# rezashkv/diffusion_pruning

Measured on AMD Instinct MI355X. Metric: denoise-steps/s (SD-2.1 U-Net forward, 512x512, bs=4 per GPU, 50% channel mask), higher is better.
Workload: dtype bf16; 1 GPU; BASELINE configs[1]: SD-2.1 UNet2DConditionModelGated.forward, 64x64 latents (512x512), bs=4/GPU, fixed 50% mask (gated semantics), seeded random-init weights, HIP graph replay; global_batch=4, parallelism=replicas x1 (no data-path collective)

## Files before the change

diffusion_pruning_amd/csrc/conv_gemm.hip:

```cpp
#include "conv_gemm_core.h"

using namespace aptp_cg;

namespace {

template <typename T> struct Elem;
template <> struct Elem<__bf16> { static constexpr int EPC = 8, KS = 64; };
template <> struct Elem<float> { static constexpr int EPC = 4, KS = 32; };

template <int BM, int BN, int WM, int WN, typename T = __bf16>
__global__ __launch_bounds__(256) void conv_gemm_kernel(const KParams p) {
  static_assert(WM * WN == 4, "4 waves per workgroup");
  constexpr int EPC = Elem<T>::EPC, KS = Elem<T>::KS, ES = (int)sizeof(T);
  constexpr bool F32 = sizeof(T) == 4;
  constexpr int WTM = BM / WM, WTN = BN / WN;
  constexpr int MF = WTM / 16, NF = WTN / 16;
  constexpr int A_PASS = BM / 32, B_PASS = BN / 32;
  static_assert(BM % 32 == 0 && BN % 32 == 0 && WTM % 16 == 0 && WTN % 16 == 0, "tile shape");

  __shared__ __attribute__((aligned(16))) T smem[2 * (BM + BN) * KS];
  T* As = smem;
  T* Bs = smem + 2 * BM * KS;

  const int tid = threadIdx.x, lane = tid & 63, wave = tid >> 6;
  const int wm = wave / WN, wn = wave % WN;
  const int tiles_n = (p.N + BN - 1) / BN;
  const int tiles_m = (p.M + BM - 1) / BM;
  int tm, tn, kz;
  decode_block(p, tiles_m, tiles_n, tm, tn, kz);
  const int m0 = tm * BM, n0 = tn * BN;
  const int kt_begin = p.fd_sk.div(p.nK * kz);
  const int kt_end = p.fd_sk.div(p.nK * (kz + 1));
  LnRaw<MF> ln_raw;
  ln_rows_issue<MF, WTM>(p, m0, wm, lane, ln_raw);

  const __amdgpu_buffer_rsrc_t xsrc = __builtin_amdgcn_make_buffer_rsrc(const_cast<__bf16*>(p.x), 0, p.x_bytes, 0x00020000);
  const __amdgpu_buffer_rsrc_t wsrc = __builtin_amdgcn_make_buffer_rsrc(const_cast<__bf16*>(p.w), 0, p.w_bytes, 0x00020000);
  const __amdgpu_buffer_rsrc_t x2src = __builtin_amdgcn_make_buffer_rsrc(const_cast<__bf16*>(p.x2 ? p.x2 : p.x), 0, p.x2 ? p.x2_bytes : 0, 0x00020000);
  constexpr unsigned OOB = 0x80000000u;
  const int chunk = tid & 7, rowbase = tid >> 3;
  int a_iy0[A_PASS], a_ix0[A_PASS], a_pix0[A_PASS], a_m[A_PASS];
#pragma unroll
  for (int i = 0; i < A_PASS; ++i) {
    const int m = m0 + rowbase + 32 * i;
    if (m < p.M) {
      const int b = p.fd_hw.div(m), rem = m - b * p.HW;
      const int oy = p.fd_wout.div(rem), ox = rem - oy * p.Wout;
      a_iy0[i] = oy * p.stride - p.pad;
      a_ix0[i] = ox * p.stride - p.pad;
      a_pix0[i] = b * p.Hin * p.Win;
      a_m[i] = m;
    } else {
      a_iy0[i] = -100000; a_ix0[i] = -100000; a_pix0[i] = 0; a_m[i] = -1;
    }
  }
  unsigned b_off[B_PASS];
#pragma unroll
  for (int i = 0; i < B_PASS; ++i) {
    const int n = n0 + rowbase + 32 * i;
    b_off[i] = n < p.N ? (unsigned)(((int64_t)n * p.Ktot + chunk * EPC) * ES) : OOB;
  }

  const int nk_taps = p.KH * p.KW * p.ncc;
  int l_kt = kt_begin;
  int l_tap = 0, l_cc = 0, l_ky = 0, l_kx = 0;
  if (kt_begin != 0) {
    l_tap = kt_begin / p.ncc;
    l_cc = kt_begin - l_tap * p.ncc;
    l_ky = l_tap / p.KW;
    l_kx = l_tap - l_ky * p.KW;
  }
  if (kt_begin >= nk_taps) { l_ky = p.KH; l_kx = 0; l_cc = kt_begin - nk_taps; }

  u32x4 ra[A_PASS], rb[B_PASS];

  auto load_tile = [&](bool pred) {
    const int c = l_cc * KS + chunk * EPC;
    if (l_ky >= p.KH) {
      const bool c_ok = pred && c < p.Cin2;
#pragma unroll
      for (int i = 0; i < A_PASS; ++i) {
        const unsigned off = ((unsigned)a_m[i] * (unsigned)p.ldx2 + (unsigned)c) * (unsigned)ES;
        ra[i] = __builtin_amdgcn_raw_buffer_load_b128(x2src, (c_ok && a_m[i] >= 0) ? off : OOB, 0, 0);
      }
    } else {
      const bool c_ok = pred && c < p.Cin;
#pragma unroll
      for (int i = 0; i < A_PASS; ++i) {
        int iy = a_iy0[i] + l_ky, ix = a_ix0[i] + l_kx;
        const bool ok = c_ok && (unsigned)iy < (unsigned)p.HinE && (unsigned)ix < (unsigned)p.WinE && !(p.zins & (iy | ix));
        iy >>= p.ups; ix >>= p.ups;
        const unsigned off = ((unsigned)(a_pix0[i] + iy * p.Win + ix) * (unsigned)p.ldx + (unsigned)c) * (unsigned)ES;
        ra[i] = __builtin_amdgcn_raw_buffer_load_b128(xsrc, ok ? off : OOB, 0, 0);
      }
    }
    const unsigned koff = (unsigned)l_kt * (KS * ES);
#pragma unroll
    for (int i = 0; i < B_PASS; ++i) {
      rb[i] = __builtin_amdgcn_raw_buffer_load_b128(wsrc, (b_off[i] == OOB || !pred) ? OOB : b_off[i] + koff, 0, 0);
    }
    ++l_kt;
    if (++l_cc == (l_ky >= p.KH ? p.ncc2 : p.ncc)) {
      l_cc = 0;
      if (++l_kx == p.KW || l_ky >= p.KH) { l_kx = 0; ++l_ky; }
    }
  };

  auto store_tile = [&](int buf) {
#pragma unroll
    for (int i = 0; i < A_PASS; ++i) {
      const int r = rowbase + 32 * i;
      const int sw = chunk ^ ((r >> 1) & 7);
      *reinterpret_cast<u32x4*>(As + (buf * BM + r) * KS + sw * EPC) = ra[i];
    }
#pragma unroll
    for (int i = 0; i < B_PASS; ++i) {
      const int r = rowbase + 32 * i;
      const int sw = chunk ^ ((r >> 1) & 7);
      *reinterpret_cast<u32x4*>(Bs + (buf * BN + r) * KS + sw * EPC) = rb[i];
    }
  };

  f32x4 acc[MF][NF];
#pragma unroll
  for (int i = 0; i < MF; ++i)
#pragma unroll
    for (int j = 0; j < NF; ++j) acc[i][j] = (f32x4){0.f, 0.f, 0.f, 0.f};

  const int frow = lane & 15, fq = lane >> 4;
  auto compute = [&](int buf) {
    if constexpr (F32) {
#pragma unroll
// ... 3 lines not shown
        for (int i = 0; i < MF; ++i) {
          const int r = wm * WTM + i * 16 + frow;
          const int sw = (fq * 2 + h) ^ ((r >> 1) & 7);
          af[i] = *reinterpret_cast<const f32x4*>(As + (buf * BM + r) * KS + sw * EPC);
        }
#pragma unroll
        for (int j = 0; j < NF; ++j) {
          const int r = wn * WTN + j * 16 + frow;
          const int sw = (fq * 2 + h) ^ ((r >> 1) & 7);
          wf[j] = *reinterpret_cast<const f32x4*>(Bs + (buf * BN + r) * KS + sw * EPC);
        }
#pragma unroll
        for (int e = 0; e < 4; ++e)
#pragma unroll
          for (int i = 0; i < MF; ++i)
#pragma unroll
            for (int j = 0; j < NF; ++j)
              acc[i][j] = __builtin_amdgcn_mfma_f32_16x16x4f32(wf[j][e], af[i][e], acc[i][j], 0, 0, 0);
      }
    } else {
#pragma unroll
      for (int s = 0; s < 2; ++s) {
        bf16x8 af[MF], wf[NF];
#pragma unroll
        for (int i = 0; i < MF; ++i) {
          const int r = wm * WTM + i * 16 + frow;
          const int sw = (s * 4 + fq) ^ ((r >> 1) & 7);
          af[i] = *reinterpret_cast<const bf16x8*>(As + (buf * BM + r) * KS + sw * EPC);
        }
#pragma unroll
        for (int j = 0; j < NF; ++j) {
          const int r = wn * WTN + j * 16 + frow;
          const int sw = (s * 4 + fq) ^ ((r >> 1) & 7);
          wf[j] = *reinterpret_cast<const bf16x8*>(Bs + (buf * BN + r) * KS + sw * EPC);
        }
#pragma unroll
        for (int i = 0; i < MF; ++i)
#pragma unroll
          for (int j = 0; j < NF; ++j)
            acc[i][j] = __builtin_amdgcn_mfma_f32_16x16x32_bf16(wf[j], af[i], acc[i][j], 0, 0, 0);
      }
    }
  };

  float ln_mean[MF], ln_rstd[MF];
#pragma unroll
  for (int i = 0; i < MF; ++i) { ln_mean[i] = 0.f; ln_rstd[i] = 1.f; }
  {
    load_tile(kt_begin < kt_end);
    ln_rows_finish<MF>(p, lane, ln_raw, ln_mean, ln_rstd);
    store_tile(0);
    __syncthreads();
    int buf = 0;
    for (int kt = kt_begin; kt < kt_end; ++kt) {
      load_tile((kt + 1) < kt_end);
      compute(buf);
      store_tile(buf ^ 1);
      __syncthreads();
      buf ^= 1;
    }
  }

  if (p.split_k > 1 && p.counters) {
    if (!splitk_combine<256, MF, NF>(p, acc, tm * tiles_n + tn, kz, tid, reinterpret_cast<int*>(smem))) return;
    ln_rows_issue<MF, WTM>(p, m0, wm, lane, ln_raw, true);
    ln_rows_finish<MF>(p, lane, ln_raw, ln_mean, ln_rstd, true);
  } else
  if (p.split_k > 1) {
    float* ws = p.ws + (int64_t)kz * p.M * p.ws_ld;
#pragma unroll
    for (int i = 0; i < MF; ++i) {
      const int m = m0 + wm * WTM + i * 16 + frow;
      if (m >= p.M) continue;
#pragma unroll
      for (int j = 0; j < NF; ++j) {
        const int n = n0 + wn * WTN + j * 16 + fq * 4;
        if (n >= p.N) continue;
        float4 o; o.x = acc[i][j][0]; o.y = acc[i][j][1]; o.z = acc[i][j][2]; o.w = acc[i][j][3];
        *reinterpret_cast<float4*>(ws + (int64_t)m * p.ws_ld + n) = o;
      }
    }
    return;
  }
  run_epilogue<4, MF, NF, WTM, WTN, WN>(p, acc, m0, n0, tn, wm, wn, lane, wave, ln_mean, ln_rstd, reinterpret_cast<__bf16*>(smem));
}

__device__ uint4 g_zero_page[512];

template <int BM, int BN, int WM, int WN, int STAGES, bool PP = false, int KU = 1, int KS = 1>
__global__ __launch_bounds__(WM * WN * KS * 64) void conv_gemm_dma_kernel(const KParams p) {
  constexpr int NW = WM * WN;
  constexpr int NWA = NW * KS;
  constexpr int NT = NWA * 64;
  constexpr int RPP = NT / 8;
  static_assert(NWA == 4 || NWA == 8, "4 or 8 waves per workgroup");
  static_assert(KS == 1 || (KS == 2 && !PP), "intra-workgroup K split: two copies, ring schedules only");
  constexpr int WTM = BM / WM, WTN = BN / WN;
  constexpr int MF = WTM / 16, NF = WTN / 16;
  constexpr int A_PASS = (BM + RPP - 1) / RPP, B_PASS = (BN + RPP - 1) / RPP;
  static_assert(WTM % 16 == 0 && WTN % 16 == 0 && BM % 8 == 0 && BN % 8 == 0, "tile shape");

  __shared__ __attribute__((aligned(16))) __bf16 smem[STAGES * (BM + BN) * BK];
  __bf16* As = smem;
  __bf16* Bs = smem + STAGES * BM * BK;

  const int tid = threadIdx.x, lane = tid & 63;
  const int wave = __builtin_amdgcn_readfirstlane(tid >> 6);
  const int ks = KS == 2 ? wave / NW : 0, cw = KS == 2 ? wave % NW : wave;
  const int wm = cw / WN, wn = cw % WN;
  const int tiles_n = (p.N + BN - 1) / BN;
  const int tiles_m = (p.M + BM - 1) / BM;
  int tm, tn, kz;
  decode_block(p, tiles_m, tiles_n, tm, tn, kz);
  const int m0 = tm * BM, n0 = tn * BN;
  const int kt_begin = p.fd_sk.div(p.nK * kz);
  const int kt_end = p.fd_sk.div(p.nK * (kz + 1));
  __shared__ unsigned pf_scratch[64];
  prefetch_next(p, tid, NT, pf_scratch);
  LnRaw<MF> ln_raw;
  ln_rows_issue<MF, WTM>(p, m0, wm, lane, ln_raw);

  const int rowbase = tid >> 3;
  const int schunk = (tid & 7) ^ ((rowbase >> 1) & 7);
  const char* zpage = reinterpret_cast<const char*>(g_zero_page) + schunk * 16;
  const char* xbase = reinterpret_cast<const char*>(p.x) + schunk * 16;
  const bool tail_bad = ((p.ncc - 1) * BK + schunk * 8) >= p.Cin;
  const bool tail_bad2 = ((p.ncc2 - 1) * BK + schunk * 8) >= p.Cin2;
  const char* x2base = reinterpret_cast<const char*>(p.x2) + schunk * 16;
  int a_iy0[A_PASS], a_ix0[A_PASS], a_pix0[A_PASS], a_m[A_PASS];
#pragma unroll
  for (int i = 0; i < A_PASS; ++i) {
    const int m = m0 + rowbase + RPP * i;
    if (m < p.M && rowbase + RPP * i < BM) {
      const int b = p.fd_hw.div(m), rem = m - b * p.HW;
      const int oy = p.fd_wout.div(rem), ox = rem - oy * p.Wout;
      a_iy0[i] = oy * p.stride - p.pad;
      a_ix0[i] = ox * p.stride - p.pad;
      a_pix0[i] = b * p.Hin * p.Win;
      a_m[i] = m;
    } else {
      a_iy0[i] = -100000; a_ix0[i] = -100000; a_pix0[i] = 0; a_m[i] = -1;
    }
  }

  const int nk_taps = p.KH * p.KW * p.ncc;
  int l_tap = 0, l_cc = 0, l_ky = 0, l_kx = 0;
  if (kt_begin != 0) {
    l_tap = kt_begin / p.ncc;
    l_cc = kt_begin - l_tap * p.ncc;
    l_ky = l_tap / p.KW;
    l_kx = l_tap - l_ky * p.KW;
  }
  if (kt_begin >= nk_taps) { l_ky = p.KH; l_kx = 0; l_cc = kt_begin - nk_taps; }

  const char* a_ptr[A_PASS];
  auto set_tap = [&](int cc0) {
    if (l_ky >= p.KH) {
#pragma unroll
      for (int i = 0; i < A_PASS; ++i) {
        const uint64_t va = reinterpret_cast<uint64_t>(x2base) + ((unsigned)a_m[i] * (unsigned)p.ldx2) * 2u + (unsigned)cc0 * (BK * 2);
        const uint64_t vz = reinterpret_cast<uint64_t>(zpage) + (unsigned)cc0 * (BK * 2);
        a_ptr[i] = reinterpret_cast<const char*>((a_m[i] >= 0 && p.x2) ? va : vz);
      }
      return;
    }
#pragma unroll
    for (int i = 0; i < A_PASS; ++i) {
      int iy = a_iy0[i] + l_ky, ix = a_ix0[i] + l_kx;
      const bool ok = (unsigned)iy < (unsigned)p.HinE && (unsigned)ix < (unsigned)p.WinE && !(p.zins & (iy | ix));
      iy >>= p.ups; ix >>= p.ups;
      const unsigned off = ((unsigned)(a_pix0[i] + iy * p.Win + ix) * (unsigned)p.ldx) * 2u + (unsigned)cc0 * (BK * 2);
      const uint64_t va = reinterpret_cast<uint64_t>(xbase) + off;
      const uint64_t vz = reinterpret_cast<uint64_t>(zpage) + (unsigned)cc0 * (BK * 2);
      a_ptr[i] = reinterpret_cast<const char*>(ok ? va : vz);
    }
  };
  const char* b_ptr[B_PASS];
#pragma unroll
  for (int i = 0; i < B_PASS; ++i) {
    int n = n0 + rowbase + RPP * i;
    n = n < p.N ? n : p.N - 1;
    b_ptr[i] = reinterpret_cast<const char*>(p.w) + ((int64_t)n * p.Ktot + (int64_t)kt_begin * BK + schunk * 8) * 2;
  }
  set_tap(l_cc);

  auto issue_tile = [&](int buf) {
    const bool seg2 = l_ky >= p.KH;
    const bool last_cc = l_cc == (seg2 ? p.ncc2 : p.ncc) - 1;
    const bool tb = seg2 ? tail_bad2 : tail_bad;
#pragma unroll
    for (int i = 0; i < A_PASS; ++i) {
      if (wave * 8 + RPP * i < BM) {
        const char* src = (last_cc && tb) ? zpage : a_ptr[i];
        __bf16* dst = As + (buf * BM + wave * 8 + RPP * i) * BK;
        __builtin_amdgcn_global_load_lds((gbl_ptr)src, (lds_ptr)dst, 16, 0, 0);
      }
      a_ptr[i] += BK * 2;
    }
#pragma unroll
    for (int i = 0; i < B_PASS; ++i) {
      if (wave * 8 + RPP * i < BN) {
        __bf16* dst = Bs + (buf * BN + wave * 8 + RPP * i) * BK;
        __builtin_amdgcn_global_load_lds((gbl_ptr)b_ptr[i], (lds_ptr)dst, 16, 0, 0);
      }
      b_ptr[i] += BK * 2;
    }
    if (++l_cc == (seg2 ? p.ncc2 : p.ncc)) {
      l_cc = 0;
      if (++l_kx == p.KW || seg2) { l_kx = 0; ++l_ky; }
      set_tap(0);
    }
  };

  f32x4 acc[MF][NF];
  zero_acc(acc);

  const int frow = lane & 15, fq = lane >> 4;
  auto compute = [&](int buf) {
#pragma unroll
    for (int s0 = 0; s0 < 2 / KS; ++s0) {
      const int s = KS == 2 ? ks : s0;
      bf16x8 af[MF], wf[NF];
#pragma unroll
      for (int i = 0; i < MF; ++i) {
        const int r = wm * WTM + i * 16 + frow;
        const int sw = (s * 4 + fq) ^ ((r >> 1) & 7);
        af[i] = *reinterpret_cast<const bf16x8*>(As + (buf * BM + r) * BK + sw * 8);
      }
#pragma unroll
      for (int j = 0; j < NF; ++j) {
        const int r = wn * WTN + j * 16 + frow;
        const int sw = (s * 4 + fq) ^ ((r >> 1) & 7);
        wf[j] = *reinterpret_cast<const bf16x8*>(Bs + (buf * BN + r) * BK + sw * 8);
      }
#pragma unroll
      for (int i = 0; i < MF; ++i)
#pragma unroll
        for (int j = 0; j < NF; ++j) {
          acc[i][j] = __builtin_amdgcn_mfma_f32_16x16x32_bf16(wf[j], af[i], acc[i][j], 0, 0, 0);
        }
    }
  };

  float ln_mean[MF], ln_rstd[MF];
#pragma unroll
  for (int i = 0; i < MF; ++i) { ln_mean[i] = 0.f; ln_rstd[i] = 1.f; }
  if constexpr (STAGES == 2 && !PP && KU == 1) {
    if (kt_begin < kt_end) {
      issue_tile(0);
      ln_rows_finish<MF>(p, lane, ln_raw, ln_mean, ln_rstd);
      __syncthreads();
      int buf = 0;
      for (int kt = kt_begin; kt < kt_end; ++kt) {
        if (kt + 1 < kt_end) issue_tile(buf ^ 1);
        compute(buf);
        __syncthreads();
        buf ^= 1;
      }
    }
  } else {
    constexpr int D = (PP || KU == 2) ? STAGES - 2 : STAGES - 1;
    constexpr int DW = KU == 2 ? D - 2 : D - 1;
    constexpr int A_FULL = BM / RPP, B_FULL = BN / RPP;
    constexpr int NLD_LO = A_FULL + B_FULL, NLD_HI = A_PASS + B_PASS;
    static_assert(BM % RPP == 0, "ring: the activation tile must be whole row passes");
    static_assert(!PP || (NWA == 8 && KS == 1 && KU == 1), "ping-pong needs 8 waves");
    const bool hi = (NLD_HI != NLD_LO) && (wave * 8 + RPP * (B_PASS - 1) < BN);
    auto wait_ring = [&](bool full) { ring_wait<NLD_LO, NLD_HI, DW>(hi, full); };
    const int n = kt_end - kt_begin;
    if (n > 0) {
      const int pre = n < D ? n : D;
      for (int t = 0; t < pre; ++t) issue_tile(t);
      ln_rows_finish<MF>(p, lane, ln_raw, ln_mean, ln_rstd);
      wait_ring(pre == D);
      __builtin_amdgcn_s_barrier();
      asm volatile("" ::: "memory");
      if constexpr (PP) kloop_pp<STAGES, D>(n, wave >> 2, issue_tile, compute, wait_ring);
      else if constexpr (KU == 2) kloop_ku2<STAGES, D>(n, issue_tile, compute, wait_ring);
      else kloop_ring<STAGES, D>(n, issue_tile, compute, wait_ring);
    }
  }

  if constexpr (KS == 2) {
    f32x4* xch = reinterpret_cast<f32x4*>(smem) + cw * (MF * NF * 64) + lane;
    if (ks == 1) {
#pragma unroll
      for (int i = 0; i < MF; ++i)
#pragma unroll
        for (int j = 0; j < NF; ++j) xch[(i * NF + j) * 64] = acc[i][j];
    }
    __syncthreads();
    if (ks == 1) return;
#pragma unroll
    for (int i = 0; i < MF; ++i)
#pragma unroll
      for (int j = 0; j < NF; ++j) acc[i][j] += xch[(i * NF + j) * 64];
  }
  if (p.split_k > 1 && p.counters) {
    if (!splitk_combine<NW * 64, MF, NF>(p, acc, tm * tiles_n + tn, kz, tid, reinterpret_cast<int*>(smem))) return;
    ln_rows_issue<MF, WTM>(p, m0, wm, lane, ln_raw, true);
    ln_rows_finish<MF>(p, lane, ln_raw, ln_mean, ln_rstd, true);
  } else
  if (p.split_k > 1) {
    store_splitk_slab(p, acc, kz, m0 + wm * WTM, n0 + wn * WTN, frow, fq);
    return;
  }
  static_assert(NW * 16 * (WTN + 4) * 4 <= (int)sizeof(smem), "epilogue transpose buffer");
  static_assert(KS == 1 || NW * MF * NF * 64 * 16 <= (int)sizeof(smem), "accumulator hand-over buffer");
  run_epilogue<NW, MF, NF, WTM, WTN, WN>(p, acc, m0, n0, tn, wm, wn, lane, cw, ln_mean, ln_rstd, smem);
}

template <int BN, int STAGES>
__global__ __launch_bounds__(512) void conv3x3_halo_kernel(const KParams p) {
  constexpr int BM = 128, WM = 4, WN = 2, NW = 8, NT = 512, RPP = 64;
  constexpr int WTM = BM / WM, WTN = BN / WN, MF = WTM / 16, NF = WTN / 16;
  constexpr int PROWS = 264;
  constexpr int P_PASS = (PROWS + RPP - 1) / RPP, B_PASS = (BN + RPP - 1) / RPP;
  constexpr int D = STAGES - 1;
  static_assert(WTN % 16 == 0 && STAGES >= 3, "tile shape");

  __shared__ __attribute__((aligned(16))) __bf16 smem[2 * PROWS * BK + STAGES * BN * BK];
  __bf16* Ps = smem;
  __bf16* Bs = smem + 2 * PROWS * BK;

  const int tid = threadIdx.x, lane = tid & 63;
  const int wave = __builtin_amdgcn_readfirstlane(tid >> 6);
  const int wm = wave / WN, wn = wave % WN;
  const int tiles_n = (p.N + BN - 1) / BN;
  const int tiles_m = (p.M + BM - 1) / BM;
  int tm, tn, kz;
  decode_block(p, tiles_m, tiles_n, tm, tn, kz);
  const int m0 = tm * BM, n0 = tn * BN;
  const int kt_begin = p.fd_sk.div(p.nK * kz);
  const int kt_end = p.fd_sk.div(p.nK * (kz + 1));
  LnRaw<MF> ln_raw;
  ln_rows_issue<MF, WTM>(p, m0, wm, lane, ln_raw);

  const int W = p.Wout, PW = W + 2, R = BM / W;
  const int prows = (R + 2) * PW;
  const int b_img = p.fd_hw.div(m0), oy0 = (m0 - b_img * p.HW) / W;

  const int rowbase = tid >> 3;
  const int schunk = (tid & 7) ^ ((rowbase >> 1) & 7);
  const char* zpage = reinterpret_cast<const char*>(g_zero_page) + schunk * 16;
  const bool tail_bad = ((p.ncc - 1) * BK + schunk * 8) >= p.Cin;
  const char* p_ptr[P_PASS];
#pragma unroll
  for (int i = 0; i < P_PASS; ++i) {
    const int pr_ = rowbase + RPP * i;
    const int pr = pr_ / PW, pc = pr_ - pr * PW;
    const int iy = oy0 - 1 + pr, ix = pc - 1;
    const bool ok = pr_ < prows && (unsigned)iy < (unsigned)p.Hin && (unsigned)ix < (unsigned)p.Win;
    const unsigned off = ((unsigned)((b_img * p.Hin + iy) * p.Win + ix) * (unsigned)p.ldx) * 2u;
    p_ptr[i] = ok ? reinterpret_cast<const char*>(p.x) + off + schunk * 16 : nullptr;
  }
  auto issue_patch = [&](int cc, int pbuf) {
    const bool bad = tail_bad && cc == p.ncc - 1;
#pragma unroll
    for (int i = 0; i < P_PASS; ++i) {
      if (wave * 8 + RPP * i < prows) {
        const char* src = (p_ptr[i] && !bad) ? p_ptr[i] + cc * (BK * 2) : zpage;
        __bf16* dst = Ps + (pbuf * PROWS + wave * 8 + RPP * i) * BK;
        __builtin_amdgcn_global_load_lds((gbl_ptr)src, (lds_ptr)dst, 16, 0, 0);
      }
    }
  };
  const char* b_row[B_PASS];
#pragma unroll
  for (int i = 0; i < B_PASS; ++i) {
    int n = n0 + rowbase + RPP * i;
    n = n < p.N ? n : p.N - 1;
    b_row[i] = reinterpret_cast<const char*>(p.w) + ((int64_t)n * p.Ktot + schunk * 8) * 2;
  }
  const int cin_pad = p.ncc * BK;
  auto issue_w = [&](int kt, int stage) {
    const int cc = kt / 9, tap = kt - cc * 9;
    const int koff = (tap * cin_pad + cc * BK) * 2;
#pragma unroll
    for (int i = 0; i < B_PASS; ++i) {
      if (wave * 8 + RPP * i < BN) {
        __bf16* dst = Bs + (stage * BN + wave * 8 + RPP * i) * BK;
        __builtin_amdgcn_global_load_lds((gbl_ptr)(b_row[i] + koff), (lds_ptr)dst, 16, 0, 0);
      }
    }
  };

  f32x4 acc[MF][NF];
  zero_acc(acc);

  const int frow = lane & 15, fq = lane >> 4;
  int prow0[MF];
#pragma unroll
// ... 15 lines not shown
        af[i] = *reinterpret_cast<const bf16x8*>(Ps + (pbuf * PROWS + pr_) * BK + sw * 8);
      }
#pragma unroll
      for (int j = 0; j < NF; ++j) {
        const int r = wn * WTN + j * 16 + frow;
        const int sw = (s2 * 4 + fq) ^ ((r >> 1) & 7);
        wf[j] = *reinterpret_cast<const bf16x8*>(Bs + (stage * BN + r) * BK + sw * 8);
      }
#pragma unroll
      for (int i = 0; i < MF; ++i)
#pragma unroll
        for (int j = 0; j < NF; ++j)
          acc[i][j] = __builtin_amdgcn_mfma_f32_16x16x32_bf16(wf[j], af[i], acc[i][j], 0, 0, 0);
    }
  };

  float ln_mean[MF], ln_rstd[MF];
#pragma unroll
  for (int i = 0; i < MF; ++i) { ln_mean[i] = 0.f; ln_rstd[i] = 1.f; }

  constexpr int B_FULL = BN / RPP;
  constexpr int NLD_LO = B_FULL, NLD_HI = B_PASS;
  const bool hi = (NLD_HI != NLD_LO) && (wave * 8 + RPP * (B_PASS - 1) < BN);
  const int nld = hi ? NLD_HI : NLD_LO;
  int pw_cnt = 0;
#pragma unroll
  for (int i = 0; i < P_PASS; ++i) pw_cnt += (wave * 8 + RPP * i < prows) ? 1 : 0;
  auto wait_vm = [&](int allowed) {
    switch (allowed) {
      case 4: asm volatile("s_waitcnt vmcnt(4)" ::: "memory"); break;
      case 6: asm volatile("s_waitcnt vmcnt(6)" ::: "memory"); break;
      case 7: asm volatile("s_waitcnt vmcnt(7)" ::: "memory"); break;
      case 8: asm volatile("s_waitcnt vmcnt(8)" ::: "memory"); break;
      case 9: asm volatile("s_waitcnt vmcnt(9)" ::: "memory"); break;
      case 10: asm volatile("s_waitcnt vmcnt(10)" ::: "memory"); break;
      case 11: asm volatile("s_waitcnt vmcnt(11)" ::: "memory"); break;
      default: asm volatile("s_waitcnt vmcnt(0)" ::: "memory"); break;
    }
  };
  const int n = kt_end - kt_begin;
  if (n > 0) {
    const int cc_first = kt_begin / 9;
    issue_patch(cc_first, cc_first & 1);
    const int pre = n < D ? n : D;
    for (int t = 0; t < pre; ++t) issue_w(kt_begin + t, t);
    ln_rows_finish<MF>(p, lane, ln_raw, ln_mean, ln_rstd);
    ring_wait<NLD_LO, NLD_HI, D - 1>(hi, pre == D);
    __builtin_amdgcn_s_barrier();
    asm volatile("" ::: "memory");
    int cur = 0, nxt = D % STAGES;
    int cc = cc_first, tap = kt_begin - cc_first * 9;
    int since_patch = D;
    for (int kt = kt_begin; kt < kt_end; ++kt) {
      const bool issue = kt + D < kt_end;
      if (issue) issue_w(kt + D, nxt);
      if ((tap == 0 || kt == kt_begin) && (cc + 1) * 9 < kt_end) { issue_patch(cc + 1, (cc + 1) & 1); since_patch = 0; }
      compute(cc & 1, tap, cur);
      asm volatile("" ::: "memory");
      if (issue) wait_vm(nld * (D - 1) + (since_patch < D ? pw_cnt : 0));
      else asm volatile("s_waitcnt vmcnt(0)" ::: "memory");
      ++since_patch;
      asm volatile("s_waitcnt lgkmcnt(0)" ::: "memory");
      __builtin_amdgcn_s_barrier();
      asm volatile("" ::: "memory");
      cur = cur + 1 == STAGES ? 0 : cur + 1;
      nxt = nxt + 1 == STAGES ? 0 : nxt + 1;
      if (++tap == 9) { tap = 0; ++cc; }
    }
  }

  if (p.split_k > 1 && p.counters) {
    if (!splitk_combine<NT, MF, NF>(p, acc, tm * tiles_n + tn, kz, tid, reinterpret_cast<int*>(smem))) return;
    ln_rows_issue<MF, WTM>(p, m0, wm, lane, ln_raw, true);
    ln_rows_finish<MF>(p, lane, ln_raw, ln_mean, ln_rstd, true);
  } else
  if (p.split_k > 1) {
    store_splitk_slab(p, acc, kz, m0 + wm * WTM, n0 + wn * WTN, frow, fq);
    return;
  }
  static_assert(NW * 16 * (WTN + 4) * 4 <= (int)sizeof(smem), "epilogue transpose buffer");
  run_epilogue<NW, MF, NF, WTM, WTN, WN>(p, acc, m0, n0, tn, wm, wn, lane, wave, ln_mean, ln_rstd, smem);
}

__global__ __launch_bounds__(256) void splitk_reduce_kernel(const KParams p) {
  const int quads = (p.act == APTP_ACT_GEGLU) ? p.N / 8 : p.N / 4;
  const int64_t idx = (int64_t)blockIdx.x * blockDim.x + threadIdx.x;
  if (idx >= (int64_t)p.M * quads) return;
  const int m = (int)(idx / quads);
  const int q = (int)(idx - (int64_t)m * quads);
  int n;
  if (p.act == APTP_ACT_GEGLU) n = (q >> 2) * 32 + (q & 3) * 4;
  else n = q * 4;
  float h[4] = {0.f, 0.f, 0.f, 0.f}, g[4] = {0.f, 0.f, 0.f, 0.f};
  for (int z0 = 0; z0 < p.split_k; z0 += 4) {
    float4 a[4], c[4];
#pragma unroll
    for (int u = 0; u < 4; ++u) {
      const int z = z0 + u < p.split_k ? z0 + u : z0;
      const float* row = p.ws + ((int64_t)z * p.M + m) * p.ws_ld;
      a[u] = *reinterpret_cast<const float4*>(row + n);
      if (p.act == APTP_ACT_GEGLU) c[u] = *reinterpret_cast<const float4*>(row + n + 16);
    }
#pragma unroll
    for (int u = 0; u < 4; ++u) {
      if (z0 + u < p.split_k) {
        h[0] += a[u].x; h[1] += a[u].y; h[2] += a[u].z; h[3] += a[u].w;
        if (p.act == APTP_ACT_GEGLU) { g[0] += c[u].x; g[1] += c[u].y; g[2] += c[u].z; g[3] += c[u].w; }
      }
    }
  }
  RowCtx rc;
  row_info(p, m, rc);
  if (p.ln_stats) {
    const float4* sp = reinterpret_cast<const float4*>(p.ln_stats);
    float a = 0.f, a2 = 0.f;
    for (int pr = 0; pr < (p.ln_slots >> 1); ++pr) { const float4 t = sp[(int64_t)pr * p.M + m]; a += t.x + t.z; a2 += t.y + t.w; }
    ln_finish(p, a, a2, rc);
  }
  float st[2] = {0.f, 0.f};
  if (p.act == APTP_ACT_GEGLU) epilogue_quad<true>(p, m, rc, n, h, g, st);
  else epilogue_quad<false>(p, m, rc, n, h, h, st);
}

constexpr int GN_RED_NT = 1024;
constexpr int GN_RED_QPT = 6;
__global__ __launch_bounds__(GN_RED_NT) void splitk_reduce_gn_kernel(const KParams p) {
  __shared__ float red[2][GN_RED_NT];
  __shared__ float stat[2];
  const int g = blockIdx.x, b = blockIdx.y, tid = threadIdx.x;
  const int cg = p.gn_C / p.gn_groups, qpr = cg >> 2;
  const int nquads = p.HW * qpr;
  float v[GN_RED_QPT][4];
  float s1 = 0.f, s2 = 0.f;
#pragma unroll
  for (int i = 0; i < GN_RED_QPT; ++i) {
    const int q = tid + GN_RED_NT * i;
    if (q < nquads) {
      const int r = q / qpr, n = g * cg + (q - r * qpr) * 4;
      const int m = b * p.HW + r;
      float a[4] = {0.f, 0.f, 0.f, 0.f};
      for (int z0 = 0; z0 < p.split_k; z0 += 4) {
        float4 t[4];
#pragma unroll
        for (int u = 0; u < 4; ++u) {
          const int z = z0 + u < p.split_k ? z0 + u : z0;
          t[u] = *reinterpret_cast<const float4*>(p.ws + ((int64_t)z * p.M + m) * p.ws_ld + n);
        }
#pragma unroll
        for (int u = 0; u < 4; ++u)
          if (z0 + u < p.split_k) { a[0] += t[u].x; a[1] += t[u].y; a[2] += t[u].z; a[3] += t[u].w; }
      }
#pragma unroll
      for (int e = 0; e < 4; ++e) {
        float x = a[e];
        if (p.bias) x += p.bias[n + e];
        if (p.rowbias) x += p.rowbias[(int64_t)b * p.ld_rowbias + n + e];
        x = (float)(__bf16)x;
        v[i][e] = x;
        s1 += x; s2 += x * x;
      }
    }
  }
  red[0][tid] = s1; red[1][tid] = s2;
  __syncthreads();
  if (tid < 64) {
    float a = 0.f, c = 0.f;
#pragma unroll
    for (int w = 0; w < GN_RED_NT / 64; ++w) { a += red[0][tid + 64 * w]; c += red[1][tid + 64 * w]; }
#pragma unroll
    for (int off = 32; off >= 1; off >>= 1) { a += __shfl_xor(a, off); c += __shfl_xor(c, off); }
    if (tid == 0) {
      const float inv = 1.0f / ((float)cg * (float)p.HW);
      const float mean = a * inv;
      float var = c * inv - mean * mean;
      var = var < 0.f ? 0.f : var;
      stat[0] = mean; stat[1] = rsqrtf(var + p.gn_eps);
    }
  }
  __syncthreads();
  const float mean = stat[0], rstd = stat[1];
  __bf16* y = reinterpret_cast<__bf16*>(p.y);
#pragma unroll
  for (int i = 0; i < GN_RED_QPT; ++i) {
    const int q = tid + GN_RED_NT * i;
    if (q < nquads) {
      const int r = q / qpr, n = g * cg + (q - r * qpr) * 4;
      const int m = b * p.HW + r;
      float o[4];
#pragma unroll
      for (int e = 0; e < 4; ++e) {
        const float z = (v[i][e] - mean) * rstd * p.gn_gamma[n + e] + p.gn_beta[n + e];
        o[e] = p.gn_silu ? silu_f(z) : z;
      }
      uint2 pk; pk.x = pack_bf16x2(o[0], o[1]); pk.y = pack_bf16x2(o[2], o[3]);
      *reinterpret_cast<uint2*>(y + (int64_t)m * p.ldy + n) = pk;
    }
  }
  if (g == p.gn_groups - 1 && p.N > p.gn_C) {
    const int padw = p.N - p.gn_C;
    for (int e = tid; e < p.HW * padw; e += GN_RED_NT) {
      const int r = e / padw, n = p.gn_C + (e - r * padw);
      y[(int64_t)(b * p.HW + r) * p.ldy + n] = (__bf16)0.0f;
    }
  }
}

int pick_tile(const AptpConvGemmParams* p, int M) {
  if (p->tile != APTP_TILE_AUTO) return p->tile;
  const bool geglu = p->act == APTP_ACT_GEGLU;
  auto waste = [&](int bn) { return ((p->N + bn - 1) / bn) * bn - p->N; };
  int bn = 128;
  if (!geglu && waste(160) < waste(128)) bn = 160;
  if (p->N <= 64 || (waste(64) < waste(bn) && p->N < 128)) bn = 64;
  auto blocks = [&](int bm, int bn_) { return (int64_t)((M + bm - 1) / bm) * ((p->N + bn_ - 1) / bn_); };
  int bm = blocks(128, bn) >= 512 ? 128 : 64;
  if (bn == 160) return bm == 128 ? APTP_TILE_128x160 : APTP_TILE_64x160;
  if (bn == 128) return bm == 128 ? APTP_TILE_128x128 : APTP_TILE_64x128;
  return bm == 128 ? APTP_TILE_128x64 : APTP_TILE_64x64;
}

int fill_kparams(const AptpConvGemmParams* p, KParams& k) {
  APTP_CHECK(p && p->x && p->w && p->y, "conv_gemm: null pointer");
  APTP_CHECK(p->B > 0 && p->Hin > 0 && p->Win > 0 && p->Hout > 0 && p->Wout > 0, "conv_gemm: bad extent");
  APTP_CHECK(p->Cin > 0 && p->Cin % 8 == 0, "conv_gemm: Cin (%d) must be a positive multiple of 8", p->Cin);
  APTP_CHECK(p->ldx % 8 == 0 && p->ldx >= p->Cin, "conv_gemm: ldx (%lld) must be a multiple of 8 and >= Cin", (long long)p->ldx);
  APTP_CHECK(p->N > 0 && p->N % 8 == 0, "conv_gemm: N (%d) must be a positive multiple of 8", p->N);
  APTP_CHECK(p->cin_pad % BK == 0 && p->cin_pad >= p->Cin && p->cin_pad < p->Cin + BK, "conv_gemm: cin_pad (%d) != ceil(Cin/64)*64", p->cin_pad);
  APTP_CHECK(p->KH >= 1 && p->KW >= 1 && p->stride >= 1 && p->pad >= 0 && p->ups >= 0 && p->ups <= 2, "conv_gemm: bad filter geometry");
  APTP_CHECK(((uintptr_t)p->x % 16) == 0 && ((uintptr_t)p->w % 16) == 0 && ((uintptr_t)p->y % 8) == 0, "conv_gemm: pointer alignment");
  APTP_CHECK((p->act >= APTP_ACT_NONE && p->act <= APTP_ACT_GELU) || p->act == APTP_ACT_QUICK_GELU, "conv_gemm: unknown act %d", p->act);
  const int geglu = p->act == APTP_ACT_GEGLU;
  APTP_CHECK(!geglu || p->N % 32 == 0, "conv_gemm: GEGLU needs N %% 32 == 0");
  const int nout = geglu ? p->N / 2 : p->N;
  APTP_CHECK(p->ldy >= nout && p->ldy % 4 == 0, "conv_gemm: ldy (%lld) must be >= %d and a multiple of 4", (long long)p->ldy, nout);
  APTP_CHECK(!p->colgate || (p->gate_group > 0 && p->gate_B > 0 && nout % p->gate_group == 0), "conv_gemm: bad gate geometry");
  APTP_CHECK(!p->corr || (p->corr_B > 0 && p->Hout >= 2 && p->Wout >= 2), "conv_gemm: corr needs Hout,Wout >= 2");
  APTP_CHECK(!p->residual || (p->ldres % 4 == 0 && ((uintptr_t)p->residual % 8) == 0), "conv_gemm: residual alignment");
  APTP_CHECK(!p->depth || (p->depth_in && p->depth_B > 0 && p->lddin % 4 == 0), "conv_gemm: depth gate needs depth_in");
  APTP_CHECK(!p->rowbias || p->ld_rowbias % 4 == 0, "conv_gemm: ld_rowbias must be a multiple of 4");
  APTP_CHECK(p->split_k >= 1, "conv_gemm: split_k >= 1");
  const int64_t M64 = (int64_t)p->B * p->Hout * p->Wout;
  APTP_CHECK(M64 < (1ll << 31), "conv_gemm: M too large");
  const int sh = p->ups ? 1 : 0;
  const int HinE = p->Hin << sh, WinE = p->Win << sh;
  APTP_CHECK(p->pad_end >= 0, "conv_gemm: pad_end (%d) must be >= 0", p->pad_end);
  APTP_CHECK(p->pad_end == 0 || (!p->corr && !p->x2 && p->ups == 0), "conv_gemm: pad_end > 0 does not go with corr, x2 or ups");
  APTP_CHECK(p->Hout == (HinE + 2 * p->pad + p->pad_end - p->KH) / p->stride + 1 &&
             p->Wout == (WinE + 2 * p->pad + p->pad_end - p->KW) / p->stride + 1,
             "conv_gemm: Hout/Wout inconsistent with input extent, filter, stride and padding");
  k.x = (const __bf16*)p->x; k.ldx = p->ldx;
  k.B = p->B; k.Hin = p->Hin; k.Win = p->Win; k.Cin = p->Cin; k.Hout = p->Hout; k.Wout = p->Wout;
  k.KH = p->KH; k.KW = p->KW; k.stride = p->stride; k.pad = p->pad; k.ups = sh; k.zins = p->ups == 2 ? 1 : 0;
  k.HinE = HinE; k.WinE = WinE;
  const int f32 = p->io_f32 ? 1 : 0, es = f32 ? 4 : 2, ks = f32 ? 32 : BK;
  APTP_CHECK(!f32 || (p->out_f32 && !p->colstat_out && !p->gn_gamma && !p->prefetch),
             "conv_gemm: io_f32 (fp32 parity path) writes fp32 and has no column statistics / fused GroupNorm / prefetch");
  k.io_f32 = f32;
  k.x2 = (const __bf16*)p->x2; k.ldx2 = p->ldx2; k.Cin2 = p->x2 ? p->Cin2 : 0; k.ncc2 = p->x2 ? p->cin2_pad / ks : 0; k.x2_bytes = 0;
  if (p->x2) {
    APTP_CHECK(p->Cin2 > 0 && p->Cin2 % 8 == 0 && p->cin2_pad % BK == 0 && p->cin2_pad >= p->Cin2 && p->cin2_pad < p->Cin2 + BK,
               "conv_gemm: x2 needs Cin2 (%d) a positive multiple of 8 and cin2_pad (%d) == ceil(Cin2/64)*64", p->Cin2, p->cin2_pad);
    APTP_CHECK(p->ldx2 % 8 == 0 && p->ldx2 >= p->Cin2 && ((uintptr_t)p->x2 % 16) == 0, "conv_gemm: x2 row stride / alignment");
    APTP_CHECK(p->stride == 1 && p->ups == 0 && p->Hout == p->Hin && p->Wout == p->Win,
               "conv_gemm: x2 (second operand read at the output pixel) needs a stride-1, same-size convolution");
    const int64_t x2b = (((int64_t)p->B * p->Hout * p->Wout - 1) * p->ldx2 + p->Cin2) * es;
    APTP_CHECK(x2b < (1ll << 31), "conv_gemm: x2 larger than 2 GiB");
    k.x2_bytes = (int)x2b;
  }
  k.w = (const __bf16*)p->w; k.N = p->N; k.ncc = p->cin_pad / ks; k.nK = p->KH * p->KW * k.ncc + k.ncc2;
  k.Ktot = (int64_t)k.nK * ks;
  k.bias = p->bias; k.rowbias = p->rowbias; k.ld_rowbias = p->ld_rowbias;
  k.colgate = p->colgate; k.gate_group = p->gate_group; k.gate_B = p->gate_B;
  k.act = p->act; k.corr = p->corr; k.corr_B = p->corr_B;
  k.residual = (const __bf16*)p->residual; k.ldres = p->ldres;
  k.depth = p->depth; k.depth_B = p->depth_B; k.depth_in = (const __bf16*)p->depth_in; k.lddin = p->lddin;
  k.y = p->y; k.ldy = p->ldy; k.out_f32 = p->out_f32;
  k.split_k = p->split_k < k.nK ? p->split_k : k.nK;
  k.ws = (float*)p->workspace;
  k.M = (int)M64; k.HW = p->Hout * p->Wout; k.Nout = nout;
  k.ws_ld = p->N;
  APTP_CHECK(p->order >= 0 && p->order <= 3, "conv_gemm: order %d", p->order);
  if (p->order == 0) {
    const int64_t w_bytes = (int64_t)p->N * k.Ktot * 2;
    const int64_t a_bytes = (int64_t)p->B * p->Hin * p->Win * p->Cin * 2;
    k.order = w_bytes > a_bytes ? 1 : 2;
  } else {
    k.order = p->order - 1;
  }
  k.rstat_out = p->rowstat_out; k.rstat_slots = p->rowstat_slots;
  k.ln_stats = p->ln_stats; k.ln_slots = p->ln_slots; k.ln_colsum = p->ln_colsum; k.ln_eps = p->ln_eps;
  k.ln_invC = p->ln_C > 0 ? 1.0f / (float)p->ln_C : 0.f;
  APTP_CHECK(!p->rowstat_out || (!geglu && (!p->out_f32 || f32) && ((uintptr_t)p->rowstat_out % 16) == 0),
             "conv_gemm: rowstat_out needs a bf16, non-GEGLU output and an 8-byte aligned buffer");
  APTP_CHECK(!p->ln_stats || (p->ln_colsum && p->ln_slots > 0 && p->ln_C > 0 && p->KH == 1 && p->KW == 1 &&
                              p->ln_slots % 2 == 0 && ((uintptr_t)p->ln_stats % 16) == 0 && ((uintptr_t)p->ln_colsum % 16) == 0),
             "conv_gemm: folded LayerNorm needs ln_colsum [N], ln_slots > 0, ln_C > 0 and a 1x1 filter");
  k.counters = p->tile_counters;
  k.pf_ptr = ((uintptr_t)p->prefetch & 3) ? nullptr : (const char*)p->prefetch;
  k.pf_bytes = k.pf_ptr ? (p->prefetch_bytes < (1ll << 36) ? p->prefetch_bytes : (1ll << 36)) : 0;
  k.cstat_out = p->colstat_out; k.cstat_ld = p->colstat_ld;
  k.ustat_out = (long long*)p->ustat_out; k.ustat_unit = p->ustat_unit; k.ustat_units = p->ustat_units; k.ustat_nrep = p->ustat_nrep;
  APTP_CHECK(!p->ustat_out || (p->colstat_out && p->ustat_unit > 0 && p->ustat_units * p->ustat_unit >= nout && p->ustat_nrep >= 1 &&
                               (p->ustat_nrep & (p->ustat_nrep - 1)) == 0 && ((uintptr_t)p->ustat_out % 8) == 0),
             "conv_gemm: ustat_out goes with colstat_out; ustat_unit > 0, ustat_units >= ceil(N_out / unit), ustat_nrep a power of two");
  k.epi16 = !p->out_f32 && p->ldy % 8 == 0 && ((uintptr_t)p->y % 16) == 0 && nout % 8 == 0 &&
            (!p->residual || (p->ldres % 8 == 0 && ((uintptr_t)p->residual % 16) == 0)) &&
            (!p->depth || (p->lddin % 8 == 0 && ((uintptr_t)p->depth_in % 16) == 0));
  if (p->epilogue == 1) k.epi16 = 0;
  const int64_t xb = (((int64_t)p->B * p->Hin * p->Win - 1) * p->ldx + p->Cin) * es;
  const int64_t wb = (int64_t)p->N * k.Ktot * es;
  APTP_CHECK(xb < (1ll << 31) && wb < (1ll << 31), "conv_gemm: operand larger than 2 GiB");
  k.x_bytes = (int)xb; k.w_bytes = (int)wb;
  return APTP_OK;
}

template <int BM, int BN>
dim3 tile_grid(const KParams& k) { return dim3(((k.M + BM - 1) / BM) * ((k.N + BN - 1) / BN) * k.split_k, 1, 1); }
template <int BM, int BN, int WM, int WN>
void launch_tile(const KParams& k, hipStream_t s) {
  if (k.io_f32) hipLaunchKernelGGL((conv_gemm_kernel<BM, BN, WM, WN, float>), (tile_grid<BM, BN>(k)), dim3(256), 0, s, k);
  else hipLaunchKernelGGL((conv_gemm_kernel<BM, BN, WM, WN>), (tile_grid<BM, BN>(k)), dim3(256), 0, s, k);
}

template <int BM, int BN, int WM, int WN, int STAGES, bool PP, int KU, int KS>
void launch_dma(const KParams& k, hipStream_t s) {
  hipLaunchKernelGGL((conv_gemm_dma_kernel<BM, BN, WM, WN, STAGES, PP, KU, KS>), (tile_grid<BM, BN>(k)), dim3(WM * WN * KS * 64), 0, s, k);
}

template <int BM, int BN, int STAGES>
int launch_halo(const AptpConvGemmParams* p, const KParams& k, hipStream_t s) {
  static_assert(BM == 128, "conv3x3_halo_kernel: 128 output pixels per tile");
  const int W = p->Wout;
  if (!(p->KH == 3 && p->KW == 3 && p->stride == 1 && p->pad == 1 && p->pad_end == 0 && p->ups == 0 && !p->x2 && W > 0 && 128 % W == 0 &&
        (p->Hout * W) % 128 == 0 && (128 / W + 2) * (W + 2) <= 264)) {
    aptp_set_error("conv_gemm: the halo tiles need a 3x3 / stride-1 / pad-1 convolution without x2 whose width divides 128 (16, 32 or 64)");
    return APTP_EINVAL;
  }
  hipLaunchKernelGGL((conv3x3_halo_kernel<BN, STAGES>), (tile_grid<BM, BN>(k)), dim3(512), 0, s, k);
  return APTP_OK;
}

template <TileFamily F, int BM, int BN, int WM, int WN, int STAGES, int KU, int KS>
int launch_row(const AptpConvGemmParams* p, const KParams& k, int t, hipStream_t s) {
  if constexpr (F == TileFamily::REG) launch_tile<BM, BN, WM, WN>(k, s);
  else if constexpr (F == TileFamily::DMA || F == TileFamily::PP) launch_dma<BM, BN, WM, WN, STAGES, F == TileFamily::PP, KU, KS>(k, s);
  else if constexpr (F == TileFamily::HALO) return launch_halo<BM, BN, STAGES>(p, k, s);
  else if (k.split_k > 1 && !k.counters) { aptp_set_error("conv_gemm: the stream-K tiles combine in-kernel: split_k > 1 needs tile_counters"); return APTP_EINVAL; }
  else return aptp_launch_sk(k, t, s);
  return APTP_OK;
}

}

extern "C" int64_t aptp_conv_gemm_workspace_bytes(const AptpConvGemmParams* p) {
  if (!p || p->split_k <= 1) return 0;
  const int64_t M = (int64_t)p->B * p->Hout * p->Wout;
  const int t = pick_tile(p, (int)M);
  if (is_sk_tile(t))
    return (int64_t)aptp_sk_cus() * 2 * kTiles[t].bm * kTiles[t].bn * (int64_t)sizeof(float);
  int64_t mp = M, np = p->N;
  if (t > 0 && t < kNumTiles) {
    mp = (M + kTiles[t].bm - 1) / kTiles[t].bm * kTiles[t].bm;
    np = ((int64_t)p->N + kTiles[t].bn - 1) / kTiles[t].bn * kTiles[t].bn;
  }
  return (int64_t)p->split_k * mp * np * (int64_t)sizeof(float);
}

extern "C" int aptp_conv_gemm_tiles(const AptpConvGemmParams* p) {
  if (!p) return 0;
  const int64_t M = (int64_t)p->B * p->Hout * p->Wout;
  const int t = pick_tile(p, (int)M);
  if (t <= 0 || t >= kNumTiles) return 0;
  return (int)(((M + kTiles[t].bm - 1) / kTiles[t].bm) * ((p->N + kTiles[t].bn - 1) / kTiles[t].bn));
}

extern "C" int aptp_conv_gemm_colstat_rows(const AptpConvGemmParams* p) {
  if (!p) return 0;
  const int t = pick_tile(p, p->B * p->Hout * p->Wout);
  if (t <= 0 || t >= kNumTiles) return 0;
  return kTiles[t].bm / (kTiles[t].nw / kTiles[t].wn);
}

extern "C" int aptp_conv_gemm_rowstat_slots(const AptpConvGemmParams* p) {
  if (!p) return 0;
  const int t = pick_tile(p, p->B * p->Hout * p->Wout);
  if (t <= 0 || t >= kNumTiles) return 0;
  return ((p->N + kTiles[t].bn - 1) / kTiles[t].bn) * kTiles[t].wn;
}

extern "C" int aptp_conv_gemm_suggest_split_k(const AptpConvGemmParams* p) {
  if (!p) return 1;
  const int M = p->B * p->Hout * p->Wout;
  const int t = pick_tile(p, M);
  const int64_t blocks = (int64_t)((M + kTiles[t].bm - 1) / kTiles[t].bm) * ((p->N + kTiles[t].bn - 1) / kTiles[t].bn);
  const int nK = p->KH * p->KW * (p->cin_pad / BK);
  if (blocks >= 256) return 1;
  int s = (int)((512 + blocks - 1) / blocks);
  const int max_s = nK / 8 > 0 ? nK / 8 : 1;
  if (s > max_s) s = max_s;
  if (s > 32) s = 32;
  return s < 1 ? 1 : s;
}

extern "C" int aptp_conv_gemm(const AptpConvGemmParams* p, aptp_stream_t stream) {
  KParams k;
  const int rc = fill_kparams(p, k);
  if (rc != APTP_OK) return rc;
  if (k.split_k > 1) APTP_CHECK(k.ws != nullptr && ((uintptr_t)k.ws % 16) == 0, "conv_gemm: split_k > 1 needs a 16B-aligned workspace");
  if (k.split_k == 1) k.counters = nullptr;
  k.gn_gamma = p->gn_gamma; k.gn_beta = p->gn_beta; k.gn_groups = p->gn_groups; k.gn_C = p->gn_C; k.gn_silu = p->gn_silu; k.gn_eps = p->gn_eps;
  if (k.gn_gamma) {
    APTP_CHECK(k.gn_beta && k.split_k > 1 && !k.counters && !k.out_f32 && k.act == APTP_ACT_NONE && !k.colgate && !k.corr && !k.residual && !k.depth
               && !k.rstat_out && !k.cstat_out && !k.ln_stats, "conv_gemm: gn_gamma needs a plain bf16 convolution split along K with a reduce launch");
    APTP_CHECK(k.gn_groups > 0 && k.gn_C > 0 && k.gn_C <= k.N && k.gn_C % k.gn_groups == 0 && k.gn_C % 8 == 0 && (k.gn_C / k.gn_groups) % 4 == 0
               && (int64_t)k.HW * (k.gn_C / k.gn_groups) <= 4LL * GN_RED_QPT * GN_RED_NT && k.ldy % 4 == 0,
               "conv_gemm: gn_gamma geometry (C=%d groups=%d HW=%d)", k.gn_C, k.gn_groups, k.HW);
  }
  hipStream_t s = (hipStream_t)stream;
  int t = pick_tile(p, k.M);
  if (t < 0 || t >= kNumTiles) { aptp_set_error("conv_gemm: unknown tile %d", t); return APTP_EINVAL; }
  if (k.io_f32 && !is_reg_tile(t)) {
    aptp_set_error("conv_gemm: io_f32 (fp32 parity path) runs on the register-staged tiles 1..6 only (got tile %d)", t);
    return APTP_EINVAL;
  }
  if (is_dma_tile(t) && (p->cin_pad * 2 > 8064 || (p->x2 && p->cin2_pad * 2 > 8064))) {
    aptp_set_error("conv_gemm: LDS-DMA tiles need Cin <= 4032 (got cin_pad %d)", p->cin_pad);
    return APTP_EINVAL;
  }
  if (k.rstat_out) {
    const int slots = ((k.N + kTiles[t].bn - 1) / kTiles[t].bn) * kTiles[t].wn;
    if ((k.split_k != 1 && !k.counters) || k.rstat_slots != slots) {
      aptp_set_error("conv_gemm: rowstat_out needs split_k == 1 (or the in-kernel reduction) and rowstat_slots == aptp_conv_gemm_rowstat_slots() (%d), got split_k %d, slots %d",
                     slots, k.split_k, k.rstat_slots);
      return APTP_EINVAL;
    }
  }
  if (k.cstat_out) {
    const int wtm = kTiles[t].bm / (kTiles[t].nw / kTiles[t].wn), wtn = kTiles[t].bn / kTiles[t].wn;
    if (!k.epi16 || k.act == APTP_ACT_GEGLU || (k.split_k != 1 && !k.counters) || k.HW % wtm != 0 || wtn < 32 ||
        k.cstat_ld < k.Nout || ((uintptr_t)k.cstat_out % 8) != 0) {
      aptp_set_error("conv_gemm: colstat_out needs the coalesced bf16 epilogue, no GEGLU, split_k == 1 (or the in-kernel reduction), "
                     "Hout*Wout %% %d == 0 (aptp_conv_gemm_colstat_rows) and colstat_ld >= N", wtm);
      return APTP_EINVAL;
    }
    const int wl = k.act == APTP_ACT_GEGLU ? wtn / 2 : wtn;
    if (k.ustat_out && (wl % k.ustat_unit == 0 ? wl / k.ustat_unit : (wl - 1) / k.ustat_unit + 2) > 64) {
      aptp_set_error("conv_gemm: ustat_unit %d too small for the %d columns of a wave of tile %d (at most 64 units per wave)", k.ustat_unit, wl, t);
      return APTP_EINVAL;
    }
  }
  if (k.act == APTP_ACT_GEGLU && (kTiles[t].bn == 160)) {
    aptp_set_error("conv_gemm: GEGLU cannot use a 160-wide tile");
    return APTP_EINVAL;
  }
  {
    const int tiles_m = (k.M + kTiles[t].bm - 1) / kTiles[t].bm, tiles_n = (k.N + kTiles[t].bn - 1) / kTiles[t].bn;
    APTP_CHECK((int64_t)tiles_m * tiles_n * k.split_k < (1ll << 31) && (int64_t)k.nK * (k.split_k + 1) < (1ll << 31), "conv_gemm: grid too large");
    k.fd_hw = make_fastdiv(k.HW); k.fd_wout = make_fastdiv(k.Wout);
    k.fd_tm = make_fastdiv(tiles_m); k.fd_tn = make_fastdiv(tiles_n); k.fd_sk = make_fastdiv(k.split_k);
    k.fd_perm = make_fastdiv(tiles_n * k.split_k); k.fd_tmn = make_fastdiv(tiles_m * tiles_n);
  }
  static const bool lin_on = !(getenv("APTP_LIN") && getenv("APTP_LIN")[0] == '0');
  if (lin_on && p->epilogue != 2 && p->pad_end == 0 && aptp_lin_eligible(k, t)) {
    const int rc2 = aptp_launch_lin(k, t, s);
    if (rc2 != APTP_OK) return rc2;
    APTP_LAUNCH_CHECK();
    return APTP_OK;
  }
  static const bool lean_on = !(getenv("APTP_CONV_LEAN") && getenv("APTP_CONV_LEAN")[0] == '0');
  int rc2 = APTP_OK;
  if (lean_on && p->epilogue == 0 && p->pad_end == 0 && aptp_conv_lean_eligible(k, t)) rc2 = aptp_launch_conv_lean(k, t, s);
  else switch (t) {
#define X(NAME, FAMILY, BM, BN, WM, WN, STAGES, KU, KS, LIN, C3) \
    case APTP_TILE_##NAME: rc2 = launch_row<TileFamily::FAMILY, BM, BN, WM, WN, STAGES, KU, KS>(p, k, t, s); break;
    APTP_CONV_GEMM_TILES(X)
#undef X
    default: aptp_set_error("conv_gemm: unknown tile %d", t); return APTP_EINVAL;
  }
  if (rc2 != APTP_OK) return rc2;
  APTP_LAUNCH_CHECK();
  if (k.split_k > 1 && !k.counters) {
    if (k.gn_gamma) {
      hipLaunchKernelGGL(splitk_reduce_gn_kernel, dim3(k.gn_groups, k.B), dim3(GN_RED_NT), 0, s, k);
    } else {
      const int quads = (k.act == APTP_ACT_GEGLU) ? k.N / 8 : k.N / 4;
      const int64_t total = (int64_t)k.M * quads;
      hipLaunchKernelGGL(splitk_reduce_kernel, dim3((unsigned)((total + 255) / 256)), dim3(256), 0, s, k);
    }
    APTP_LAUNCH_CHECK();
  }
  return APTP_OK;
}
```

diffusion_pruning_amd/csrc/conv_gemm_core.h:

```cpp
#pragma once
#include "aptp_common.h"

namespace aptp_cg {


constexpr int BK = 64;
typedef __attribute__((ext_vector_type(4))) unsigned int u32x4;

struct FastDiv {
  unsigned mul, shr, one;
  __device__ __forceinline__ int div(int n) const { return (int)((__umulhi((unsigned)n, mul) + ((unsigned)n & one)) >> shr); }
};

struct KParams {
  const __bf16* x; int64_t ldx;
  int B, Hin, Win, Cin, Hout, Wout, KH, KW, stride, pad, ups;
  int zins;
  int HinE, WinE;
  const __bf16* w; int N; int ncc; int nK; int64_t Ktot;
  const __bf16* x2; int64_t ldx2; int Cin2; int ncc2; int x2_bytes;
  const float* bias; const float* rowbias; int ld_rowbias;
  const float* colgate; int gate_group, gate_B;
  int act;
  const float* corr; int corr_B;
  const __bf16* residual; int64_t ldres;
  const float* depth; int depth_B; const __bf16* depth_in; int64_t lddin;
  void* y; int64_t ldy; int out_f32;
  int split_k; float* ws;
  int x_bytes, w_bytes;
  int M, HW, Nout;
  int64_t ws_ld;
  int order;
  const char* pf_ptr; int64_t pf_bytes;
  int pf_lines, pf_per;
  int* counters;
  float* cstat_out; int cstat_ld;
  int epi16;
  int io_f32;
  float* rstat_out; int rstat_slots;
  const float* ln_stats; int ln_slots; const float* ln_colsum; float ln_eps; float ln_invC;
  const float* gn_gamma; const float* gn_beta; int gn_groups, gn_C, gn_silu; float gn_eps;
  long long* ustat_out; int ustat_unit, ustat_units, ustat_nrep;
  FastDiv fd_hw, fd_wout;
  FastDiv fd_tm, fd_tn, fd_sk, fd_perm, fd_tmn;
};

__device__ __forceinline__ void decode_block(const KParams& p, int tiles_m, int tiles_n, int& tm, int& tn, int& kz) {
  const int L = blockIdx.x;
  if (p.order == 0) {
    kz = p.fd_tmn.div(L);
    const int t = L - kz * (tiles_m * tiles_n);
    tm = p.fd_tn.div(t);
    tn = t - tm * tiles_n;
    return;
  }
  const int T = gridDim.x;
  const int xcd = L & 7, j = L >> 3;
  const int qq = T >> 3, r = T & 7;
  const int q = (xcd < r ? xcd * (qq + 1) : r * (qq + 1) + (xcd - r) * qq) + j;
  if (p.order == 1) {
    const int w = p.fd_tm.div(q);
    tm = q - w * tiles_m;
    tn = p.fd_sk.div(w);
    kz = w - tn * p.split_k;
  } else {
    const int per_m = tiles_n * p.split_k;
    tm = p.fd_perm.div(q);
    const int rest = q - tm * per_m;
    kz = p.fd_tn.div(rest);
    tn = rest - kz * tiles_n;
  }
}

struct RowCtx { int b, cls; float mean, rstd; };

struct ColVecs { float4 cs, cg, bb, bg; };

template <bool GEGLU>
__device__ __forceinline__ void load_colvecs(const KParams& p, int n, ColVecs& c) {
  c.cs = c.cg = c.bb = c.bg = make_float4(0.f, 0.f, 0.f, 0.f);
  if (p.ln_stats) {
    c.cs = *reinterpret_cast<const float4*>(p.ln_colsum + n);
    if (GEGLU) c.cg = *reinterpret_cast<const float4*>(p.ln_colsum + n + 16);
  }
  if (p.bias) {
    c.bb = *reinterpret_cast<const float4*>(p.bias + n);
    if (GEGLU) c.bg = *reinterpret_cast<const float4*>(p.bias + n + 16);
  }
}

template <bool GEGLU>
__device__ __forceinline__ void epilogue_pre(const KParams& p, const RowCtx& rc, int n, const ColVecs& cv, float h[4], float g[4], float v[4]) {
  const int b = rc.b, cls = rc.cls;
  if (p.ln_stats) {
    h[0] = rc.rstd * (h[0] - rc.mean * cv.cs.x); h[1] = rc.rstd * (h[1] - rc.mean * cv.cs.y);
    h[2] = rc.rstd * (h[2] - rc.mean * cv.cs.z); h[3] = rc.rstd * (h[3] - rc.mean * cv.cs.w);
    if (GEGLU) {
      g[0] = rc.rstd * (g[0] - rc.mean * cv.cg.x); g[1] = rc.rstd * (g[1] - rc.mean * cv.cg.y);
      g[2] = rc.rstd * (g[2] - rc.mean * cv.cg.z); g[3] = rc.rstd * (g[3] - rc.mean * cv.cg.w);
    }
  }
  if (p.bias) {
    h[0] += cv.bb.x; h[1] += cv.bb.y; h[2] += cv.bb.z; h[3] += cv.bb.w;
    if (GEGLU) { g[0] += cv.bg.x; g[1] += cv.bg.y; g[2] += cv.bg.z; g[3] += cv.bg.w; }
  }
  if (p.rowbias) {
    const float4 rb = *reinterpret_cast<const float4*>(p.rowbias + (int64_t)b * p.ld_rowbias + n);
    h[0] += rb.x; h[1] += rb.y; h[2] += rb.z; h[3] += rb.w;
  }
  const int c = GEGLU ? ((n >> 5) * 16 + (n & 15)) : n;
  if (p.colgate) {
    const float* gr = p.colgate + (int64_t)(b % p.gate_B) * ((GEGLU ? p.Nout : p.N) / p.gate_group);
#pragma unroll
    for (int r = 0; r < 4; ++r) {
      const float gm = gr[(c + r) / p.gate_group];
      h[r] *= gm;
      if (GEGLU) g[r] *= gm;
    }
  }
  if (GEGLU) {
#pragma unroll
    for (int r = 0; r < 4; ++r) v[r] = h[r] * gelu_erf_f(g[r]);
  } else if (p.act == APTP_ACT_SILU) {
#pragma unroll
    for (int r = 0; r < 4; ++r) v[r] = silu_f(h[r]);
  } else if (p.act == APTP_ACT_GELU) {
#pragma unroll
    for (int r = 0; r < 4; ++r) v[r] = gelu_erf_f(h[r]);
  } else if (p.act == APTP_ACT_QUICK_GELU) {
#pragma unroll
    for (int r = 0; r < 4; ++r) v[r] = quick_gelu_f(h[r]);
  } else {
#pragma unroll
    for (int r = 0; r < 4; ++r) v[r] = h[r];
  }
  if (p.corr) {
    const float4 cc = *reinterpret_cast<const float4*>(p.corr + ((int64_t)(b % p.corr_B) * 9 + cls) * p.Nout + c);
    v[0] += cc.x; v[1] += cc.y; v[2] += cc.z; v[3] += cc.w;
  }
}

template <bool GEGLU>
__device__ __forceinline__ void epilogue_quad(const KParams& p, int m, const RowCtx& rc, int n, float h[4], float g[4], float st[2]) {
  const int b = rc.b;
  float v[4];
  ColVecs cv;
  load_colvecs<GEGLU>(p, n, cv);
  epilogue_pre<GEGLU>(p, rc, n, cv, h, g, v);
  const int c = GEGLU ? ((n >> 5) * 16 + (n & 15)) : n;
  if (p.residual) {
    if (p.io_f32) {
      const float4 rr = *reinterpret_cast<const float4*>(reinterpret_cast<const float*>(p.residual) + (int64_t)m * p.ldres + c);
      v[0] += rr.x; v[1] += rr.y; v[2] += rr.z; v[3] += rr.w;
    } else {
      const uint2 rr = *reinterpret_cast<const uint2*>(p.residual + (int64_t)m * p.ldres + c);
      union { uint2 u; __bf16 e[4]; } ru; ru.u = rr;
#pragma unroll
      for (int r = 0; r < 4; ++r) v[r] += (float)ru.e[r];
    }
  }
  if (p.depth) {
    const float d = p.depth[b % p.depth_B];
    float din[4];
    if (p.io_f32) {
      const float4 rr = *reinterpret_cast<const float4*>(reinterpret_cast<const float*>(p.depth_in) + (int64_t)m * p.lddin + c);
      din[0] = rr.x; din[1] = rr.y; din[2] = rr.z; din[3] = rr.w;
    } else {
      const uint2 rr = *reinterpret_cast<const uint2*>(p.depth_in + (int64_t)m * p.lddin + c);
      union { uint2 u; __bf16 e[4]; } ru; ru.u = rr;
#pragma unroll
      for (int r = 0; r < 4; ++r) din[r] = (float)ru.e[r];
    }
#pragma unroll
    for (int r = 0; r < 4; ++r) v[r] = (1.0f - d) * din[r] + d * v[r];
  }
  if (p.out_f32) {
    float4 o; o.x = v[0]; o.y = v[1]; o.z = v[2]; o.w = v[3];
    *reinterpret_cast<float4*>(reinterpret_cast<float*>(p.y) + (int64_t)m * p.ldy + c) = o;
    if (p.io_f32 && p.rstat_out) {
#pragma unroll
      for (int r = 0; r < 4; ++r) { st[0] += v[r]; st[1] += v[r] * v[r]; }
    }
  } else {
    union { uint2 u; __bf16 e[4]; } o;
    o.u.x = pack_bf16x2(v[0], v[1]); o.u.y = pack_bf16x2(v[2], v[3]);
    *reinterpret_cast<uint2*>(reinterpret_cast<__bf16*>(p.y) + (int64_t)m * p.ldy + c) = o.u;
    if (p.rstat_out) {
#pragma unroll
      for (int r = 0; r < 4; ++r) { const float f = (float)o.e[r]; st[0] += f; st[1] += f * f; }
    }
  }
}

__device__ __forceinline__ void row_info(const KParams& p, int m, RowCtx& rc) {
  rc.b = p.fd_hw.div(m);
  rc.cls = 4;
  rc.mean = 0.f; rc.rstd = 1.f;
  if (p.corr) {
    const int rem = m - rc.b * p.HW;
    const int oy = p.fd_wout.div(rem), ox = rem - oy * p.Wout;
    const int rr = oy == 0 ? 0 : (oy == p.Hout - 1 ? 2 : 1);
    const int cc = ox == 0 ? 0 : (ox == p.Wout - 1 ? 2 : 1);
    rc.cls = rr * 3 + cc;
  }
}

__device__ __forceinline__ void ln_finish(const KParams& p, float a, float a2, RowCtx& rc) {
  const float mean = a * p.ln_invC;
  float var = a2 * p.ln_invC - mean * mean;
  var = var < 0.f ? 0.f : var;
  rc.mean = mean;
  rc.rstd = rsqrtf(var + p.ln_eps);
}

template <int MF>
struct LnRaw { float4 v[4][MF]; int mr[MF]; };

template <int MF, int WTM>
__device__ __forceinline__ void ln_rows_issue(const KParams& p, int m0, int wm, int lane, LnRaw<MF>& raw, bool split_ok = false) {
  if (!p.ln_stats || (p.split_k > 1 && !split_ok)) return;
  const int frow = lane & 15, fq = lane >> 4;
  const float4* sp = reinterpret_cast<const float4*>(p.ln_stats);
  const int npair = p.ln_slots >> 1;
#pragma unroll
  for (int i = 0; i < MF; ++i) {
    const int m = m0 + wm * WTM + i * 16 + frow;
    raw.mr[i] = m < p.M ? m : p.M - 1;
  }
#pragma unroll
  for (int u = 0; u < 4; ++u) {
    if (u * 4 < npair) {
      const int pr = u * 4 + fq;
      const int64_t row0 = (int64_t)(pr < npair ? pr : 0) * p.M;
#pragma unroll
      for (int i = 0; i < MF; ++i) raw.v[u][i] = sp[row0 + raw.mr[i]];
    } else {
#pragma unroll
      for (int i = 0; i < MF; ++i) raw.v[u][i] = make_float4(0.f, 0.f, 0.f, 0.f);
    }
  }
  asm volatile("" ::: "memory");
}

template <int MF>
__device__ __forceinline__ void ln_rows_finish(const KParams& p, int lane, const LnRaw<MF>& raw, float (&ln_mean)[MF], float (&ln_rstd)[MF],
                                               bool split_ok = false) {
  if (!p.ln_stats || (p.split_k > 1 && !split_ok)) return;
  const int fq = lane >> 4;
  const float4* sp = reinterpret_cast<const float4*>(p.ln_stats);
  const int npair = p.ln_slots >> 1;
  float lna[MF], lna2[MF];
#pragma unroll
  for (int i = 0; i < MF; ++i) { lna[i] = 0.f; lna2[i] = 0.f; }
#pragma unroll
  for (int u = 0; u < 4; ++u) {
    const bool ok = u * 4 + fq < npair;
#pragma unroll
    for (int i = 0; i < MF; ++i) {
      lna[i] += ok ? raw.v[u][i].x + raw.v[u][i].z : 0.f;
      lna2[i] += ok ? raw.v[u][i].y + raw.v[u][i].w : 0.f;
    }
  }
  for (int base = 16; base < npair; base += 16) {
#pragma unroll
    for (int u = 0; u < 4; ++u) {
      if (base + u * 4 < npair) {
        const int pr = base + u * 4 + fq;
        const bool ok = pr < npair;
        const int64_t row0 = (int64_t)(ok ? pr : 0) * p.M;
#pragma unroll
        for (int i = 0; i < MF; ++i) {
          const float4 t = sp[row0 + raw.mr[i]];
          lna[i] += ok ? t.x + t.z : 0.f; lna2[i] += ok ? t.y + t.w : 0.f;
        }
      }
    }
  }
#pragma unroll
  for (int i = 0; i < MF; ++i) {
    lna[i] += __shfl_xor(lna[i], 16); lna2[i] += __shfl_xor(lna2[i], 16);
    lna[i] += __shfl_xor(lna[i], 32); lna2[i] += __shfl_xor(lna2[i], 32);
    RowCtx rc;
    ln_finish(p, lna[i], lna2[i], rc);
    ln_mean[i] = rc.mean; ln_rstd[i] = rc.rstd;
  }
}

template <int MF, int NF, int WTM, int WTN, int WN>
__device__ __forceinline__ void tile_epilogue(const KParams& p, f32x4 (&acc)[MF][NF], int m0, int n0, int tn, int wm, int wn, int lane,
                                              const float (&ln_mean)[MF], const float (&ln_rstd)[MF]) {
  const int frow = lane & 15, fq = lane >> 4;
#pragma unroll
  for (int i = 0; i < MF; ++i) {
    const int m = m0 + wm * WTM + i * 16 + frow;
    if (m >= p.M) continue;
    RowCtx rc;
    row_info(p, m, rc);
    rc.mean = ln_mean[i]; rc.rstd = ln_rstd[i];
    float st[2] = {0.f, 0.f};
    if (p.act == APTP_ACT_GEGLU) {
      if constexpr (NF % 2 == 0) {
#pragma unroll
        for (int j = 0; j < NF; j += 2) {
          const int n = n0 + wn * WTN + j * 16 + fq * 4;
          if (n >= p.N) continue;
          float h[4] = {acc[i][j][0], acc[i][j][1], acc[i][j][2], acc[i][j][3]};
          float g[4] = {acc[i][j + 1][0], acc[i][j + 1][1], acc[i][j + 1][2], acc[i][j + 1][3]};
          epilogue_quad<true>(p, m, rc, n, h, g, st);
        }
      }
    } else {
#pragma unroll
      for (int j = 0; j < NF; ++j) {
        const int n = n0 + wn * WTN + j * 16 + fq * 4;
        if (n >= p.N) continue;
        float h[4] = {acc[i][j][0], acc[i][j][1], acc[i][j][2], acc[i][j][3]};
        epilogue_quad<false>(p, m, rc, n, h, h, st);
      }
    }
    if (p.rstat_out) {
      st[0] += __shfl_xor(st[0], 16); st[1] += __shfl_xor(st[1], 16);
      st[0] += __shfl_xor(st[0], 32); st[1] += __shfl_xor(st[1], 32);
      if (fq == 0) {
        float2 o; o.x = st[0]; o.y = st[1];
        const int slot = tn * WN + wn;
        reinterpret_cast<float2*>(p.rstat_out)[((int64_t)(slot >> 1) * p.M + m) * 2 + (slot & 1)] = o;
      }
    }
  }
}

constexpr float USTAT_SUM_SCALE = 1048576.0f;
constexpr float USTAT_SQ_SCALE = 4096.0f;
template <int WL>
__device__ __forceinline__ void emit_unit_stats(const KParams& p, const float (&tot)[2][(WL + 63) / 64], float* buf, int lane, int cw0,
                                                int row0) {
  __builtin_amdgcn_fence(__ATOMIC_ACQ_REL, "wavefront");
  __builtin_amdgcn_wave_barrier();
#pragma unroll
  for (int q = 0; q < (WL + 63) / 64; ++q) {
    const int t = lane + 64 * q;
    if (t < WL) { buf[t] = tot[0][q]; buf[WL + t] = tot[1][q]; }
  }
  __builtin_amdgcn_fence(__ATOMIC_ACQ_REL, "wavefront");
  __builtin_amdgcn_wave_barrier();
  const int cend = cw0 + WL < p.Nout ? cw0 + WL : p.Nout;
  if (cw0 >= cend || row0 >= p.M) return;
  const int unit = p.ustat_unit;
  const int u0 = cw0 / unit, u1 = (cend - 1) / unit;
  const int u = u0 + lane;
  if (u > u1) return;
  const int lo = (u * unit > cw0 ? u * unit : cw0) - cw0;
  const int hi = ((u + 1) * unit < cend ? (u + 1) * unit : cend) - cw0;
  float s = 0.f, s2 = 0.f;
  for (int c = lo; c < hi; ++c) { s += buf[c]; s2 += buf[WL + c]; }
  const int b = p.fd_hw.div(row0);
  const int rep = (int)blockIdx.x & (p.ustat_nrep - 1);
  unsigned long long* dst = reinterpret_cast<unsigned long long*>(p.ustat_out) + (((int64_t)rep * p.B + b) * p.ustat_units + u) * 2;
  __hip_atomic_fetch_add(dst, (unsigned long long)__float2ll_rn(s * USTAT_SUM_SCALE), __ATOMIC_RELAXED, __HIP_MEMORY_SCOPE_AGENT);
  __hip_atomic_fetch_add(dst + 1, (unsigned long long)__float2ll_rn(s2 * USTAT_SQ_SCALE), __ATOMIC_RELAXED, __HIP_MEMORY_SCOPE_AGENT);
}

template <int WL, int RPP>
__device__ __forceinline__ void emit_col_stats(const KParams& p, const float (&cs)[8], const float (&cs2)[8], float* buf, int lane, int lrow,
                                               int lc8, int cw0, int rblk, int row0) {
  float tot[2][(WL + 63) / 64];
#pragma unroll
  for (int ph = 0; ph < 2; ++ph) {
    if (lrow < RPP) {
      float* dst = buf + lrow * WL + lc8 * 8;
      if (ph == 0) {
        *reinterpret_cast<float4*>(dst) = make_float4(cs[0], cs[1], cs[2], cs[3]);
        *reinterpret_cast<float4*>(dst + 4) = make_float4(cs[4], cs[5], cs[6], cs[7]);
      } else {
        *reinterpret_cast<float4*>(dst) = make_float4(cs2[0], cs2[1], cs2[2], cs2[3]);
        *reinterpret_cast<float4*>(dst + 4) = make_float4(cs2[4], cs2[5], cs2[6], cs2[7]);
      }
    }
    __builtin_amdgcn_fence(__ATOMIC_ACQ_REL, "wavefront");
    __builtin_amdgcn_wave_barrier();
#pragma unroll
    for (int q = 0; q < (WL + 63) / 64; ++q) {
      const int t = lane + 64 * q;
      float a = 0.f;
      if (t < WL) {
#pragma unroll
        for (int r = 0; r < RPP; ++r) a += buf[r * WL + t];
      }
      tot[ph][q] = a;
    }
    __builtin_amdgcn_fence(__ATOMIC_ACQ_REL, "wavefront");
    __builtin_amdgcn_wave_barrier();
  }
  float2* dstg = reinterpret_cast<float2*>(p.cstat_out) + (int64_t)rblk * p.cstat_ld;
#pragma unroll
  for (int q = 0; q < (WL + 63) / 64; ++q) {
    const int t = lane + 64 * q;
    if (t < WL && cw0 + t < p.Nout) dstg[cw0 + t] = make_float2(tot[0][q], tot[1][q]);
  }
  if (p.ustat_out) emit_unit_stats<WL>(p, tot, buf, lane, cw0, row0);
}

template <bool GEGLU, int MF, int NF, int WTM, int WTN, int WN>
__device__ __forceinline__ void tile_epilogue_lds(const KParams& p, f32x4 (&acc)[MF][NF], int m0, int n0, int tn, int wm, int wn,
                                                  int lane, const float (&ln_mean)[MF], const float (&ln_rstd)[MF], float* buf) {
  constexpr int WL = GEGLU ? WTN / 2 : WTN;
  constexpr int PITCH = WL + 4;
  constexpr int LPR = WL / 8;
  constexpr int RPP = 64 / LPR;
  constexpr int NPASS = (16 + RPP - 1) / RPP;
  constexpr bool POW2 = (LPR & (LPR - 1)) == 0;
  const int frow = lane & 15, fq = lane >> 4;
  const int lrow = lane / LPR, lc8 = lane - lrow * LPR;
  const int c0 = (GEGLU ? ((n0 + wn * WTN) >> 1) : (n0 + wn * WTN)) + lc8 * 8;
  const bool lane_on = lrow < RPP && c0 < p.Nout;
  __bf16* const yb = reinterpret_cast<__bf16*>(p.y);
  float cs[8], cs2[8];
#pragma unroll
  for (int e = 0; e < 8; ++e) { cs[e] = 0.f; cs2[e] = 0.f; }
#pragma unroll
  for (int i = 0; i < MF; ++i) {
    const int mbase = m0 + wm * WTM + i * 16;
    u32x4 rres[NPASS], rdin[NPASS];
#pragma unroll
    for (int ps = 0; ps < NPASS; ++ps) {
      const int r = ps * RPP + lrow, m2 = mbase + r;
      const bool on = lane_on && r < 16 && m2 < p.M;
      rres[ps] = (u32x4){0u, 0u, 0u, 0u}; rdin[ps] = (u32x4){0u, 0u, 0u, 0u};
      if (on && p.residual) rres[ps] = *reinterpret_cast<const u32x4*>(p.residual + (int64_t)m2 * p.ldres + c0);
      if (on && p.depth) rdin[ps] = *reinterpret_cast<const u32x4*>(p.depth_in + (int64_t)m2 * p.lddin + c0);
    }
    {
      const int m = mbase + frow;
      RowCtx rc;
      row_info(p, m < p.M ? m : p.M - 1, rc);
      rc.mean = ln_mean[i]; rc.rstd = ln_rstd[i];
      if constexpr (GEGLU) {
        if constexpr (NF % 2 == 0) {
#pragma unroll
          for (int j = 0; j < NF; j += 2) {
            const int n = n0 + wn * WTN + j * 16 + fq * 4;
            float h[4] = {acc[i][j][0], acc[i][j][1], acc[i][j][2], acc[i][j][3]};
            float g[4] = {acc[i][j + 1][0], acc[i][j + 1][1], acc[i][j + 1][2], acc[i][j + 1][3]};
            float v[4] = {0.f, 0.f, 0.f, 0.f};
            if (n < p.N) {
              ColVecs cv;
              load_colvecs<true>(p, n, cv);
              epilogue_pre<true>(p, rc, n, cv, h, g, v);
            }
            *reinterpret_cast<float4*>(buf + frow * PITCH + (j / 2) * 16 + fq * 4) = make_float4(v[0], v[1], v[2], v[3]);
          }
        }
      } else {
#pragma unroll
        for (int j = 0; j < NF; ++j) {
          const int n = n0 + wn * WTN + j * 16 + fq * 4;
          float h[4] = {acc[i][j][0], acc[i][j][1], acc[i][j][2], acc[i][j][3]};
          float v[4] = {0.f, 0.f, 0.f, 0.f};
          if (n < p.N) {
            ColVecs cv;
            load_colvecs<false>(p, n, cv);
            epilogue_pre<false>(p, rc, n, cv, h, h, v);
          }
          *reinterpret_cast<float4*>(buf + frow * PITCH + j * 16 + fq * 4) = make_float4(v[0], v[1], v[2], v[3]);
        }
      }
    }
    __builtin_amdgcn_fence(__ATOMIC_ACQ_REL, "wavefront");
    __builtin_amdgcn_wave_barrier();
#pragma unroll
    for (int ps = 0; ps < NPASS; ++ps) {
      const int r = ps * RPP + lrow, m2 = mbase + r;
      const bool on = lane_on && r < 16 && m2 < p.M;
      float v[8];
      {
        const int rr = r < 16 ? r : 15;
        const float4 a = *reinterpret_cast<const float4*>(buf + rr * PITCH + lc8 * 8);
        const float4 b4 = *reinterpret_cast<const float4*>(buf + rr * PITCH + lc8 * 8 + 4);
        v[0] = a.x; v[1] = a.y; v[2] = a.z; v[3] = a.w; v[4] = b4.x; v[5] = b4.y; v[6] = b4.z; v[7] = b4.w;
      }
      if (p.residual) {
        float f[8];
        union { u32x4 v; uint4 s; } cv; cv.v = rres[ps];
        unpack_bf16x8(cv.s, f);
#pragma unroll
        for (int e = 0; e < 8; ++e) v[e] += f[e];
      }
      if (p.depth) {
        const float d = p.depth[p.fd_hw.div(m2 < p.M ? m2 : p.M - 1) % p.depth_B];
        float f[8];
        union { u32x4 v; uint4 s; } cv; cv.v = rdin[ps];
        unpack_bf16x8(cv.s, f);
#pragma unroll
        for (int e = 0; e < 8; ++e) v[e] = (1.0f - d) * f[e] + d * v[e];
      }
      const uint4 o = pack_bf16x8(v);
      if (on) *reinterpret_cast<uint4*>(yb + (int64_t)m2 * p.ldy + c0) = o;
      if constexpr (!GEGLU) {
        if (p.cstat_out && on) {
          float f[8];
          unpack_bf16x8(o, f);
#pragma unroll
          for (int e = 0; e < 8; ++e) { cs[e] += f[e]; cs2[e] += f[e] * f[e]; }
        }
      }
      if constexpr (POW2) {
        if (p.rstat_out) {
          float f[8], s0 = 0.f, s1 = 0.f;
          unpack_bf16x8(o, f);
          if (c0 < p.Nout) {
#pragma unroll
            for (int e = 0; e < 8; ++e) { s0 += f[e]; s1 += f[e] * f[e]; }
          }
#pragma unroll
          for (int off = 1; off < LPR; off <<= 1) { s0 += __shfl_xor(s0, off); s1 += __shfl_xor(s1, off); }
          if (lrow < RPP && r < 16 && m2 < p.M && lc8 == 0) {
            float2 q; q.x = s0; q.y = s1;
            const int slot = tn * WN + wn;
            reinterpret_cast<float2*>(p.rstat_out)[((int64_t)(slot >> 1) * p.M + m2) * 2 + (slot & 1)] = q;
          }
        }
      }
    }
  }
  if constexpr (!GEGLU && WL >= 32) {
    static_assert(RPP * WL <= 16 * PITCH, "column-statistics staging");
    if (p.cstat_out) emit_col_stats<WL, RPP>(p, cs, cs2, buf, lane, lrow, lc8, n0 + wn * WTN, m0 / WTM + wm, m0 + wm * WTM);
  }
}

template <int WTM, int WTN>
struct LeanEpiIn {
  static constexpr int LPR = WTN / 8, RPF = 64 / LPR, NPF = (16 + RPF - 1) / RPF, NP = (WTM / 16) * NPF;
  float cb[8], rb[8], gm[8];
  float cr[NP][8];
  u32x4 res[NP];
  bool one_b;
};

template <int WTM, int WTN>
__device__ __forceinline__ void lean_epi_sample(const KParams& p, int b, int cc, float (&rb)[8], float (&gm)[8]) {
  if (p.rowbias) {
    const float4 a = *reinterpret_cast<const float4*>(p.rowbias + (int64_t)b * p.ld_rowbias + cc);
    const float4 c = *reinterpret_cast<const float4*>(p.rowbias + (int64_t)b * p.ld_rowbias + cc + 4);
    rb[0] = a.x; rb[1] = a.y; rb[2] = a.z; rb[3] = a.w; rb[4] = c.x; rb[5] = c.y; rb[6] = c.z; rb[7] = c.w;
  }
  if (p.colgate) {
    const float* gr = p.colgate + (int64_t)(b % p.gate_B) * (p.N / p.gate_group);
#pragma unroll
    for (int e = 0; e < 8; ++e) gm[e] = gr[(cc + e) / p.gate_group];
  }
}

template <int WTM, int WTN>
__device__ __forceinline__ void lean_epi_load(const KParams& p, int m0, int n0, int wm, int wn, int lane, LeanEpiIn<WTM, WTN>& in) {
  using E = LeanEpiIn<WTM, WTN>;
  const int lrow = lane / E::LPR, lc8 = lane - lrow * E::LPR;
  const int c0 = n0 + wn * WTN + lc8 * 8;
  const int cc = c0 < p.Nout ? c0 : p.Nout - 8;
  const int mw0 = m0 + wm * WTM;
  const int mf = mw0 < p.M ? mw0 : p.M - 1, ml = mw0 + WTM - 1 < p.M ? mw0 + WTM - 1 : p.M - 1;
  const int b0 = p.fd_hw.div(mf);
  in.one_b = p.fd_hw.div(ml) == b0;
#pragma unroll
  for (int e = 0; e < 8; ++e) { in.cb[e] = 0.f; in.rb[e] = 0.f; in.gm[e] = 1.f; }
  if (p.bias) {
    const float4 a = *reinterpret_cast<const float4*>(p.bias + cc), c = *reinterpret_cast<const float4*>(p.bias + cc + 4);
    in.cb[0] = a.x; in.cb[1] = a.y; in.cb[2] = a.z; in.cb[3] = a.w; in.cb[4] = c.x; in.cb[5] = c.y; in.cb[6] = c.z; in.cb[7] = c.w;
  }
  lean_epi_sample<WTM, WTN>(p, b0, cc, in.rb, in.gm);
#pragma unroll
  for (int q = 0; q < E::NP; ++q) {
    const int i = q / E::NPF, ps = q - i * E::NPF;
    const int r = ps * E::RPF + lrow, m2 = mw0 + i * 16 + (r < 16 ? r : 15);
    const int mc = m2 < p.M ? m2 : p.M - 1;
    in.res[q] = (u32x4){0u, 0u, 0u, 0u};
    if (p.residual) in.res[q] = *reinterpret_cast<const u32x4*>(p.residual + (int64_t)mc * p.ldres + cc);
#pragma unroll
    for (int e = 0; e < 8; ++e) in.cr[q][e] = 0.f;
    if (p.corr) {
      RowCtx rc;
      row_info(p, mc, rc);
      const float* cp = p.corr + ((int64_t)(rc.b % p.corr_B) * 9 + rc.cls) * p.Nout + cc;
      const float4 a = *reinterpret_cast<const float4*>(cp), c = *reinterpret_cast<const float4*>(cp + 4);
      in.cr[q][0] = a.x; in.cr[q][1] = a.y; in.cr[q][2] = a.z; in.cr[q][3] = a.w;
      in.cr[q][4] = c.x; in.cr[q][5] = c.y; in.cr[q][6] = c.z; in.cr[q][7] = c.w;
    }
  }
}

template <int MF, int NF, int WTM, int WTN>
__device__ __forceinline__ void lean_epilogue(const KParams& p, f32x4 (&acc)[MF][NF], int m0, int n0, int wm, int wn, int lane,
                                              const LeanEpiIn<WTM, WTN>& in, float* buf) {
  using E = LeanEpiIn<WTM, WTN>;
  constexpr int WL = WTN, PITCH = WL + 4, LPR = E::LPR, RPF = E::RPF, NPF = E::NPF;
  static_assert(WL % 8 == 0 && WL >= 32 && RPF * WL <= 16 * PITCH, "transposed layout / column-statistics staging");
  const int frow = lane & 15, fq = lane >> 4;
  const int lrow = lane / LPR, lc8 = lane - lrow * LPR;
  const int c0 = n0 + wn * WTN + lc8 * 8;
  const int cc = c0 < p.Nout ? c0 : p.Nout - 8;
  const bool lane_on = lrow < RPF && c0 < p.Nout;
  const int mw0 = m0 + wm * WTM;
  __bf16* const yb = reinterpret_cast<__bf16*>(p.y);
  float cs[8], cs2[8];
#pragma unroll
  for (int e = 0; e < 8; ++e) { cs[e] = 0.f; cs2[e] = 0.f; }
#pragma unroll
  for (int i = 0; i < MF; ++i) {
    if (i > 0) {
      __builtin_amdgcn_fence(__ATOMIC_ACQ_REL, "wavefront");
      __builtin_amdgcn_wave_barrier();
    }
#pragma unroll
    for (int j = 0; j < NF; ++j) *reinterpret_cast<f32x4*>(buf + frow * PITCH + j * 16 + fq * 4) = acc[i][j];
    __builtin_amdgcn_fence(__ATOMIC_ACQ_REL, "wavefront");
    __builtin_amdgcn_wave_barrier();
#pragma unroll
    for (int ps = 0; ps < NPF; ++ps) {
      const int q = i * NPF + ps;
      const int r = ps * RPF + lrow, m2 = mw0 + i * 16 + r;
      const bool on = lane_on && r < 16 && m2 < p.M;
      float v[8];
      {
        const int rr = r < 16 ? r : 15;
        const float4 a = *reinterpret_cast<const float4*>(buf + rr * PITCH + lc8 * 8);
        const float4 b4 = *reinterpret_cast<const float4*>(buf + rr * PITCH + lc8 * 8 + 4);
        v[0] = a.x; v[1] = a.y; v[2] = a.z; v[3] = a.w; v[4] = b4.x; v[5] = b4.y; v[6] = b4.z; v[7] = b4.w;
      }
      float rb[8], gm[8];
#pragma unroll
      for (int e = 0; e < 8; ++e) { rb[e] = in.rb[e]; gm[e] = in.gm[e]; }
      if (!in.one_b && (p.rowbias || p.colgate)) {
        const int mr = mw0 + i * 16 + (r < 16 ? r : 15), mc = mr < p.M ? mr : p.M - 1;
        lean_epi_sample<WTM, WTN>(p, p.fd_hw.div(mc), cc, rb, gm);
      }
      if (p.bias) {
#pragma unroll
        for (int e = 0; e < 8; ++e) v[e] += in.cb[e];
      }
      if (p.rowbias) {
#pragma unroll
        for (int e = 0; e < 8; ++e) v[e] += rb[e];
      }
      if (p.colgate) {
#pragma unroll
        for (int e = 0; e < 8; ++e) v[e] *= gm[e];
      }
      if (p.act == APTP_ACT_SILU) {
#pragma unroll
        for (int e = 0; e < 8; ++e) v[e] = silu_f(v[e]);
      }
      if (p.corr) {
#pragma unroll
        for (int e = 0; e < 8; ++e) v[e] += in.cr[q][e];
      }
#if defined(__HIP_DEVICE_COMPILE__)
#pragma unroll
      for (int e = 0; e < 8; ++e) asm volatile("" : "+v"(v[e]));
#endif
      if (p.residual) {
        float f[8];
        union { u32x4 v; uint4 s; } cv; cv.v = in.res[q];
        unpack_bf16x8(cv.s, f);
#pragma unroll
        for (int e = 0; e < 8; ++e) v[e] += f[e];
      }
      const uint4 o = pack_bf16x8(v);
      if (on) *reinterpret_cast<uint4*>(yb + (int64_t)m2 * p.ldy + c0) = o;
      if (p.cstat_out && on) {
        float f[8];
        unpack_bf16x8(o, f);
#pragma unroll
        for (int e = 0; e < 8; ++e) { cs[e] += f[e]; cs2[e] += f[e] * f[e]; }
      }
    }
  }
  if (p.cstat_out) {
    __builtin_amdgcn_fence(__ATOMIC_ACQ_REL, "wavefront");
    __builtin_amdgcn_wave_barrier();
    emit_col_stats<WL, RPF>(p, cs, cs2, buf, lane, lrow, lc8, n0 + wn * WTN, m0 / WTM + wm, mw0);
  }
}

template <int NT, int MF, int NF>
__device__ __forceinline__ bool splitk_combine(const KParams& p, f32x4 (&acc)[MF][NF], int tile, int kz, int tid, int* lds_word) {
  constexpr int PER = MF * NF;
  float4* const slab = reinterpret_cast<float4*>(p.ws) + (int64_t)tile * p.split_k * (PER * NT);
  float4* const mine = slab + (int64_t)kz * (PER * NT);
  {
    const __amdgpu_buffer_rsrc_t srsrc = __builtin_amdgcn_make_buffer_rsrc(mine, 0, PER * NT * 16, 0x00020000);
#pragma unroll
    for (int i = 0; i < MF; ++i)
#pragma unroll
      for (int j = 0; j < NF; ++j) {
        __builtin_amdgcn_raw_buffer_store_b128(__builtin_bit_cast(u32x4, acc[i][j]), srsrc, ((i * NF + j) * NT + tid) * 16, 0, 16);
      }
  }
  asm volatile("s_waitcnt vmcnt(0)" ::: "memory");
  __syncthreads();
  if (tid == 0) *lds_word = __hip_atomic_fetch_add(p.counters + tile, 1, __ATOMIC_RELAXED, __HIP_MEMORY_SCOPE_AGENT);
  __syncthreads();
  const int ticket = *reinterpret_cast<volatile int*>(lds_word);
  if (ticket != p.split_k - 1) return false;
  if (tid == 0) {
    __hip_atomic_store(p.counters + tile, 0, __ATOMIC_RELAXED, __HIP_MEMORY_SCOPE_AGENT);
    __builtin_amdgcn_fence(__ATOMIC_ACQUIRE, "agent");
    asm volatile("s_waitcnt vmcnt(0)" ::: "memory");
  }
  __syncthreads();
#pragma unroll
  for (int i = 0; i < MF; ++i)
#pragma unroll
    for (int j = 0; j < NF; ++j) acc[i][j] = (f32x4){0.f, 0.f, 0.f, 0.f};
  for (int z = 0; z < p.split_k; ++z) {
    const float4* src = slab + (int64_t)z * (PER * NT);
    float4 t[MF][NF];
#pragma unroll
    for (int i = 0; i < MF; ++i)
#pragma unroll
      for (int j = 0; j < NF; ++j) t[i][j] = src[(i * NF + j) * NT + tid];
#pragma unroll
    for (int i = 0; i < MF; ++i)
#pragma unroll
      for (int j = 0; j < NF; ++j) {
        acc[i][j][0] += t[i][j].x; acc[i][j][1] += t[i][j].y; acc[i][j][2] += t[i][j].z; acc[i][j][3] += t[i][j].w;
      }
  }
  return true;
}

__device__ __forceinline__ void prefetch_next(const KParams& p, int tid, int nt, unsigned* scratch) {
  if (!p.pf_ptr) return;
  const int xcd = blockIdx.x & 7;
  aptp_prefetch_slice(p.pf_ptr, p.pf_bytes, xcd, blockIdx.x >> 3, ((int)gridDim.x + 7 - xcd) >> 3, tid, nt, scratch);
}

template <int NW, int MF, int NF, int WTM, int WTN, int WN>
__device__ __forceinline__ void run_epilogue(const KParams& p, f32x4 (&acc)[MF][NF], int m0, int n0, int tn, int wm, int wn, int lane,
                                             int wave, const float (&ln_mean)[MF], const float (&ln_rstd)[MF], __bf16* smem) {
  constexpr int PITCH_MAX = WTN + 4;
  constexpr bool POW2 = ((WTN / 8) & (WTN / 8 - 1)) == 0;
  if (p.epi16 && (POW2 || !p.rstat_out)) {
    __syncthreads();
    float* buf = reinterpret_cast<float*>(smem) + wave * 16 * PITCH_MAX;
    if (p.act == APTP_ACT_GEGLU) {
      if constexpr (NF % 2 == 0) tile_epilogue_lds<true, MF, NF, WTM, WTN, WN>(p, acc, m0, n0, tn, wm, wn, lane, ln_mean, ln_rstd, buf);
    } else {
      tile_epilogue_lds<false, MF, NF, WTM, WTN, WN>(p, acc, m0, n0, tn, wm, wn, lane, ln_mean, ln_rstd, buf);
    }
  } else {
    tile_epilogue<MF, NF, WTM, WTN, WN>(p, acc, m0, n0, tn, wm, wn, lane, ln_mean, ln_rstd);
  }
}

inline FastDiv make_fastdiv(int d) {
  FastDiv f;
  if (d <= 1) { f.mul = 0; f.shr = 0; f.one = ~0u; return f; }
  int l = 0;
  while ((1ll << l) < d) ++l;
  const int p = 31 + l;
  f.mul = (unsigned)(((1ull << p) + (unsigned)d - 1) / (unsigned)d);
  f.shr = (unsigned)(p - 32);
  f.one = 0;
  return f;
}

int aptp_sk_cus();
int aptp_launch_sk(const KParams& k, int tile, hipStream_t s);
bool aptp_lin_eligible(const KParams& k, int tile);
int aptp_launch_lin(const KParams& k, int tile, hipStream_t s);
bool aptp_conv_lean_eligible(const KParams& k, int tile);
int aptp_launch_conv_lean(const KParams& k, int tile, hipStream_t s);

}

#include "conv_gemm_tiles.h"
#include "conv_gemm_kloop.h"
```

diffusion_pruning_amd/csrc/conv_gemm_sk.hip:

```cpp
#include "conv_gemm_core.h"

using namespace aptp_cg;

namespace {


struct SkParams {
  int G, T, tiles_m, tiles_n, nK, U;
  int whole;
  FastDiv fd_nk, fd_G, fd_U, fd_tm, fd_tn;
};

__device__ __forceinline__ void wait_vm(int allowed) {
  if (allowed >= 7) asm volatile("s_waitcnt vmcnt(7)" ::: "memory");
  else if (allowed >= 6) asm volatile("s_waitcnt vmcnt(6)" ::: "memory");
  else if (allowed >= 3) asm volatile("s_waitcnt vmcnt(3)" ::: "memory");
  else asm volatile("s_waitcnt vmcnt(0)" ::: "memory");
}

__device__ __forceinline__ void wait_tile(int t, int hidx, int cnt_h0, int cnt_h1) {
  const int newer = hidx - (2 * t + 2);
  wait_vm(newer <= 0 ? 0 : ((newer + 1) >> 1) * cnt_h0 + (newer >> 1) * cnt_h1);
}

// ... 258 lines not shown
        slot_barrier();
        cur = nxt;
      }
    } else {
      for (int tt = 0; tt < n; ++tt) {
        read_frags(cur, 0, af0, wf0);
        issue_half();
        slot_barrier();
        __builtin_amdgcn_s_setprio(1);
        mfmas(af0, wf0);
        __builtin_amdgcn_s_setprio(0);
        slot_barrier();
        read_frags(cur, 1, af0, wf0);
        issue_half();
        if (grp == 1) wait_tile(tt + 1, hidx, cnt_h0, cnt_h1);
        slot_barrier();
        __builtin_amdgcn_s_setprio(1);
        mfmas(af0, wf0);
        __builtin_amdgcn_s_setprio(0);
        if (grp == 0) wait_tile(tt + 1, hidx, cnt_h0, cnt_h1);
        slot_barrier();
        cur = cur + 1 == S ? 0 : cur + 1;
      }
    }
    if (grp == 0) slot_barrier();

    bool emit = true;
    if (n != sk.nK) emit = sk_combine<NT, MF, NF>(p, sk, acc, tile, g, tid, reinterpret_cast<int*>(smem));
    if (emit) {
      float ln_mean[MF], ln_rstd[MF];
#pragma unroll
      for (int i = 0; i < MF; ++i) { ln_mean[i] = 0.f; ln_rstd[i] = 1.f; }
      LnRaw<MF> ln_raw;
      ln_rows_issue<MF, WTM>(p, m0, wm, lane, ln_raw, true);
      ln_rows_finish<MF>(p, lane, ln_raw, ln_mean, ln_rstd, true);
      run_epilogue<NW, MF, NF, WTM, WTN, WN>(p, acc, m0, n0, tn, wm, wn, lane, wave, ln_mean, ln_rstd, smem);
    }
    __syncthreads();
    u += n;
  }
}

int g_sk_cus = 0;

template <int BM, int BN, int WM, int WN, bool RDC>
int launch_sk(const KParams& k, hipStream_t s) {
  SkParams sk;
  sk.tiles_m = (k.M + BM - 1) / BM; sk.tiles_n = (k.N + BN - 1) / BN;
  sk.T = sk.tiles_m * sk.tiles_n; sk.nK = k.nK;
  const int64_t U = (int64_t)sk.T * sk.nK;
  const int cus = aptp_sk_cus();
  sk.whole = k.split_k > 1 ? 0 : 1;
  const int64_t units = sk.whole ? sk.T : U;
  sk.G = (int)(units < cus ? units : cus);
  APTP_CHECK(U * (sk.G + 1) < (1ll << 31) && sk.T <= 65536, "conv_gemm: stream-K work list too large (%d tiles x %d K-steps)", sk.T, sk.nK);
  sk.U = (int)U;
  APTP_CHECK(sk.whole || (k.ws && k.counters), "conv_gemm: the stream-K tiles with split_k > 1 need workspace and tile_counters");
  sk.fd_nk = make_fastdiv(sk.nK); sk.fd_G = make_fastdiv(sk.G); sk.fd_U = make_fastdiv(sk.U);
  sk.fd_tm = make_fastdiv(sk.tiles_m); sk.fd_tn = make_fastdiv(sk.tiles_n);
  hipLaunchKernelGGL((conv_gemm_sk_kernel<BM, BN, WM, WN, RDC>), dim3(sk.G), dim3(512), 0, s, k, sk);
  return APTP_OK;
}

}

namespace aptp_cg {

int aptp_sk_cus() {
  if (g_sk_cus == 0) {
    int dev = 0, n = 0;
    if (hipGetDevice(&dev) != hipSuccess || hipDeviceGetAttribute(&n, hipDeviceAttributeMultiprocessorCount, dev) != hipSuccess || n <= 0) n = 256;
    g_sk_cus = n;
  }
  return g_sk_cus;
}

template <TileFamily F, int BM, int BN, int WM, int WN>
static int launch_sk_row(const KParams& k, int tile, hipStream_t s) {
  if constexpr (F == TileFamily::SK || F == TileFamily::SKL) return launch_sk<BM, BN, WM, WN, F == TileFamily::SK>(k, s);
  aptp_set_error("conv_gemm: unknown stream-K tile %d", tile); return APTP_EINVAL;
}

int aptp_launch_sk(const KParams& k, int tile, hipStream_t s) {
  switch (tile) {
#define X(NAME, FAMILY, BM, BN, WM, WN, STAGES, KU, KS, LIN, C3) \
    case APTP_TILE_##NAME: return launch_sk_row<TileFamily::FAMILY, BM, BN, WM, WN>(k, tile, s);
    APTP_CONV_GEMM_TILES(X)
#undef X
  }
  return launch_sk_row<TileFamily::NONE, 0, 0, 0, 0>(k, tile, s);
}

}
```

diffusion_pruning_amd/csrc/conv_lean.hip:

```cpp
#include "conv_gemm_core.h"

namespace {
using namespace aptp_cg;

constexpr unsigned ZERO_OFF = 0x80000000u;
constexpr int NTAB = 10;

__device__ __forceinline__ void dma16(__amdgpu_buffer_rsrc_t r, __bf16* lds, unsigned voff, int soff) {
#if defined(__HIP_DEVICE_COMPILE__)
  __builtin_amdgcn_raw_ptr_buffer_load_lds(r, (lds_ptr)lds, 16, voff, soff, 0, 0);
#endif
}

template <int BM, int BN, int WM, int WN, int STAGES, bool PP, int KU>
__global__ __launch_bounds__(WM * WN * 64) void conv_lean_kernel(const KParams p) {
  constexpr int NW = WM * WN, NT = NW * 64, RPP = NT / 8;
  constexpr int WTM = BM / WM, WTN = BN / WN, MF = WTM / 16, NF = WTN / 16;
  constexpr int A_PASS = BM / RPP, B_PASS = (BN + RPP - 1) / RPP;
  constexpr int B_FULL = BN / RPP, NLD_LO = A_PASS + B_FULL, NLD_HI = A_PASS + B_PASS;
  static_assert(NW == 4 || NW == 8, "4 or 8 waves");
  static_assert(BM % RPP == 0 && WTM % 16 == 0 && WTN % 16 == 0 && BN % 8 == 0, "tile shape");
  static_assert(NW * 16 * (WTN + 4) * 4 <= STAGES * (BM + BN) * BK * 2, "epilogue transpose buffer");

  __shared__ __attribute__((aligned(16))) __bf16 smem[STAGES * (BM + BN) * BK];
  __shared__ unsigned pf_scratch[64];
  __bf16* As = smem;
  __bf16* Bs = smem + STAGES * BM * BK;

  const int tid = threadIdx.x, lane = tid & 63;
  const int wave = __builtin_amdgcn_readfirstlane(tid >> 6);
  const int wm = wave / WN, wn = wave % WN;
  const int tiles_n = (p.N + BN - 1) / BN, tiles_m = (p.M + BM - 1) / BM;
  int tm, tn, kz;
  decode_block(p, tiles_m, tiles_n, tm, tn, kz);
  const int m0 = tm * BM, n0 = tn * BN;
  const int kt_begin = p.fd_sk.div(p.nK * kz);
  const int kt_end = p.fd_sk.div(p.nK * (kz + 1));

  prefetch_hosted(p, tid, NT, pf_scratch);

  const int rowbase = tid >> 3;
  const unsigned schunk = (unsigned)((tid & 7) ^ ((rowbase >> 1) & 7));
  unsigned tab[A_PASS][NTAB];
#pragma unroll
  for (int i = 0; i < A_PASS; ++i) {
    const int m = m0 + rowbase + RPP * i;
    if (m < p.M) {
      const int b = p.fd_hw.div(m), rem = m - b * p.HW;
      const int oy = p.fd_wout.div(rem), ox = rem - oy * p.Wout;
      const int iy0 = oy * p.stride - 1, ix0 = ox * p.stride - 1, pix0 = b * p.Hin * p.Win;
#pragma unroll
      for (int t = 0; t < 9; ++t) {
        int iy = iy0 + t / 3, ix = ix0 + t % 3;
        const bool ok = (unsigned)iy < (unsigned)p.HinE && (unsigned)ix < (unsigned)p.WinE && !(p.zins & (iy | ix));
        iy >>= p.ups; ix >>= p.ups;
        tab[i][t] = ok ? ((unsigned)(pix0 + iy * p.Win + ix) * (unsigned)p.ldx) * 2u + schunk * 16u : ZERO_OFF;
      }
      tab[i][9] = p.x2 ? ((unsigned)m * (unsigned)p.ldx2) * 2u + schunk * 16u : ZERO_OFF;
    } else {
#pragma unroll
      for (int t = 0; t < NTAB; ++t) tab[i][t] = ZERO_OFF;
    }
  }
  unsigned boff[B_PASS];
#pragma unroll
  for (int i = 0; i < B_PASS; ++i) {
    int n = n0 + rowbase + RPP * i;
    n = n < p.N ? n : p.N - 1;
    boff[i] = (unsigned)(n * (unsigned)p.Ktot) * 2u + schunk * 16u;
  }
  const bool tail_bad = (int)((p.ncc - 1) * BK + schunk * 8) >= p.Cin;
  const bool tail_bad2 = (int)((p.ncc2 - 1) * BK + schunk * 8) >= p.Cin2;
  const __amdgpu_buffer_rsrc_t xr = __builtin_amdgcn_make_buffer_rsrc(const_cast<__bf16*>(p.x), 0, p.x_bytes, 0x00020000);
  const __amdgpu_buffer_rsrc_t x2r =
      __builtin_amdgcn_make_buffer_rsrc(const_cast<__bf16*>(p.x2 ? p.x2 : p.x), 0, p.x2 ? p.x2_bytes : 0, 0x00020000);
  const __amdgpu_buffer_rsrc_t wr = __builtin_amdgcn_make_buffer_rsrc(const_cast<__bf16*>(p.w), 0, p.w_bytes, 0x00020000);

  int l_kt = kt_begin, l_tap = 0, l_cc = kt_begin;
  if (kt_begin != 0) {
    l_tap = kt_begin / p.ncc;
    if (l_tap > 9) l_tap = 9;
    l_cc = kt_begin - l_tap * p.ncc;
  }
  auto next_tap = [&]() {
#pragma unroll
    for (int i = 0; i < A_PASS; ++i)
#pragma unroll
      for (int t = 0; t + 1 < NTAB; ++t) tab[i][t] = tab[i][t + 1];
  };
  for (int t = 0; t < l_tap; ++t) next_tap();

  auto issue_tile = [&](int stage) {
    const bool seg2 = l_tap == 9;
    const int ncur = seg2 ? p.ncc2 : p.ncc;
    const bool pad = l_cc == ncur - 1 && (seg2 ? tail_bad2 : tail_bad);
    const int sa = __builtin_amdgcn_readfirstlane(l_cc * (BK * 2));
    const int sb = __builtin_amdgcn_readfirstlane(l_kt * (BK * 2));
#pragma unroll
    for (int i = 0; i < A_PASS; ++i) {
      __bf16* dst = As + (stage * BM + wave * 8 + RPP * i) * BK;
      if (seg2) dma16(x2r, dst, pad ? ZERO_OFF : tab[i][0], sa);
      else dma16(xr, dst, pad ? ZERO_OFF : tab[i][0], sa);
    }
#pragma unroll
    for (int i = 0; i < B_PASS; ++i) {
      if (wave * 8 + RPP * i < BN) {
        __bf16* dst = Bs + (stage * BN + wave * 8 + RPP * i) * BK;
        dma16(wr, dst, boff[i], sb);
      }
    }
    ++l_kt;
    if (++l_cc == ncur) {
      l_cc = 0;
      if (l_tap < 9) {
        ++l_tap;
        next_tap();
      }
    }
  };

  f32x4 acc[MF][NF];
  zero_acc(acc);
  const int frow = lane & 15, fq = lane >> 4;
  auto compute = [&](int stage) {
#pragma unroll
    for (int s = 0; s < 2; ++s) {
      bf16x8 af[MF], wf[NF];
#pragma unroll
      for (int i = 0; i < MF; ++i) {
        const int r = wm * WTM + i * 16 + frow;
        af[i] = *reinterpret_cast<const bf16x8*>(As + (stage * BM + r) * BK + ((s * 4 + fq) ^ ((r >> 1) & 7)) * 8);
      }
#pragma unroll
      for (int j = 0; j < NF; ++j) {
        const int r = wn * WTN + j * 16 + frow;
        wf[j] = *reinterpret_cast<const bf16x8*>(Bs + (stage * BN + r) * BK + ((s * 4 + fq) ^ ((r >> 1) & 7)) * 8);
      }
#pragma unroll
      for (int i = 0; i < MF; ++i)
#pragma unroll
        for (int j = 0; j < NF; ++j) acc[i][j] = __builtin_amdgcn_mfma_f32_16x16x32_bf16(wf[j], af[i], acc[i][j], 0, 0, 0);
    }
  };

  constexpr int D = PP ? STAGES - 2 : (KU == 2 ? STAGES - 2 : STAGES - 1);
  constexpr int DW = KU == 2 ? D - 2 : D - 1;
  static_assert(STAGES >= 2 && D >= 1, "ring");
  static_assert(!PP || NW == 8, "ping-pong: 8 waves");
  static_assert(KU == 1 || !PP, "two K-tiles per barrier: ring schedule only");
  const bool hi = (NLD_HI != NLD_LO) && (wave * 8 + RPP * (B_PASS - 1) < BN);
  auto wait_ring = [&](bool full) { ring_wait<NLD_LO, NLD_HI, DW>(hi, full); };
  const int n = kt_end - kt_begin;
  const int pre = n < D ? n : D;
  for (int t = 0; t < pre; ++t) issue_tile(t);
  LeanEpiIn<WTM, WTN> ein;
  if (p.split_k == 1) lean_epi_load<WTM, WTN>(p, m0, n0, wm, wn, lane, ein);

  if (n > 0) {
    wait_ring(pre == D);
    __builtin_amdgcn_s_barrier();
    asm volatile("" ::: "memory");
    if constexpr (PP) kloop_pp<STAGES, D>(n, wave >> 2, issue_tile, compute, wait_ring);
    else if constexpr (KU == 2) kloop_ku2<STAGES, D>(n, issue_tile, compute, wait_ring);
    else kloop_ring<STAGES, D>(n, issue_tile, compute, wait_ring);
  }

  if (p.split_k > 1 && p.counters) {
    if (!splitk_combine<NT, MF, NF>(p, acc, tm * tiles_n + tn, kz, tid, reinterpret_cast<int*>(smem))) return;
    lean_epi_load<WTM, WTN>(p, m0, n0, wm, wn, lane, ein);
  } else if (p.split_k > 1) {
    store_splitk_slab(p, acc, kz, m0 + wm * WTM, n0 + wn * WTN, frow, fq);
    return;
  }
  __syncthreads();
  lean_epilogue<MF, NF, WTM, WTN>(p, acc, m0, n0, wm, wn, lane, ein, reinterpret_cast<float*>(smem) + wave * 16 * (WTN + 4));
}

template <int BM, int BN, int WM, int WN, int STAGES, bool PP, int KU>
void launch_lean(KParams k, hipStream_t s) {
  const int grid = ((k.M + BM - 1) / BM) * ((k.N + BN - 1) / BN) * k.split_k;
  set_prefetch_slices(k, grid);
  hipLaunchKernelGGL((conv_lean_kernel<BM, BN, WM, WN, STAGES, PP, KU>), dim3(grid), dim3(WM * WN * 64), 0, s, k);
}

}

namespace aptp_cg {

bool aptp_conv_lean_eligible(const KParams& k, int tile) {
  if (k.KH != 3 || k.KW != 3 || k.pad != 1 || (k.stride != 1 && k.stride != 2)) return false;
  if (k.io_f32 || k.out_f32 || !k.epi16 || k.ln_stats || k.rstat_out || k.depth) return false;
  if (k.act != APTP_ACT_NONE && k.act != APTP_ACT_SILU) return false;
  if (k.Nout < 8 || k.ncc < 1) return false;
  return tile_known(tile) && kTiles[tile].c3;
}

template <bool C3, int BM, int BN, int WM, int WN, int STAGES, bool PP, int KU>
static bool launch_lean_row(const KParams& k, hipStream_t s) {
  if constexpr (C3) launch_lean<BM, BN, WM, WN, STAGES, PP, KU>(k, s);
  return C3;
}

int aptp_launch_conv_lean(const KParams& k, int tile, hipStream_t s) {
  switch (tile) {
#define X(NAME, FAMILY, BM, BN, WM, WN, STAGES, KU, KS, LIN, C3) case APTP_TILE_##NAME: \
    if (launch_lean_row<C3 != 0, BM, BN, WM, WN, STAGES, TileFamily::FAMILY == TileFamily::PP, KU>(k, s)) return APTP_OK; break;
    APTP_CONV_GEMM_TILES(X)
#undef X
  }
  aptp_set_error("conv_lean: tile %d has no lean instantiation", tile); return APTP_EINVAL;
}

}
```

diffusion_pruning_amd/launch_policy.py:

```python
import json
import math
import os
import re

from . import _lib as L

BK = 64
DMA_TILE_FIRST = L.TILE_DMA_128x128
DMA_MAX_CHANNELS = 4032
SK_TILE_FIRST = L.TILE_SK_256x160
SK_MAX_CHANNELS = 32704
_HALO_TILES = (L.TILE_HALO_128x160, L.TILE_HALO_128x128)
_LEAN_TILES = frozenset(getattr(L, "TILE_" + t) for t in (
    "DMA_64x128 DMA_128x64 DMA_64x64 DMA3_64x128 DMA3_128x64 DMA3_64x64 DMA4_64x128 DMA4_64x64 DMA4_128x64 DMA6_64x64 DMA8S_64x64 "
    "DMA6_64x128 DMA6_128x64 KU2S4_64x64 KU2S6_64x64 KU2S4_64x128 KU2S6_64x128 KU2S4_128x64").split())

TUNING_NEAREST = os.environ.get("APTP_TUNING_NEAREST", "1") != "0"
TUNING_MAX_DIST = 2.0
LEAN_REMAP = os.environ.get("APTP_LEAN_REMAP", "1") != "0"
SK_AUTO = os.environ.get("APTP_SK_AUTO", "1") == "1"
SK_AUTO_MIN_OUTPUTS = 256 * 256 * 160
SK_AUTO_MIN_KSTEPS = 16
SPLITK_FORCE_IN_KERNEL = os.environ.get("APTP_SPLITK_FORCE_INKERNEL", "0") == "1"
COLS_SPLIT_MAX = int(os.environ.get("APTP_COLS_SPLIT_MAX", "2"))

_KEY = re.compile(r"M(\d+)_N(\d+)_C(\d+)_T(\d+)_s(\d+)u(\d+)g(\d+)(?:x(\d+))?$")


def tuning_key(M, N, Cin, taps, stride, ups, geglu, Cin2: int = 0) -> str:
    return f"M{M}_N{N}_C{Cin}_T{taps}_s{stride}u{ups}g{int(bool(geglu))}" + (f"x{Cin2}" if Cin2 else "")


def parse_key(key: str):
    m = _KEY.match(key)
    return m and tuple(int(t) if t else 0 for t in m.groups())


def key_of(p) -> str:
    return tuning_key(p.B * p.Hout * p.Wout, p.N, p.Cin, p.KH * p.KW, p.stride, p.ups, p.act == L.ACT_GEGLU, p.Cin2 if p.x2 else 0)


_path = os.environ.get("APTP_TUNING") or os.path.join(os.path.dirname(os.path.abspath(__file__)), "tuning_gfx950.json")
TUNING = {}
if os.path.exists(_path):
    with open(_path) as _f:
        TUNING.update(json.load(_f))
_classes = None
_near = {}


def invalidate():
    global _classes
    _classes = None
    _near.clear()


def set_tuning(table):
    table = dict(table)
    TUNING.clear()
    TUNING.update(table)
    invalidate()


def set_entry(key: str, entry):
    if entry is None:
        TUNING.pop(key, None)
    else:
        TUNING[key] = entry
    invalidate()


def _nearest(key, M, N, Cin, taps, stride, ups, geglu, Cin2):
    global _classes
    if key in _near:
        return _near[key]
    if _classes is None:
        _classes = {}
        for k, v in TUNING.items():
            s = parse_key(k)
            if s is not None:
                _classes.setdefault((s[3], s[4], s[5], s[6], s[7] > 0), []).append((s[0], s[1], s[3] * s[2] + s[7], v))
    K = taps * Cin + Cin2
    best, bd = None, TUNING_MAX_DIST
    for (M2, N2, K2, v) in _classes.get((taps, stride, ups, int(bool(geglu)), Cin2 > 0), ()):
        if v["tile"] in _HALO_TILES and M2 != M:
            continue
        if v["tile"] >= DMA_TILE_FIRST and max(Cin, Cin2) > DMA_MAX_CHANNELS:
            continue
        dm = math.log2(M / M2)
        d = (0.5 * dm if dm > 0 else -1.5 * dm) + abs(math.log2(N / N2)) + abs(math.log2(K / K2))
        if d < bd:
            best, bd = v, d
    if best is not None:
        nK = (K + BK - 1) // BK
        best = dict(best)
        best["split_k"] = max(1, min(int(best["split_k"]), nK // 4 if nK >= 8 else 1))
    _near[key] = best
    return best


def tuning_lookup(M, N, Cin, taps, stride, ups, geglu, Cin2: int = 0):
    key = tuning_key(M, N, Cin, taps, stride, ups, geglu, Cin2)
    hit = TUNING.get(key)
    if hit is None and TUNING_NEAREST:
        hit = _nearest(key, M, N, Cin, taps, stride, ups, geglu, Cin2)
    return hit


def _lean_tile(M):
    return L.TILE_DMA_128x64 if M >= 8192 else (L.TILE_DMA3_64x64 if M >= 2048 else L.TILE_KU2S4_64x64)


def choose_launch(M, N, Cin, cin_pad, KH, KW, stride, ups, act, Cin2, cin2_pad, *, plain_linear, f32, tile, split_k, order):
    if split_k is not None or tile != 0 or f32:
        return tile, split_k, None, order
    taps, geglu = KH * KW, act == L.ACT_GEGLU
    channels = max(cin_pad, cin2_pad)
    sk_sized = SK_AUTO and M * N >= SK_AUTO_MIN_OUTPUTS and taps * (cin_pad // BK) + cin2_pad // BK >= SK_AUTO_MIN_KSTEPS
    lean = LEAN_REMAP and plain_linear and cin_pad <= DMA_MAX_CHANNELS
    key = tuning_key(M, N, Cin, taps, stride, ups, geglu, Cin2)
    tuned = TUNING.get(key)
    if tuned is None and TUNING_NEAREST:
        tuned = _nearest(key, M, N, Cin, taps, stride, ups, geglu, Cin2)
        if tuned is not None and sk_sized:
            tuned = None
    if tuned is not None and tuned["tile"] >= DMA_TILE_FIRST \
            and channels > (SK_MAX_CHANNELS if tuned["tile"] >= SK_TILE_FIRST else DMA_MAX_CHANNELS):
        tuned = None
    if tuned is not None:
        tile = tuned["tile"]
        if lean and tile not in _LEAN_TILES and tuned["split_k"] == 1 and "insitu" not in tuned:
            tile = _lean_tile(M)
        return tile, tuned["split_k"], bool(tuned.get("in_kernel", 0)), order or tuned.get("order", 1)
    if lean and not (M <= 512 and cin_pad >= 1280):
        return _lean_tile(M), 1, None, order
    if sk_sized and channels <= SK_MAX_CHANNELS:
        return (L.TILE_SK_256x128 if geglu else L.TILE_SK_256x160), 2, True, order or 3
    return 0, None, None, order


def splitk_in_kernel(split_k, in_kernel, *, explicit, reduce_launch, rowstats, colstats) -> bool:
    if reduce_launch:
        return False
    if SPLITK_FORCE_IN_KERNEL:
        return True
    if in_kernel is None:
        in_kernel = split_k <= 4 or explicit
    return in_kernel or rowstats or (colstats and split_k <= COLS_SPLIT_MAX)
```

diffusion_pruning_amd/ops.py:

```python
from __future__ import annotations

import ctypes
import os
import threading
from dataclasses import dataclass
from typing import Optional

import torch

from . import _lib, scratch
from ._lib import ImageInParams, LatentDistParams, UnetEpilogueParams, UnetPrologueParams
from ._lib import ACT_GELU, AttentionCausalParams, TokenEmbedParams
from ._lib import AttentionBiasParams, EmbedLnParams, MaskedMeanParams
from ._lib import ACT_QUICK_GELU, ImagePatchesParams, L2NormalizeParams, MmdRbfParams, VitEmbedLnParams
from ._lib import EOS_ARGMAX, EOS_FIRST, EosPoolLnParams, ImagePatchesPilParams, PairedCosineParams
from ._lib import GuidedStepParams, LossStageParams, LossTermsParams, PhiloxNormalParams, TrainNoiseParams
from ._lib import (ACT_GEGLU, ACT_NONE, ACT_SILU, AttentionBwdParams, AttentionParams, ConvGemmParams, DepthLerpParams, GateBwdParams, WgradParams, FfTailParams, FoldRowsParams, PackDgradParams, MseParams,
                   GegluParams, GroupNormBwdParams, GroupNormParams, LayerNormBwdParams, LayerNormParams,
                   ColsumParams, LayerNormPgradParams, AttentionWideParams, ImageOutParams)
from .launch_policy import (BK, SK_AUTO, SK_TILE_FIRST, TUNING, _HALO_TILES, choose_launch, key_of, parse_key,
                            set_entry, set_tuning, splitk_in_kernel, tuning_key, tuning_lookup)

ACT_DTYPE = torch.bfloat16


def _stream() -> int:
    return torch.cuda.current_stream().cuda_stream


def _ptr(t: Optional[torch.Tensor]):
    return None if t is None else ctypes.c_void_p(t.data_ptr())


def _check_act(x: torch.Tensor, name: str):
    if x.dtype not in (torch.bfloat16, torch.float32) or x.dim() != 4 or x.stride(3) != 1 or not x.is_cuda:
        raise ValueError(f"{name}: expected a CUDA bf16 (or, parity path, fp32) [B,H,W,C] tensor with contiguous channels, got "
                         f"{x.dtype} {tuple(x.shape)} strides {x.stride()}")
    B, H, W, C = x.shape
    ld = _ld(x)
    if (W > 1 and x.stride(2) != ld) or (H > 1 and x.stride(1) != W * ld) or (B > 1 and x.stride(0) != H * W * ld):
        raise ValueError(f"{name}: rows must be uniformly strided (ld={ld}), got strides {x.stride()}")
    if ld % 8 != 0 or x.data_ptr() % 16 != 0:
        raise ValueError(f"{name}: pixel stride {ld} must be a multiple of 8 elements and the base 16-byte aligned")
    return ld


def _ld(x: torch.Tensor) -> int:
    B, H, W, C = x.shape
    if W > 1:
        return x.stride(2)
    if H > 1:
        return x.stride(1)
    if B > 1:
        return x.stride(0)
    return max(x.stride(2), C)


def _set_views(p, **views):
    for name, t in views.items():
        setattr(p, name, t.data_ptr())
        setattr(p, name + "_stride_b", t.stride(0))
        setattr(p, name + "_stride_l", t.stride(1))


@dataclass
class PackedWeight:
    w: torch.Tensor
    bias: Optional[torch.Tensor]
    N: int
    Cin: int
    KH: int
    KW: int
    geglu: bool = False
    ln_colsum: Optional[torch.Tensor] = None
    Cin2: int = 0
    cin2_pad: int = 0
    cin_pad_: int = 0

    @property
    def cin_pad(self) -> int:
        return self.cin_pad_ or self.w.shape[2]


def round_up(v: int, m: int) -> int:
    return (v + m - 1) // m * m


def pack_weight(w: torch.Tensor, bias: Optional[torch.Tensor] = None, *, out_idx: Optional[torch.Tensor] = None,
                in_idx: Optional[torch.Tensor] = None, n_pad_to: int = 8, cin_pad_to: int = 8,
                geglu: bool = False, device=None, ln_gamma: Optional[torch.Tensor] = None,
                ln_beta: Optional[torch.Tensor] = None) -> PackedWeight:
    if w.dim() == 2:
        w = w[:, :, None, None]
    device = device or w.device
    w = w.to(device=device, dtype=torch.float32)
    if bias is not None:
        bias = bias.to(device=device, dtype=torch.float32)
    if ln_gamma is not None:
        assert w.shape[2] == 1 and w.shape[3] == 1 and in_idx is None, "a LayerNorm folds into a linear layer over all its channels"
        ga = ln_gamma.to(device=device, dtype=torch.float32)
        be = ln_beta.to(device=device, dtype=torch.float32)
        shift = w[:, :, 0, 0] @ be
        bias = shift if bias is None else bias + shift
        w = w * ga[None, :, None, None]
    if geglu:
        inner = w.shape[0] // 2
        wh, wg = w[:inner], w[inner:]
        bh, bg = (bias[:inner], bias[inner:]) if bias is not None else (None, None)
        if out_idx is not None:
            out_idx = out_idx.to(device)
            wh, wg = wh[out_idx], wg[out_idx]
            if bias is not None:
                bh, bg = bh[out_idx], bg[out_idx]
        if in_idx is not None:
            in_idx = in_idx.to(device)
            wh, wg = wh[:, in_idx], wg[:, in_idx]
        n_live = wh.shape[0]
        n_p = round_up(n_live, 16)

        def padrows(t):
            if t.shape[0] == n_p:
                return t
            return torch.cat([t, t.new_zeros((n_p - t.shape[0],) + tuple(t.shape[1:]))], 0)
        wh, wg = padrows(wh), padrows(wg)
        w = torch.stack([wh.reshape(n_p // 16, 16, *wh.shape[1:]), wg.reshape(n_p // 16, 16, *wg.shape[1:])], 1)
        w = w.reshape(2 * n_p, *wh.shape[1:])
        if bias is not None:
            bh, bg = padrows(bh), padrows(bg)
            bias = torch.stack([bh.reshape(n_p // 16, 16), bg.reshape(n_p // 16, 16)], 1).reshape(2 * n_p)
    else:
        if out_idx is not None:
            out_idx = out_idx.to(device)
            w = w[out_idx]
            if bias is not None:
                bias = bias[out_idx]
        if in_idx is not None:
            w = w[:, in_idx.to(device)]
        n_live = w.shape[0]
        n_p = round_up(n_live, n_pad_to)
        if n_p != n_live:
            w = torch.cat([w, w.new_zeros((n_p - n_live,) + tuple(w.shape[1:]))], 0)
            if bias is not None:
                bias = torch.cat([bias, bias.new_zeros(n_p - n_live)], 0)
    N, Cin, KH, KW = w.shape
    cin_live = round_up(Cin, cin_pad_to)
    cin_pad = round_up(cin_live, BK)
    packed = torch.zeros(N, KH * KW, cin_pad, dtype=ACT_DTYPE, device=device)
    packed[:, :, :Cin] = w.permute(0, 2, 3, 1).reshape(N, KH * KW, Cin).to(ACT_DTYPE)
    colsum = packed.float().sum(dim=(1, 2)).contiguous() if ln_gamma is not None else None
    return PackedWeight(packed.contiguous(), None if bias is None else bias.contiguous(), N, cin_live, KH, KW, geglu, colsum)


def pack_weight_cat(pw: PackedWeight, w2: torch.Tensor, bias2: Optional[torch.Tensor] = None, *,
                    in_idx: Optional[torch.Tensor] = None) -> PackedWeight:
    assert not pw.geglu and pw.ln_colsum is None and pw.Cin2 == 0
    dev = pw.w.device
    w2 = w2.to(device=dev, dtype=torch.float32).reshape(w2.shape[0], -1)
    if in_idx is not None:
        w2 = w2[:, in_idx.to(dev)]
    n_live, c2 = w2.shape
    assert n_live <= pw.N
    c2_live = round_up(c2, 8)
    c2_pad = round_up(c2_live, BK)
    ext = torch.zeros(pw.N, c2_pad, dtype=ACT_DTYPE, device=dev)
    ext[:n_live, :c2] = w2.to(ACT_DTYPE)
    flat = torch.cat([pw.w.reshape(pw.N, -1), ext], 1).reshape(pw.N, 1, -1).contiguous()
    bias = pw.bias
    if bias2 is not None:
        b2 = torch.zeros(pw.N, dtype=torch.float32, device=dev)
        b2[:n_live] = bias2.to(device=dev, dtype=torch.float32)
        bias = b2 if bias is None else bias + b2
    return PackedWeight(flat, bias, pw.N, pw.Cin, pw.KH, pw.KW, False, None, c2_live, c2_pad, pw.cin_pad)


LAUNCH_LOG = None
GN_LAUNCH_LOG = None
ATTN_LAUNCH_LOG = None

SPLITK_IN_KERNEL = True

scratch_domain, _domain = scratch.scratch_domain, scratch.domain
_tile_counters, _N_COUNTERS = scratch.counters, scratch.N_COUNTERS
_workspace, _ws_capture_keep = scratch.workspace, scratch.capture_keep
ustat_begin, ustat_end, _ustat_alloc = scratch.ustat_begin, scratch.ustat_end, scratch.ustat_alloc
USTAT, USTAT_NREP = scratch.USTAT, scratch.USTAT_NREP

GN_DEFAULT_VARIANT = 0
GN_STATS_ONE_LAUNCH = True

ATTN_VARIANT = int(os.environ.get("APTP_ATTN_VARIANT", "0"))

GN_FUSED_FINALIZE = False

EPILOGUE = 0


COLSTATS = True
COLSTATS_MIN_HW = 1024


def _root(t: torch.Tensor) -> torch.Tensor:
    return t._base if t._base is not None else t


def _colstats_drop(out: torch.Tensor):
    d = getattr(_root(out), "_aptp_colstats", None)
    if d:
        d.pop(out.storage_offset(), None)


def _colstats_put(out: torch.Tensor, stats: torch.Tensor, rows_per_block: int, ustat=None):
    root = _root(out)
    d = getattr(root, "_aptp_colstats", None)
    if d is None:
        d = {}
        root._aptp_colstats = d
    d[out.storage_offset()] = (stats, rows_per_block, out.shape[3], (out.shape[0], out.shape[1] * out.shape[2]), _ld(out), ustat)


def _colstats_get(x: torch.Tensor, C: int):
    d = getattr(_root(x), "_aptp_colstats", None)
    if not d:
        return None
    segs, off, left, pad = [], x.storage_offset(), x.shape[3], x.shape[3] - C
    while left > 0 and len(segs) < 2:
        rec = d.get(off)
        if rec is None or rec[3] != (x.shape[0], x.shape[1] * x.shape[2]) or rec[4] != _ld(x) or rec[2] > left:
            return None
        segs.append([rec[0], rec[1], rec[2], rec[5] if len(rec) > 5 else None])
        off += rec[2]
        left -= rec[2]
    if left != 0 or segs[-1][2] <= pad:
        return None
# ... 4 lines not shown
class _PrefetchPlan:

    def __init__(self):
        self.seq = []
        self.i = 0

    def begin(self):
        self.i = 0

    def step(self, w):
        i, self.i = self.i, self.i + 1
        if i < len(self.seq) and self.seq[i] is w:
            nxt = self.seq[i + 1] if i + 1 < len(self.seq) else None
        else:
            del self.seq[i:]
            self.seq.append(w)
            nxt = None
        if nxt is not None and not (PREFETCH_MIN_BYTES <= nxt.numel() * nxt.element_size() <= PREFETCH_MAX_BYTES):
            return None
        return nxt


_tls = threading.local()


def set_prefetch_plan(plan: Optional[_PrefetchPlan]):
    _tls.prefetch_plan = plan
    if plan is not None:
        plan.begin()


def _current_prefetch_plan() -> Optional[_PrefetchPlan]:
    return getattr(_tls, "prefetch_plan", None)


PREFETCH_WEIGHTS = os.environ.get("APTP_PREFETCH", "1") == "1"
PREFETCH_MIN_BYTES = int(os.environ.get("APTP_PREFETCH_MIN", "0"))
PREFETCH_MAX_BYTES = int(os.environ.get("APTP_PREFETCH_MAX", str(12 << 20)))


def conv_gemm(x: torch.Tensor, pw: PackedWeight, *, stride: int = 1, pad: Optional[int] = None, ups: int = 0,
              out: Optional[torch.Tensor] = None, rowbias: Optional[torch.Tensor] = None,
              colgate: Optional[torch.Tensor] = None, gate_group: int = 0, act: int = ACT_NONE,
              corr: Optional[torch.Tensor] = None, residual: Optional[torch.Tensor] = None,
              depth: Optional[torch.Tensor] = None, depth_in: Optional[torch.Tensor] = None,
              out_f32: bool = False, split_k: Optional[int] = None, tile: int = 0, order: int = 0,
              rowstats: bool = False, ln=None, colstats: bool = False, x2: Optional[torch.Tensor] = None,
              prefetch=None, gn=None, pad_end: int = 0):
    if pad_end < 0 or (pad_end and (ups or corr is not None or x2 is not None)):
        raise ValueError("conv_gemm: pad_end must be >= 0 and does not go with ups, corr or x2")
    lib = _lib.load()
    if gn is not None and (colgate is not None or act != ACT_NONE or pw.geglu or corr is not None or residual is not None
                           or depth is not None or out_f32 or rowstats or ln is not None or out is not None):
        raise ValueError("conv_gemm: gn= goes with a plain bf16 convolution (bias / rowbias only)")
    _check_act(x, "conv_gemm x")
    B, Hin, Win, Cx = x.shape
    if Cx != pw.Cin:
        raise ValueError(f"conv_gemm: x has {Cx} channels, packed weight expects {pw.Cin}")
    if pad is None:
        pad = pw.KH // 2
    sh = 1 if ups else 0
    HinE, WinE = Hin << sh, Win << sh
    Hout = (HinE + 2 * pad + pad_end - pw.KH) // stride + 1
    Wout = (WinE + 2 * pad + pad_end - pw.KW) // stride + 1
    if pw.geglu:
        act = ACT_GEGLU
    nout = pw.N // 2 if act == ACT_GEGLU else pw.N
    f32 = x.dtype == torch.float32
    gn_f32 = None
    if f32:
        if pw.w.dtype != torch.float32:
            raise ValueError("conv_gemm: fp32 activations need weights packed under ops.ACT_DTYPE = torch.float32")
        out_f32, colstats, prefetch, gn_f32, gn = True, False, False, gn, None
        if tile not in (0, 1, 2, 3, 4, 5, 6):
            raise ValueError("conv_gemm: the fp32 parity path runs on the register-staged tiles 1..6")
    if out is None:
        out = torch.empty(B, Hout, Wout, nout, dtype=torch.float32 if out_f32 else torch.bfloat16, device=x.device)
    else:
        _colstats_drop(out)
        if tuple(out.shape) != (B, Hout, Wout, nout) or out.stride(3) != 1:
            raise ValueError(f"conv_gemm: out shape {tuple(out.shape)} != {(B, Hout, Wout, nout)}")
        if out.dtype != (torch.float32 if out_f32 else torch.bfloat16):
            raise ValueError("conv_gemm: out dtype mismatch")
    p = ConvGemmParams()
    p.x, p.ldx = x.data_ptr(), _ld(x)
    p.B, p.Hin, p.Win, p.Cin, p.Hout, p.Wout = B, Hin, Win, Cx, Hout, Wout
    p.KH, p.KW, p.stride, p.pad, p.ups = pw.KH, pw.KW, stride, pad, ups
    p.pad_end = pad_end
    p.w, p.N, p.cin_pad = pw.w.data_ptr(), pw.N, pw.cin_pad
    if (x2 is not None) != (pw.Cin2 > 0):
        raise ValueError("conv_gemm: x2 goes with weights packed by pack_weight_cat (and only with them)")
    if x2 is not None:
        _check_act(x2, "conv_gemm x2")
        if tuple(x2.shape) != (B, Hout, Wout, pw.Cin2):
            raise ValueError(f"conv_gemm: x2 shape {tuple(x2.shape)} != {(B, Hout, Wout, pw.Cin2)}")
        p.x2, p.ldx2, p.Cin2, p.cin2_pad = x2.data_ptr(), _ld(x2), pw.Cin2, pw.cin2_pad
    p.bias = None if pw.bias is None else pw.bias.data_ptr()
    if rowbias is not None:
        assert rowbias.dtype == torch.float32 and rowbias.dim() == 2 and rowbias.shape[0] == B and rowbias.stride(1) == 1
        assert rowbias.shape[1] >= pw.N
        p.rowbias, p.ld_rowbias = rowbias.data_ptr(), rowbias.stride(0)
    if colgate is not None:
        assert colgate.dtype == torch.float32 and colgate.dim() == 2 and colgate.is_contiguous()
        assert gate_group > 0 and colgate.shape[1] * gate_group == nout and B % colgate.shape[0] == 0
        p.colgate, p.gate_group, p.gate_B = colgate.data_ptr(), gate_group, colgate.shape[0]
    p.act = act
    if corr is not None:
        assert corr.dtype == torch.float32 and corr.is_contiguous() and corr.shape[1:] == (9, nout)
        assert B % corr.shape[0] == 0
        p.corr, p.corr_B = corr.data_ptr(), corr.shape[0]
    if residual is not None:
        _check_act(residual, "conv_gemm residual")
        assert tuple(residual.shape) == (B, Hout, Wout, nout)
        p.residual, p.ldres = residual.data_ptr(), _ld(residual)
    if depth is not None:
        assert depth.dtype == torch.float32 and depth.dim() == 1 and B % depth.shape[0] == 0 and depth_in is not None
        _check_act(depth_in, "conv_gemm depth_in")
        assert tuple(depth_in.shape) == (B, Hout, Wout, nout)
        p.depth, p.depth_B = depth.data_ptr(), depth.shape[0]
        p.depth_in, p.lddin = depth_in.data_ptr(), _ld(depth_in)
    p.y, p.ldy, p.out_f32 = out.data_ptr(), _ld(out), int(out_f32)
    p.epilogue = EPILOGUE
    p.io_f32 = int(f32)
    if f32:
        for t_, nm in ((x2, "x2"), (residual, "residual"), (depth_in, "depth_in")):
            if t_ is not None and t_.dtype != torch.float32:
                raise ValueError(f"conv_gemm: fp32 parity path: {nm} must be fp32 too")
    if prefetch is False:
        prefetch = None
    elif PREFETCH_WEIGHTS and prefetch is None:
        plan = _current_prefetch_plan()
        if plan is not None:
            prefetch = plan.step(pw.w)
    if prefetch is not None:
        p.prefetch, p.prefetch_bytes = prefetch.data_ptr(), prefetch.numel() * prefetch.element_size()
    plain_linear = pw.KH == 1 and pw.KW == 1 and stride == 1 and not ups and x2 is None and colgate is None and corr is None \
        and rowbias is None and depth is None and not out_f32 and gn is None and (act != ACT_GEGLU or (residual is None and not rowstats))
    p.split_k = 1
    p.tile, sk, in_kernel, p.order = choose_launch(B * Hout * Wout, pw.N, Cx, pw.cin_pad, pw.KH, pw.KW, stride, ups, act, pw.Cin2, pw.cin2_pad,
                                                   plain_linear=plain_linear, f32=f32, tile=tile, split_k=split_k, order=order)
    p.split_k = max(1, int(lib.aptp_conv_gemm_suggest_split_k(ctypes.byref(p)) if sk is None else sk))
    ws = cnt = None
    gn_fused = False
    if gn is not None and FUSE_GN_REDUCE and p.split_k > 1 and Hout * Wout <= GN_REDUCE_MAX_HW:
        gamma, beta, groups, eps_, silu_, Cn = gn
        cgn = Cn // groups
        gn_fused = Cn % 8 == 0 and Cn % groups == 0 and cgn % 4 == 0 and Hout * Wout * cgn <= 4 * 24 * 256 and Cn <= nout
    if gn_fused:
        colstats = False
        p.gn_gamma, p.gn_beta, p.gn_groups, p.gn_C, p.gn_silu, p.gn_eps = gamma.data_ptr(), beta.data_ptr(), groups, Cn, int(silu_), eps_
    want_cols = colstats and COLSTATS and Hout * Wout >= COLSTATS_MIN_HW and act != ACT_GEGLU and not out_f32
    if p.split_k > 1:
        in_kernel = splitk_in_kernel(p.split_k, in_kernel, explicit=split_k is not None, reduce_launch=gn_fused, rowstats=rowstats, colstats=want_cols)
        sk_tile = p.tile >= SK_TILE_FIRST
        if (SPLITK_IN_KERNEL or sk_tile) and (in_kernel or sk_tile) and lib.aptp_conv_gemm_tiles(ctypes.byref(p)) <= _N_COUNTERS:
            cnt = _tile_counters(x.device)
            if cnt is not None:
                p.tile_counters = cnt.data_ptr()
        if sk_tile and cnt is None:
            p.split_k = 1
        else:
            ws = _workspace(lib.aptp_conv_gemm_workspace_bytes(ctypes.byref(p)), x.device)
            p.workspace = ws.data_ptr()
    stats = None
    if rowstats and (p.split_k == 1 or cnt is not None):
        slots = lib.aptp_conv_gemm_rowstat_slots(ctypes.byref(p))
        assert slots % 2 == 0
        stats = torch.empty(slots // 2, B * Hout * Wout, 4, dtype=torch.float32, device=x.device)
        p.rowstat_out, p.rowstat_slots = stats.data_ptr(), slots
    cstats = ustat = None
    if want_cols and (p.split_k == 1 or cnt is not None) and _ld(out) % 8 == 0 and out.data_ptr() % 16 == 0 and nout % 8 == 0 \
            and (residual is None or (_ld(residual) % 8 == 0 and residual.data_ptr() % 16 == 0)) \
            and (depth_in is None or (_ld(depth_in) % 8 == 0 and depth_in.data_ptr() % 16 == 0)) and p.epilogue == 0:
        rpb = lib.aptp_conv_gemm_colstat_rows(ctypes.byref(p))
        if rpb > 0 and (Hout * Wout) % rpb == 0:
            M = B * Hout * Wout
            nblk = (M + rpb - 1) // rpb + 16
            cstats = torch.empty(nblk, nout, 2, dtype=torch.float32, device=x.device)
            p.colstat_out, p.colstat_ld = cstats.data_ptr(), nout
            ustat = _ustat_alloc(B, nout)
            if ustat is not None:
                p.ustat_out, p.ustat_unit, p.ustat_units, p.ustat_nrep = ustat[0].data_ptr(), ustat[1], ustat[2], ustat[3]
    if ln is not None:
        ln_stats, ln_eps = ln
        if pw.ln_colsum is None:
            raise ValueError("conv_gemm: ln= needs weights packed with ln_gamma / ln_beta")
        assert ln_stats.dtype == torch.float32 and ln_stats.is_contiguous() and ln_stats.shape[1] == B * Hout * Wout \
            and ln_stats.shape[2] == 4
        p.ln_stats, p.ln_slots, p.ln_colsum = ln_stats.data_ptr(), 2 * ln_stats.shape[0], pw.ln_colsum.data_ptr()
        p.ln_eps, p.ln_C = ln_eps, Cx
    elif pw.ln_colsum is not None:
        raise ValueError("conv_gemm: weights with a folded LayerNorm need ln=(stats, eps)")
    _lib.check(lib.aptp_conv_gemm(ctypes.byref(p), _stream()), "aptp_conv_gemm")
    if cstats is not None:
        _colstats_put(out, cstats, rpb, ustat)
    if LAUNCH_LOG is not None:
        LAUNCH_LOG.append({"params": p, "flops": 2.0 * B * Hout * Wout * pw.N * (pw.KH * pw.KW * pw.Cin + pw.Cin2),
                           "keep": (x, pw, out, rowbias, colgate, corr, residual, depth, depth_in, ws, stats, ln, cnt, cstats, x2, gn, ustat)})
    if f32 and gn_f32 is not None:
        gn = gn_f32
    if gn is not None and not gn_fused:
        gamma, beta, groups, eps_, silu_, Cn = gn
        return groupnorm(out, gamma, beta, groups, eps_, silu_, C=Cn)
    return (out, stats) if rowstats else out


def linear(x: torch.Tensor, pw: PackedWeight, **kw) -> torch.Tensor:
    B, L, C = x.shape
    out = kw.pop("out", None)
    for k in ("residual", "depth_in"):
        if kw.get(k) is not None:
            kw[k] = kw[k].unsqueeze(2)
    y = conv_gemm(x.unsqueeze(2), pw, pad=0, out=None if out is None else out.unsqueeze(2), **kw)
    if "rowstats" in kw:
        return (y[0].squeeze(2), y[1]) if kw["rowstats"] else (y.squeeze(2), None)
    return y.squeeze(2)


def groupnorm(x: torch.Tensor, gamma: torch.Tensor, beta: torch.Tensor, groups: int, eps: float, silu: bool,
              C: Optional[int] = None, out: Optional[torch.Tensor] = None, keep_stats: bool = False, variant: int = 0):
    lib = _lib.load()
    _check_act(x, "groupnorm x")
    B, H, W, Cp = x.shape
# ... 1908 lines not shown
```

diffusion_pruning_amd/unet.py:

```python
from __future__ import annotations

import os

import math
from dataclasses import dataclass, field
from typing import Any, Dict, List, Optional, Tuple, Union

import torch
import torch.nn as nn

from . import ops
from .gates import DepthGate, LinearWidthGate, WidthGate
from .modules import LinearP, PlannedModule, _capturing, _Params, _PlanCache, _versions
from .ops import PackedWeight



class Conv2dP(_Params):
    def __init__(self, cin, cout, k):
        super().__init__()
        self.in_channels, self.out_channels, self.kernel_size = cin, cout, (k, k)
        self.weight = nn.Parameter(torch.empty(cout, cin, k, k))
        self.bias = nn.Parameter(torch.empty(cout))


class NormP(_Params):
    def __init__(self, c, eps, groups=None):
        super().__init__()
        self.num_channels, self.eps, self.num_groups = c, eps, groups
        self.weight = nn.Parameter(torch.empty(c))
        self.bias = nn.Parameter(torch.empty(c))


def _nhwc(x: torch.Tensor) -> torch.Tensor:
    return x.permute(0, 2, 3, 1)


def _nchw(x: torch.Tensor) -> torch.Tensor:
    return x.permute(0, 3, 1, 2)


def _f32(t: torch.Tensor) -> torch.Tensor:
    return t.detach().float().contiguous()


@dataclass
class TembBundle:
    emb_silu: torch.Tensor
    proj: Dict[int, torch.Tensor] = field(default_factory=dict)


@dataclass
class CtxBundle:
    ehs: torch.Tensor
    kv: Dict[int, torch.Tensor] = field(default_factory=dict)
    key: Any = None


def _live_index(mask: torch.Tensor, group: int) -> torch.Tensor:
    g = torch.nonzero(mask > 0.5).flatten()
    return (g[:, None] * group + torch.arange(group)[None, :]).flatten()


class _CatSlot:

    def __init__(self, c_hidden: int, c_skip: int):
        self.ch, self.cs, self.buf = c_hidden, c_skip, None

    def view(self, which: int, B: int, H: int, W: int, C: int, device) -> Optional[torch.Tensor]:
        if C != (self.ch if which == 0 else self.cs):
            return None
        if self.buf is None:
            self.buf = torch.empty(B, H, W, self.ch + self.cs, dtype=ops.ACT_DTYPE, device=device)
        elif tuple(self.buf.shape[:3]) != (B, H, W) or self.buf.device != device:
            return None
        return self.buf[..., :self.ch] if which == 0 else self.buf[..., self.ch:]


def _ft_mode(mod) -> bool:
    return torch.is_grad_enabled() or mod.__dict__.get("_pk") is not None


def _take_dst(mod, B: int, H: int, W: int, C: int, device) -> Optional[torch.Tensor]:
    d = mod.__dict__.pop("_out_dst", None)
    if d is None or _ft_mode(mod):
        return None
    return d[0].view(d[1], B, H, W, C, device)
# ... 699 lines not shown
            pw = pl[name + "_ln"] = pl[name + "_ln_make"]()
        return ops.linear(h, pw, ln=(st, 1e-5), **kw)

    @staticmethod
    def _ret(t, return_dict):
        if not return_dict:
            return (t,)
        return Transformer2DModelOutput(sample=t)

    def _ctx_kv(self, ehs, pl, tb, dev):
        if isinstance(ehs, CtxBundle):
            kv = ehs.kv.get(id(tb.attn2))
            if kv is not None:
                return kv
            ehs_t = ehs.ehs
        else:
            ehs_t = ehs.to(device=dev, dtype=ops.ACT_DTYPE)
        pw = pl.get("a2_kv")
        if pw is None:
            pw = ops.pack_weight(pl["a2_kv_w"], None, device=dev)
            pl["a2_kv"] = pw
        gkw = {}
        if pl["a2_dense_gate"]:
            gkw = dict(colgate=self._gate(tb.attn2.gate, dev, 2), gate_group=64)
        return ops.linear(ehs_t, pw, **gkw)


class Transformer2DModelWidthDepthGated(Transformer2DModelWidthGated):
    depth_gated = True

    def __init__(self, *args, **kwargs):
        super().__init__(*args, **kwargs)
        self.depth_gate = DepthGate(1)

    def _depth_state(self):
        h = self.depth_gate.host_value().flatten()
        if bool(((h == 0) | (h == 1)).all()) and bool((h == h[0]).all()):
            return float(h[0]), None
        return None, self.depth_gate.gate_f.detach().flatten().to(dtype=torch.float32)


@dataclass
class Transformer2DModelOutput:
    sample: torch.Tensor


@dataclass
class UNet2DConditionOutput:
    sample: torch.Tensor


class _Resample2D(PlannedModule):
    conv_kw: dict = {}

    def __init__(self, channels: int):
        super().__init__()
        self.conv = Conv2dP(channels, channels, 3)
        self._plans = _PlanCache(cap=1)

    def plan(self, device) -> dict:
        return self._plans.lookup(str(device), _versions(self), lambda: {
            "pw": ops.pack_weight(self.conv.weight.detach(), self.conv.bias.detach(), device=device)})

    def _out_hw(self, H: int, W: int) -> Tuple[int, int]:
        raise NotImplementedError

    def _resample(self, hidden_states):
        x = _nhwc(hidden_states)
        if _ft_mode(self):
            self.__dict__.pop("_out_dst", None)
        pl = self.plan(x.device)
        pw = pl["pw"]

        def get_bwd():
            if "pwb" not in pl:
                pl["pwb"] = ops.pack_weight_dgrad(self.conv.weight.detach(), device=x.device)
            return pl["pwb"]
        if _ft_mode(self) and self.conv.weight.requires_grad:
            return _nchw(_cw(self, x, self.conv.weight, self.conv.bias, pw, get_bwd, **self.conv_kw))
        if torch.is_grad_enabled() and x.requires_grad:
            from . import autograd as AG
            return _nchw(AG.conv(x, pw, get_bwd, **self.conv_kw))
        dst = _take_dst(self, x.shape[0], *self._out_hw(x.shape[1], x.shape[2]), pw.N, x.device)
        return _nchw(ops.conv_gemm(x, pw, out=dst, colstats=True, **self.conv_kw))


class Downsample2D(_Resample2D):
    conv_kw = {"stride": 2, "pad": 1}

    def _out_hw(self, H, W):
        return (H - 1) // 2 + 1, (W - 1) // 2 + 1

    def forward(self, hidden_states, scale: float = 1.0):
        return self._resample(hidden_states)


class Upsample2D(_Resample2D):
    conv_kw = {"ups": 1}

    def _out_hw(self, H, W):
        return 2 * H, 2 * W

    def forward(self, hidden_states, output_size=None, scale: float = 1.0):
        return self._resample(hidden_states)


class _GatedContainer(nn.Module):
    has_cross_attention = True

    def _init_common(self):
        self.structure = {"width": [], "depth": []}
        self.total_macs, self.prunable_macs = 0.0, 0.0

    def get_gate_structure(self):
        if len(self.structure["width"]) == 0:
            structure = {"width": [], "depth": []}
            for b in list(self.resnets) + list(self.attentions):
                s = b.get_gate_structure()
                structure["width"].append(s["width"])
                structure["depth"].append(s["depth"])
            self.structure = structure
        return self.structure

    def set_gate_structure(self, arch_vectors):
        width_vectors, depth_vectors = arch_vectors["width"], arch_vectors["depth"]
        for b in list(self.resnets) + list(self.attentions):
            s = b.get_gate_structure()
            block_vectors = {"width": [], "depth": []}
            for i in range(len(s["width"])):
                assert s["width"][i] == width_vectors[0].shape[1]
                block_vectors["width"].append(width_vectors.pop(0))
            for i in range(len(s["depth"])):
                if s["depth"][i] == 1:
                    block_vectors["depth"].append(depth_vectors.pop(0))
            b.set_gate_structure(block_vectors)


def _make_resnet(cin, cout, temb, depth_gated, groups, eps, concat=False, skip_dim=None):
    cls = ResnetBlock2DWidthDepthGated if depth_gated else ResnetBlock2DWidthGated
    return cls(in_channels=cin, out_channels=cout, temb_channels=temb, groups=groups, eps=eps,
               is_input_concatenated=concat, skip_connection_dim=skip_dim)


def _make_attn(ch, heads, xdim, depth_gated, groups, gated_ff, ff_gate_width):
    cls = Transformer2DModelWidthDepthGated if depth_gated else Transformer2DModelWidthGated
    return cls(heads, ch // heads, in_channels=ch, cross_attention_dim=xdim, norm_num_groups=groups,
               gated_ff=gated_ff, ff_gate_width=ff_gate_width)


class CrossAttnDownBlock2DWidthHalfDepthGated(_GatedContainer):
    def __init__(self, in_channels, out_channels, temb_channels, num_layers, num_attention_heads, cross_attention_dim,
                 add_downsample, resnet_groups=32, resnet_eps=1e-5, gated_ff=True, ff_gate_width=32, with_attention=True):
        super().__init__()
        self.has_cross_attention = with_attention
        resnets, attentions = [], []
        for i in range(num_layers):
            last = i == num_layers - 1
            resnets.append(_make_resnet(in_channels if i == 0 else out_channels, out_channels, temb_channels, last,
                                        resnet_groups, resnet_eps))
            if with_attention:
                attentions.append(_make_attn(out_channels, num_attention_heads, cross_attention_dim, last,
                                             resnet_groups, gated_ff, ff_gate_width))
        self.attentions = nn.ModuleList(attentions)
        self.resnets = nn.ModuleList(resnets)
        self.downsamplers = nn.ModuleList([Downsample2D(out_channels)]) if add_downsample else None
        self._init_common()

    def forward(self, hidden_states, temb=None, encoder_hidden_states=None, attention_mask=None,
                cross_attention_kwargs=None, encoder_attention_mask=None, scale: float = 1.0):
        output_states = ()
        for i, resnet in enumerate(self.resnets):
            hidden_states = resnet(hidden_states, temb)
            if self.has_cross_attention:
                hidden_states = self.attentions[i](hidden_states, encoder_hidden_states=encoder_hidden_states,
                                                   return_dict=False)[0]
            output_states = output_states + (hidden_states,)
        if self.downsamplers is not None:
            for d in self.downsamplers:
                hidden_states = d(hidden_states)
            output_states = output_states + (hidden_states,)
        return hidden_states, output_states
# ... 614 lines not shown
```

Baseline: 206.6 steps/s.

## Lower nearest-upsample + 3x3 conv to four 2x2 phase convolutions

Adds a phase-decomposition path for Upsample2D: the 3x3 conv over a 2x nearest-upsampled input is rewritten as four 2x2 convolutions on the original-resolution input, using pre-folded weights per output phase. Kernels gain a PHASE template that maps GEMM rows to (batch, phase, y, x), selects the per-phase weight slab, and scatters outputs to interleaved positions. This cuts the MACs per upsampler conv from 9 taps to 4 and avoids reading the virtually upsampled input. In exchange it stores a four-phase weight pack and needs tiles whose rows divide Hin*Win, and the epilogue writes are strided.

```diff
diff --git a/diffusion_pruning_amd/csrc/conv_gemm.hip b/diffusion_pruning_amd/csrc/conv_gemm.hip
--- a/diffusion_pruning_amd/csrc/conv_gemm.hip
+++ b/diffusion_pruning_amd/csrc/conv_gemm.hip
@@ -8,7 +8,7 @@
 template <> struct Elem<__bf16> { static constexpr int EPC = 8, KS = 64; };
 template <> struct Elem<float> { static constexpr int EPC = 4, KS = 32; };
 
-template <int BM, int BN, int WM, int WN, typename T = __bf16>
+template <int BM, int BN, int WM, int WN, typename T = __bf16, bool PHASE = false>
 __global__ __launch_bounds__(256) void conv_gemm_kernel(const KParams p) {
   static_assert(WM * WN == 4, "4 waves per workgroup");
   constexpr int EPC = Elem<T>::EPC, KS = Elem<T>::KS, ES = (int)sizeof(T);
@@ -35,7 +35,8 @@
   ln_rows_issue<MF, WTM>(p, m0, wm, lane, ln_raw);
 
   const __amdgpu_buffer_rsrc_t xsrc = __builtin_amdgcn_make_buffer_rsrc(const_cast<__bf16*>(p.x), 0, p.x_bytes, 0x00020000);
-  const __amdgpu_buffer_rsrc_t wsrc = __builtin_amdgcn_make_buffer_rsrc(const_cast<__bf16*>(p.w), 0, p.w_bytes, 0x00020000);
+  const char* const wtile = reinterpret_cast<const char*>(p.w) + (PHASE ? phase_w_offset(p, m0) * ES : 0);
+  const __amdgpu_buffer_rsrc_t wsrc = __builtin_amdgcn_make_buffer_rsrc(const_cast<char*>(wtile), 0, p.w_bytes, 0x00020000);
   const __amdgpu_buffer_rsrc_t x2src = __builtin_amdgcn_make_buffer_rsrc(const_cast<__bf16*>(p.x2 ? p.x2 : p.x), 0, p.x2 ? p.x2_bytes : 0, 0x00020000);
   constexpr unsigned OOB = 0x80000000u;
   const int chunk = tid & 7, rowbase = tid >> 3;
@@ -44,10 +45,15 @@
   for (int i = 0; i < A_PASS; ++i) {
     const int m = m0 + rowbase + 32 * i;
     if (m < p.M) {
-      const int b = p.fd_hw.div(m), rem = m - b * p.HW;
-      const int oy = p.fd_wout.div(rem), ox = rem - oy * p.Wout;
-      a_iy0[i] = oy * p.stride - p.pad;
-      a_ix0[i] = ox * p.stride - p.pad;
+      int b;
+      if constexpr (PHASE) gather_origin(p, m, b, a_iy0[i], a_ix0[i]);
+      else {
+        b = p.fd_hw.div(m);
+        const int rem = m - b * p.HW;
+        const int oy = p.fd_wout.div(rem), ox = rem - oy * p.Wout;
+        a_iy0[i] = oy * p.stride - p.pad;
+        a_ix0[i] = ox * p.stride - p.pad;
+      }
       a_pix0[i] = b * p.Hin * p.Win;
       a_m[i] = m;
     } else {
@@ -217,12 +223,12 @@
     }
     return;
   }
-  run_epilogue<4, MF, NF, WTM, WTN, WN>(p, acc, m0, n0, tn, wm, wn, lane, wave, ln_mean, ln_rstd, reinterpret_cast<__bf16*>(smem));
+  run_epilogue<4, MF, NF, WTM, WTN, WN, PHASE>(p, acc, m0, n0, tn, wm, wn, lane, wave, ln_mean, ln_rstd, reinterpret_cast<__bf16*>(smem));
 }
 
 __device__ uint4 g_zero_page[512];
 
-template <int BM, int BN, int WM, int WN, int STAGES, bool PP = false, int KU = 1, int KS = 1>
+template <int BM, int BN, int WM, int WN, int STAGES, bool PP = false, int KU = 1, int KS = 1, bool PHASE = false>
 __global__ __launch_bounds__(WM * WN * KS * 64) void conv_gemm_dma_kernel(const KParams p) {
   constexpr int NW = WM * WN;
   constexpr int NWA = NW * KS;
@@ -267,10 +273,15 @@
   for (int i = 0; i < A_PASS; ++i) {
     const int m = m0 + rowbase + RPP * i;
     if (m < p.M && rowbase + RPP * i < BM) {
-      const int b = p.fd_hw.div(m), rem = m - b * p.HW;
-      const int oy = p.fd_wout.div(rem), ox = rem - oy * p.Wout;
-      a_iy0[i] = oy * p.stride - p.pad;
-      a_ix0[i] = ox * p.stride - p.pad;
+      int b;
+      if constexpr (PHASE) gather_origin(p, m, b, a_iy0[i], a_ix0[i]);
+      else {
+        b = p.fd_hw.div(m);
+        const int rem = m - b * p.HW;
+        const int oy = p.fd_wout.div(rem), ox = rem - oy * p.Wout;
+        a_iy0[i] = oy * p.stride - p.pad;
+        a_ix0[i] = ox * p.stride - p.pad;
+      }
       a_pix0[i] = b * p.Hin * p.Win;
       a_m[i] = m;
     } else {
@@ -315,7 +326,7 @@
   for (int i = 0; i < B_PASS; ++i) {
     int n = n0 + rowbase + RPP * i;
     n = n < p.N ? n : p.N - 1;
-    b_ptr[i] = reinterpret_cast<const char*>(p.w) + ((int64_t)n * p.Ktot + (int64_t)kt_begin * BK + schunk * 8) * 2;
+    b_ptr[i] = reinterpret_cast<const char*>(p.w) + ((PHASE ? phase_w_offset(p, m0) : 0) + (int64_t)n * p.Ktot + (int64_t)kt_begin * BK + schunk * 8) * 2;
   }
   set_tap(l_cc);
 
@@ -442,7 +453,7 @@
   }
   static_assert(NW * 16 * (WTN + 4) * 4 <= (int)sizeof(smem), "epilogue transpose buffer");
   static_assert(KS == 1 || NW * MF * NF * 64 * 16 <= (int)sizeof(smem), "accumulator hand-over buffer");
-  run_epilogue<NW, MF, NF, WTM, WTN, WN>(p, acc, m0, n0, tn, wm, wn, lane, cw, ln_mean, ln_rstd, smem);
+  run_epilogue<NW, MF, NF, WTM, WTN, WN, PHASE>(p, acc, m0, n0, tn, wm, wn, lane, cw, ln_mean, ln_rstd, smem);
 }
 
 template <int BN, int STAGES>
@@ -624,6 +635,7 @@
   run_epilogue<NW, MF, NF, WTM, WTN, WN>(p, acc, m0, n0, tn, wm, wn, lane, wave, ln_mean, ln_rstd, smem);
 }
 
+template <bool PHASE = false>
 __global__ __launch_bounds__(256) void splitk_reduce_kernel(const KParams p) {
   const int quads = (p.act == APTP_ACT_GEGLU) ? p.N / 8 : p.N / 4;
   const int64_t idx = (int64_t)blockIdx.x * blockDim.x + threadIdx.x;
@@ -660,8 +672,8 @@
     ln_finish(p, a, a2, rc);
   }
   float st[2] = {0.f, 0.f};
-  if (p.act == APTP_ACT_GEGLU) epilogue_quad<true>(p, m, rc, n, h, g, st);
-  else epilogue_quad<false>(p, m, rc, n, h, h, st);
+  if (p.act == APTP_ACT_GEGLU) epilogue_quad<true, PHASE>(p, m, rc, n, h, g, st);
+  else epilogue_quad<false, PHASE>(p, m, rc, n, h, h, st);
 }
 
 constexpr int GN_RED_NT = 1024;
@@ -768,7 +780,7 @@
   APTP_CHECK(p->ldx % 8 == 0 && p->ldx >= p->Cin, "conv_gemm: ldx (%lld) must be a multiple of 8 and >= Cin", (long long)p->ldx);
   APTP_CHECK(p->N > 0 && p->N % 8 == 0, "conv_gemm: N (%d) must be a positive multiple of 8", p->N);
   APTP_CHECK(p->cin_pad % BK == 0 && p->cin_pad >= p->Cin && p->cin_pad < p->Cin + BK, "conv_gemm: cin_pad (%d) != ceil(Cin/64)*64", p->cin_pad);
-  APTP_CHECK(p->KH >= 1 && p->KW >= 1 && p->stride >= 1 && p->pad >= 0 && p->ups >= 0 && p->ups <= 2, "conv_gemm: bad filter geometry");
+  APTP_CHECK(p->KH >= 1 && p->KW >= 1 && p->stride >= 1 && p->pad >= 0 && p->ups >= 0 && p->ups <= 3, "conv_gemm: bad filter geometry");
   APTP_CHECK(((uintptr_t)p->x % 16) == 0 && ((uintptr_t)p->w % 16) == 0 && ((uintptr_t)p->y % 8) == 0, "conv_gemm: pointer alignment");
   APTP_CHECK((p->act >= APTP_ACT_NONE && p->act <= APTP_ACT_GELU) || p->act == APTP_ACT_QUICK_GELU, "conv_gemm: unknown act %d", p->act);
   const int geglu = p->act == APTP_ACT_GEGLU;
@@ -783,10 +795,19 @@
   APTP_CHECK(p->split_k >= 1, "conv_gemm: split_k >= 1");
   const int64_t M64 = (int64_t)p->B * p->Hout * p->Wout;
   APTP_CHECK(M64 < (1ll << 31), "conv_gemm: M too large");
-  const int sh = p->ups ? 1 : 0;
+  const bool phase = p->ups == 3;
+  const int sh = (p->ups == 1 || p->ups == 2) ? 1 : 0;
   const int HinE = p->Hin << sh, WinE = p->Win << sh;
   APTP_CHECK(p->pad_end >= 0, "conv_gemm: pad_end (%d) must be >= 0", p->pad_end);
   APTP_CHECK(p->pad_end == 0 || (!p->corr && !p->x2 && p->ups == 0), "conv_gemm: pad_end > 0 does not go with corr, x2 or ups");
+  if (phase) {
+    APTP_CHECK(p->KH == 2 && p->KW == 2 && p->stride == 1 && p->pad == 1 && p->Hout == 2 * p->Hin && p->Wout == 2 * p->Win,
+               "conv_gemm: ups = 3 (phase convolutions) needs KH = KW = 2, stride 1, pad 1, Hout = 2 Hin and Wout = 2 Win");
+    APTP_CHECK(!p->x2 && !p->corr && !p->residual && !p->rowbias && !p->colgate && !p->depth && !geglu && !p->ln_stats &&
+               !p->rowstat_out && !p->gn_gamma && p->pad_end == 0,
+               "conv_gemm: ups = 3 goes with bias, activation and column statistics only (no x2, corr, residual, rowbias, colgate, "
+               "depth, GEGLU, ln, rowstats, gn or pad_end)");
+  } else
   APTP_CHECK(p->Hout == (HinE + 2 * p->pad + p->pad_end - p->KH) / p->stride + 1 &&
              p->Wout == (WinE + 2 * p->pad + p->pad_end - p->KW) / p->stride + 1,
              "conv_gemm: Hout/Wout inconsistent with input extent, filter, stride and padding");
@@ -794,6 +815,7 @@
   k.B = p->B; k.Hin = p->Hin; k.Win = p->Win; k.Cin = p->Cin; k.Hout = p->Hout; k.Wout = p->Wout;
   k.KH = p->KH; k.KW = p->KW; k.stride = p->stride; k.pad = p->pad; k.ups = sh; k.zins = p->ups == 2 ? 1 : 0;
   k.HinE = HinE; k.WinE = WinE;
+  k.phase = phase ? 1 : 0; k.HWin = p->Hin * p->Win;
   const int f32 = p->io_f32 ? 1 : 0, es = f32 ? 4 : 2, ks = f32 ? 32 : BK;
   APTP_CHECK(!f32 || (p->out_f32 && !p->colstat_out && !p->gn_gamma && !p->prefetch),
              "conv_gemm: io_f32 (fp32 parity path) writes fp32 and has no column statistics / fused GroupNorm / prefetch");
@@ -852,6 +874,7 @@
   const int64_t xb = (((int64_t)p->B * p->Hin * p->Win - 1) * p->ldx + p->Cin) * es;
   const int64_t wb = (int64_t)p->N * k.Ktot * es;
   APTP_CHECK(xb < (1ll << 31) && wb < (1ll << 31), "conv_gemm: operand larger than 2 GiB");
+  APTP_CHECK(!phase || 4 * wb < (1ll << 31), "conv_gemm: ups = 3: the four-phase weight pack is larger than 2 GiB");
   k.x_bytes = (int)xb; k.w_bytes = (int)wb;
   return APTP_OK;
 }
@@ -860,13 +883,16 @@
 dim3 tile_grid(const KParams& k) { return dim3(((k.M + BM - 1) / BM) * ((k.N + BN - 1) / BN) * k.split_k, 1, 1); }
 template <int BM, int BN, int WM, int WN>
 void launch_tile(const KParams& k, hipStream_t s) {
-  if (k.io_f32) hipLaunchKernelGGL((conv_gemm_kernel<BM, BN, WM, WN, float>), (tile_grid<BM, BN>(k)), dim3(256), 0, s, k);
+  if (k.phase && k.io_f32) hipLaunchKernelGGL((conv_gemm_kernel<BM, BN, WM, WN, float, true>), (tile_grid<BM, BN>(k)), dim3(256), 0, s, k);
+  else if (k.phase) hipLaunchKernelGGL((conv_gemm_kernel<BM, BN, WM, WN, __bf16, true>), (tile_grid<BM, BN>(k)), dim3(256), 0, s, k);
+  else if (k.io_f32) hipLaunchKernelGGL((conv_gemm_kernel<BM, BN, WM, WN, float>), (tile_grid<BM, BN>(k)), dim3(256), 0, s, k);
   else hipLaunchKernelGGL((conv_gemm_kernel<BM, BN, WM, WN>), (tile_grid<BM, BN>(k)), dim3(256), 0, s, k);
 }
 
 template <int BM, int BN, int WM, int WN, int STAGES, bool PP, int KU, int KS>
 void launch_dma(const KParams& k, hipStream_t s) {
-  hipLaunchKernelGGL((conv_gemm_dma_kernel<BM, BN, WM, WN, STAGES, PP, KU, KS>), (tile_grid<BM, BN>(k)), dim3(WM * WN * KS * 64), 0, s, k);
+  if (k.phase) hipLaunchKernelGGL((conv_gemm_dma_kernel<BM, BN, WM, WN, STAGES, PP, KU, KS, true>), (tile_grid<BM, BN>(k)), dim3(WM * WN * KS * 64), 0, s, k);
+  else hipLaunchKernelGGL((conv_gemm_dma_kernel<BM, BN, WM, WN, STAGES, PP, KU, KS>), (tile_grid<BM, BN>(k)), dim3(WM * WN * KS * 64), 0, s, k);
 }
 
 template <int BM, int BN, int STAGES>
@@ -969,6 +995,13 @@
     aptp_set_error("conv_gemm: LDS-DMA tiles need Cin <= 4032 (got cin_pad %d)", p->cin_pad);
     return APTP_EINVAL;
   }
+  if (k.phase) {
+    if (k.HWin % kTiles[t].bm != 0 || kTiles[t].family == TileFamily::HALO || is_sk_tile(t)) {
+      aptp_set_error("conv_gemm: ups = 3 needs a tile whose %d rows divide Hin*Win (%d), and no halo / stream-K tile (got tile %d)",
+                     kTiles[t].bm, k.HWin, t);
+      return APTP_EINVAL;
+    }
+  }
   if (k.rstat_out) {
     const int slots = ((k.N + kTiles[t].bn - 1) / kTiles[t].bn) * kTiles[t].wn;
     if ((k.split_k != 1 && !k.counters) || k.rstat_slots != slots) {
@@ -999,6 +1032,7 @@
     const int tiles_m = (k.M + kTiles[t].bm - 1) / kTiles[t].bm, tiles_n = (k.N + kTiles[t].bn - 1) / kTiles[t].bn;
     APTP_CHECK((int64_t)tiles_m * tiles_n * k.split_k < (1ll << 31) && (int64_t)k.nK * (k.split_k + 1) < (1ll << 31), "conv_gemm: grid too large");
     k.fd_hw = make_fastdiv(k.HW); k.fd_wout = make_fastdiv(k.Wout);
+    k.fd_hwin = make_fastdiv(k.HWin); k.fd_win = make_fastdiv(k.Win);
     k.fd_tm = make_fastdiv(tiles_m); k.fd_tn = make_fastdiv(tiles_n); k.fd_sk = make_fastdiv(k.split_k);
     k.fd_perm = make_fastdiv(tiles_n * k.split_k); k.fd_tmn = make_fastdiv(tiles_m * tiles_n);
   }
@@ -1027,7 +1061,8 @@
     } else {
       const int quads = (k.act == APTP_ACT_GEGLU) ? k.N / 8 : k.N / 4;
       const int64_t total = (int64_t)k.M * quads;
-      hipLaunchKernelGGL(splitk_reduce_kernel, dim3((unsigned)((total + 255) / 256)), dim3(256), 0, s, k);
+      if (k.phase) hipLaunchKernelGGL(splitk_reduce_kernel<true>, dim3((unsigned)((total + 255) / 256)), dim3(256), 0, s, k);
+      else hipLaunchKernelGGL(splitk_reduce_kernel<false>, dim3((unsigned)((total + 255) / 256)), dim3(256), 0, s, k);
     }
     APTP_LAUNCH_CHECK();
   }
diff --git a/diffusion_pruning_amd/csrc/conv_gemm_core.h b/diffusion_pruning_amd/csrc/conv_gemm_core.h
--- a/diffusion_pruning_amd/csrc/conv_gemm_core.h
+++ b/diffusion_pruning_amd/csrc/conv_gemm_core.h
@@ -43,6 +43,8 @@
   long long* ustat_out; int ustat_unit, ustat_units, ustat_nrep;
   FastDiv fd_hw, fd_wout;
   FastDiv fd_tm, fd_tn, fd_sk, fd_perm, fd_tmn;
+  int phase, HWin;
+  FastDiv fd_hwin, fd_win;
 };
 
 __device__ __forceinline__ void decode_block(const KParams& p, int tiles_m, int tiles_n, int& tm, int& tn, int& kz) {
@@ -72,6 +74,27 @@
   }
 }
 
+__device__ __forceinline__ void phase_row(const KParams& p, int m, int& b, int& y, int& x, int& py, int& px) {
+  const int q = p.fd_hwin.div(m), rem = m - q * p.HWin;
+  y = p.fd_win.div(rem); x = rem - y * p.Win;
+  b = q >> 2; py = (q >> 1) & 1; px = q & 1;
+}
+__device__ __forceinline__ void gather_origin(const KParams& p, int m, int& b, int& iy0, int& ix0) {
+  int y, x, py, px;
+  phase_row(p, m, b, y, x, py, px);
+  iy0 = y + py - 1; ix0 = x + px - 1;
+}
+__device__ __forceinline__ int64_t phase_w_offset(const KParams& p, int m0) {
+  return (int64_t)(p.fd_hwin.div(m0) & 3) * p.N * p.Ktot;
+}
+template <bool PHASE>
+__device__ __forceinline__ int64_t out_row(const KParams& p, int m) {
+  if constexpr (!PHASE) return m;
+  int b, y, x, py, px;
+  phase_row(p, m, b, y, x, py, px);
+  return (int64_t)b * p.HW + (2 * y + py) * p.Wout + 2 * x + px;
+}
+
 struct RowCtx { int b, cls; float mean, rstd; };
 
 struct ColVecs { float4 cs, cg, bb, bg; };
@@ -140,7 +163,7 @@
   }
 }
 
-template <bool GEGLU>
+template <bool GEGLU, bool PHASE = false>
 __device__ __forceinline__ void epilogue_quad(const KParams& p, int m, const RowCtx& rc, int n, float h[4], float g[4], float st[2]) {
   const int b = rc.b;
   float v[4];
@@ -176,7 +199,7 @@
   }
   if (p.out_f32) {
     float4 o; o.x = v[0]; o.y = v[1]; o.z = v[2]; o.w = v[3];
-    *reinterpret_cast<float4*>(reinterpret_cast<float*>(p.y) + (int64_t)m * p.ldy + c) = o;
+    *reinterpret_cast<float4*>(reinterpret_cast<float*>(p.y) + out_row<PHASE>(p, m) * p.ldy + c) = o;
     if (p.io_f32 && p.rstat_out) {
 #pragma unroll
       for (int r = 0; r < 4; ++r) { st[0] += v[r]; st[1] += v[r] * v[r]; }
@@ -184,7 +207,7 @@
   } else {
     union { uint2 u; __bf16 e[4]; } o;
     o.u.x = pack_bf16x2(v[0], v[1]); o.u.y = pack_bf16x2(v[2], v[3]);
-    *reinterpret_cast<uint2*>(reinterpret_cast<__bf16*>(p.y) + (int64_t)m * p.ldy + c) = o.u;
+    *reinterpret_cast<uint2*>(reinterpret_cast<__bf16*>(p.y) + out_row<PHASE>(p, m) * p.ldy + c) = o.u;
     if (p.rstat_out) {
 #pragma unroll
       for (int r = 0; r < 4; ++r) { const float f = (float)o.e[r]; st[0] += f; st[1] += f * f; }
@@ -286,7 +309,7 @@
   }
 }
 
-template <int MF, int NF, int WTM, int WTN, int WN>
+template <int MF, int NF, int WTM, int WTN, int WN, bool PHASE = false>
 __device__ __forceinline__ void tile_epilogue(const KParams& p, f32x4 (&acc)[MF][NF], int m0, int n0, int tn, int wm, int wn, int lane,
                                               const float (&ln_mean)[MF], const float (&ln_rstd)[MF]) {
   const int frow = lane & 15, fq = lane >> 4;
@@ -306,7 +329,7 @@
           if (n >= p.N) continue;
           float h[4] = {acc[i][j][0], acc[i][j][1], acc[i][j][2], acc[i][j][3]};
           float g[4] = {acc[i][j + 1][0], acc[i][j + 1][1], acc[i][j + 1][2], acc[i][j + 1][3]};
-          epilogue_quad<true>(p, m, rc, n, h, g, st);
+          epilogue_quad<true, PHASE>(p, m, rc, n, h, g, st);
         }
       }
     } else {
@@ -315,7 +338,7 @@
         const int n = n0 + wn * WTN + j * 16 + fq * 4;
         if (n >= p.N) continue;
         float h[4] = {acc[i][j][0], acc[i][j][1], acc[i][j][2], acc[i][j][3]};
-        epilogue_quad<false>(p, m, rc, n, h, h, st);
+        epilogue_quad<false, PHASE>(p, m, rc, n, h, h, st);
       }
     }
     if (p.rstat_out) {
@@ -401,7 +424,7 @@
   if (p.ustat_out) emit_unit_stats<WL>(p, tot, buf, lane, cw0, row0);
 }
 
-template <bool GEGLU, int MF, int NF, int WTM, int WTN, int WN>
+template <bool GEGLU, int MF, int NF, int WTM, int WTN, int WN, bool PHASE = false>
 __device__ __forceinline__ void tile_epilogue_lds(const KParams& p, f32x4 (&acc)[MF][NF], int m0, int n0, int tn, int wm, int wn,
                                                   int lane, const float (&ln_mean)[MF], const float (&ln_rstd)[MF], float* buf) {
   constexpr int WL = GEGLU ? WTN / 2 : WTN;
@@ -495,7 +518,7 @@
         for (int e = 0; e < 8; ++e) v[e] = (1.0f - d) * f[e] + d * v[e];
       }
       const uint4 o = pack_bf16x8(v);
-      if (on) *reinterpret_cast<uint4*>(yb + (int64_t)m2 * p.ldy + c0) = o;
+      if (on) *reinterpret_cast<uint4*>(yb + out_row<PHASE>(p, m2) * p.ldy + c0) = o;
       if constexpr (!GEGLU) {
         if (p.cstat_out && on) {
           float f[8];
@@ -589,7 +612,7 @@
   }
 }
 
-template <int MF, int NF, int WTM, int WTN>
+template <int MF, int NF, int WTM, int WTN, bool PHASE = false>
 __device__ __forceinline__ void lean_epilogue(const KParams& p, f32x4 (&acc)[MF][NF], int m0, int n0, int wm, int wn, int lane,
                                               const LeanEpiIn<WTM, WTN>& in, float* buf) {
   using E = LeanEpiIn<WTM, WTN>;
@@ -666,7 +689,7 @@
         for (int e = 0; e < 8; ++e) v[e] += f[e];
       }
       const uint4 o = pack_bf16x8(v);
-      if (on) *reinterpret_cast<uint4*>(yb + (int64_t)m2 * p.ldy + c0) = o;
+      if (on) *reinterpret_cast<uint4*>(yb + out_row<PHASE>(p, m2) * p.ldy + c0) = o;
       if (p.cstat_out && on) {
         float f[8];
         unpack_bf16x8(o, f);
@@ -735,7 +758,7 @@
   aptp_prefetch_slice(p.pf_ptr, p.pf_bytes, xcd, blockIdx.x >> 3, ((int)gridDim.x + 7 - xcd) >> 3, tid, nt, scratch);
 }
 
-template <int NW, int MF, int NF, int WTM, int WTN, int WN>
+template <int NW, int MF, int NF, int WTM, int WTN, int WN, bool PHASE = false>
 __device__ __forceinline__ void run_epilogue(const KParams& p, f32x4 (&acc)[MF][NF], int m0, int n0, int tn, int wm, int wn, int lane,
                                              int wave, const float (&ln_mean)[MF], const float (&ln_rstd)[MF], __bf16* smem) {
   constexpr int PITCH_MAX = WTN + 4;
@@ -744,12 +767,12 @@
     __syncthreads();
     float* buf = reinterpret_cast<float*>(smem) + wave * 16 * PITCH_MAX;
     if (p.act == APTP_ACT_GEGLU) {
-      if constexpr (NF % 2 == 0) tile_epilogue_lds<true, MF, NF, WTM, WTN, WN>(p, acc, m0, n0, tn, wm, wn, lane, ln_mean, ln_rstd, buf);
+      if constexpr (NF % 2 == 0) tile_epilogue_lds<true, MF, NF, WTM, WTN, WN, PHASE>(p, acc, m0, n0, tn, wm, wn, lane, ln_mean, ln_rstd, buf);
     } else {
-      tile_epilogue_lds<false, MF, NF, WTM, WTN, WN>(p, acc, m0, n0, tn, wm, wn, lane, ln_mean, ln_rstd, buf);
+      tile_epilogue_lds<false, MF, NF, WTM, WTN, WN, PHASE>(p, acc, m0, n0, tn, wm, wn, lane, ln_mean, ln_rstd, buf);
     }
   } else {
-    tile_epilogue<MF, NF, WTM, WTN, WN>(p, acc, m0, n0, tn, wm, wn, lane, ln_mean, ln_rstd);
+    tile_epilogue<MF, NF, WTM, WTN, WN, PHASE>(p, acc, m0, n0, tn, wm, wn, lane, ln_mean, ln_rstd);
   }
 }
 
diff --git a/diffusion_pruning_amd/csrc/conv_gemm_sk.hip b/diffusion_pruning_amd/csrc/conv_gemm_sk.hip
--- a/diffusion_pruning_amd/csrc/conv_gemm_sk.hip
+++ b/diffusion_pruning_amd/csrc/conv_gemm_sk.hip
@@ -364,6 +364,7 @@
 }
 
 int aptp_launch_sk(const KParams& k, int tile, hipStream_t s) {
+  if (k.phase) { aptp_set_error("conv_gemm: the stream-K tiles do not take ups = 3 (phase convolutions)"); return APTP_EINVAL; }
   switch (tile) {
 #define X(NAME, FAMILY, BM, BN, WM, WN, STAGES, KU, KS, LIN, C3) \
     case APTP_TILE_##NAME: return launch_sk_row<TileFamily::FAMILY, BM, BN, WM, WN>(k, tile, s);
diff --git a/diffusion_pruning_amd/csrc/conv_lean.hip b/diffusion_pruning_amd/csrc/conv_lean.hip
--- a/diffusion_pruning_amd/csrc/conv_lean.hip
+++ b/diffusion_pruning_amd/csrc/conv_lean.hip
@@ -12,7 +12,7 @@
 #endif
 }
 
-template <int BM, int BN, int WM, int WN, int STAGES, bool PP, int KU>
+template <int BM, int BN, int WM, int WN, int STAGES, bool PP, int KU, bool PHASE = false>
 __global__ __launch_bounds__(WM * WN * 64) void conv_lean_kernel(const KParams p) {
   constexpr int NW = WM * WN, NT = NW * 64, RPP = NT / 8;
   constexpr int WTM = BM / WM, WTN = BN / WN, MF = WTM / 16, NF = WTN / 16;
@@ -46,17 +46,31 @@
   for (int i = 0; i < A_PASS; ++i) {
     const int m = m0 + rowbase + RPP * i;
     if (m < p.M) {
-      const int b = p.fd_hw.div(m), rem = m - b * p.HW;
-      const int oy = p.fd_wout.div(rem), ox = rem - oy * p.Wout;
-      const int iy0 = oy * p.stride - 1, ix0 = ox * p.stride - 1, pix0 = b * p.Hin * p.Win;
-#pragma unroll
-      for (int t = 0; t < 9; ++t) {
-        int iy = iy0 + t / 3, ix = ix0 + t % 3;
-        const bool ok = (unsigned)iy < (unsigned)p.HinE && (unsigned)ix < (unsigned)p.WinE && !(p.zins & (iy | ix));
-        iy >>= p.ups; ix >>= p.ups;
-        tab[i][t] = ok ? ((unsigned)(pix0 + iy * p.Win + ix) * (unsigned)p.ldx) * 2u + schunk * 16u : ZERO_OFF;
-      }
-      tab[i][9] = p.x2 ? ((unsigned)m * (unsigned)p.ldx2) * 2u + schunk * 16u : ZERO_OFF;
+      if constexpr (PHASE) {
+        int b, iy0, ix0;
+        gather_origin(p, m, b, iy0, ix0);
+        const int pix0 = b * p.Hin * p.Win;
+#pragma unroll
+        for (int t = 0; t < 4; ++t) {
+          const int iy = iy0 + (t >> 1), ix = ix0 + (t & 1);
+          const bool ok = (unsigned)iy < (unsigned)p.Hin && (unsigned)ix < (unsigned)p.Win;
+          tab[i][t] = ok ? ((unsigned)(pix0 + iy * p.Win + ix) * (unsigned)p.ldx) * 2u + schunk * 16u : ZERO_OFF;
+        }
+#pragma unroll
+        for (int t = 4; t < NTAB; ++t) tab[i][t] = ZERO_OFF;
+      } else {
+        const int b = p.fd_hw.div(m), rem = m - b * p.HW;
+        const int oy = p.fd_wout.div(rem), ox = rem - oy * p.Wout;
+        const int iy0 = oy * p.stride - 1, ix0 = ox * p.stride - 1, pix0 = b * p.Hin * p.Win;
+#pragma unroll
+        for (int t = 0; t < 9; ++t) {
+          int iy = iy0 + t / 3, ix = ix0 + t % 3;
+          const bool ok = (unsigned)iy < (unsigned)p.HinE && (unsigned)ix < (unsigned)p.WinE && !(p.zins & (iy | ix));
+          iy >>= p.ups; ix >>= p.ups;
+          tab[i][t] = ok ? ((unsigned)(pix0 + iy * p.Win + ix) * (unsigned)p.ldx) * 2u + schunk * 16u : ZERO_OFF;
+        }
+        tab[i][9] = p.x2 ? ((unsigned)m * (unsigned)p.ldx2) * 2u + schunk * 16u : ZERO_OFF;
+      }
     } else {
 #pragma unroll
       for (int t = 0; t < NTAB; ++t) tab[i][t] = ZERO_OFF;
@@ -74,12 +88,13 @@
   const __amdgpu_buffer_rsrc_t xr = __builtin_amdgcn_make_buffer_rsrc(const_cast<__bf16*>(p.x), 0, p.x_bytes, 0x00020000);
   const __amdgpu_buffer_rsrc_t x2r =
       __builtin_amdgcn_make_buffer_rsrc(const_cast<__bf16*>(p.x2 ? p.x2 : p.x), 0, p.x2 ? p.x2_bytes : 0, 0x00020000);
-  const __amdgpu_buffer_rsrc_t wr = __builtin_amdgcn_make_buffer_rsrc(const_cast<__bf16*>(p.w), 0, p.w_bytes, 0x00020000);
-
+  const __amdgpu_buffer_rsrc_t wr = __builtin_amdgcn_make_buffer_rsrc(const_cast<__bf16*>(p.w) + (PHASE ? phase_w_offset(p, m0) : 0), 0, p.w_bytes, 0x00020000);
+
+  constexpr int ntaps = PHASE ? 4 : 9;
   int l_kt = kt_begin, l_tap = 0, l_cc = kt_begin;
   if (kt_begin != 0) {
     l_tap = kt_begin / p.ncc;
-    if (l_tap > 9) l_tap = 9;
+    if (l_tap > ntaps) l_tap = ntaps;
     l_cc = kt_begin - l_tap * p.ncc;
   }
   auto next_tap = [&]() {
@@ -91,7 +106,7 @@
   for (int t = 0; t < l_tap; ++t) next_tap();
 
   auto issue_tile = [&](int stage) {
-    const bool seg2 = l_tap == 9;
+    const bool seg2 = l_tap == ntaps;
     const int ncur = seg2 ? p.ncc2 : p.ncc;
     const bool pad = l_cc == ncur - 1 && (seg2 ? tail_bad2 : tail_bad);
     const int sa = __builtin_amdgcn_readfirstlane(l_cc * (BK * 2));
@@ -112,7 +127,7 @@
     ++l_kt;
     if (++l_cc == ncur) {
       l_cc = 0;
-      if (l_tap < 9) {
+      if (l_tap < ntaps) {
         ++l_tap;
         next_tap();
       }
@@ -173,14 +188,15 @@
     return;
   }
   __syncthreads();
-  lean_epilogue<MF, NF, WTM, WTN>(p, acc, m0, n0, wm, wn, lane, ein, reinterpret_cast<float*>(smem) + wave * 16 * (WTN + 4));
+  lean_epilogue<MF, NF, WTM, WTN, PHASE>(p, acc, m0, n0, wm, wn, lane, ein, reinterpret_cast<float*>(smem) + wave * 16 * (WTN + 4));
 }
 
 template <int BM, int BN, int WM, int WN, int STAGES, bool PP, int KU>
 void launch_lean(KParams k, hipStream_t s) {
   const int grid = ((k.M + BM - 1) / BM) * ((k.N + BN - 1) / BN) * k.split_k;
   set_prefetch_slices(k, grid);
-  hipLaunchKernelGGL((conv_lean_kernel<BM, BN, WM, WN, STAGES, PP, KU>), dim3(grid), dim3(WM * WN * 64), 0, s, k);
+  if (k.phase) hipLaunchKernelGGL((conv_lean_kernel<BM, BN, WM, WN, STAGES, PP, KU, true>), dim3(grid), dim3(WM * WN * 64), 0, s, k);
+  else hipLaunchKernelGGL((conv_lean_kernel<BM, BN, WM, WN, STAGES, PP, KU>), dim3(grid), dim3(WM * WN * 64), 0, s, k);
 }
 
 }
@@ -188,7 +204,8 @@
 namespace aptp_cg {
 
 bool aptp_conv_lean_eligible(const KParams& k, int tile) {
-  if (k.KH != 3 || k.KW != 3 || k.pad != 1 || (k.stride != 1 && k.stride != 2)) return false;
+  if (k.phase ? (k.KH != 2 || k.KW != 2) : (k.KH != 3 || k.KW != 3)) return false;
+  if (k.pad != 1 || (k.stride != 1 && k.stride != 2)) return false;
   if (k.io_f32 || k.out_f32 || !k.epi16 || k.ln_stats || k.rstat_out || k.depth) return false;
   if (k.act != APTP_ACT_NONE && k.act != APTP_ACT_SILU) return false;
   if (k.Nout < 8 || k.ncc < 1) return false;
diff --git a/diffusion_pruning_amd/launch_policy.py b/diffusion_pruning_amd/launch_policy.py
--- a/diffusion_pruning_amd/launch_policy.py
+++ b/diffusion_pruning_amd/launch_policy.py
@@ -24,6 +24,33 @@
 SPLITK_FORCE_IN_KERNEL = os.environ.get("APTP_SPLITK_FORCE_INKERNEL", "0") == "1"
 COLS_SPLIT_MAX = int(os.environ.get("APTP_COLS_SPLIT_MAX", "2"))
 
+UPS_PHASE = os.environ.get("APTP_UPS_PHASE", "0") == "1"
+UPS_PHASE_MODE = 3
+
+_TILE_ROW = re.compile(r"^\s*X\((\w+),\s*(\w+),\s*(\d+),", re.M)
+_tile_rows = None
+
+
+def tile_rows(tile: int):
+    global _tile_rows
+    if _tile_rows is None:
+        with open(os.path.join(os.path.dirname(os.path.abspath(__file__)), "csrc", "conv_gemm_tiles.h")) as f:
+            _tile_rows = [(int(bm), fam) for _, fam, bm in _TILE_ROW.findall(f.read())]
+    return _tile_rows[tile - 1] if 1 <= tile <= len(_tile_rows) else None
+
+
+def phase_tile_ok(tile: int, phase_rows: int) -> bool:
+    row = tile_rows(tile)
+    return row is not None and row[1] not in ("HALO", "SK", "SKL") and phase_rows % row[0] == 0
+
+
+def phase_out_row(m: int, B: int, Hin: int, Win: int) -> int:
+    q, rem = divmod(m, Hin * Win)
+    y, x = divmod(rem, Win)
+    b, py, px = q >> 2, (q >> 1) & 1, q & 1
+    return b * 4 * Hin * Win + (2 * y + py) * 2 * Win + 2 * x + px
+
+
 _KEY = re.compile(r"M(\d+)_N(\d+)_C(\d+)_T(\d+)_s(\d+)u(\d+)g(\d+)(?:x(\d+))?$")
 
 
@@ -70,8 +97,10 @@
     invalidate()
 
 
-def _nearest(key, M, N, Cin, taps, stride, ups, geglu, Cin2):
+def _nearest(key, M, N, Cin, taps, stride, ups, geglu, Cin2, phase_rows=None):
     global _classes
+    if phase_rows is not None:
+        key = f"{key}@{phase_rows}"
     if key in _near:
         return _near[key]
     if _classes is None:
@@ -87,6 +116,8 @@
             continue
         if v["tile"] >= DMA_TILE_FIRST and max(Cin, Cin2) > DMA_MAX_CHANNELS:
             continue
+        if phase_rows is not None and v["tile"] != 0 and not phase_tile_ok(v["tile"], phase_rows):
+            continue
         dm = math.log2(M / M2)
         d = (0.5 * dm if dm > 0 else -1.5 * dm) + abs(math.log2(N / N2)) + abs(math.log2(K / K2))
         if d < bd:
@@ -111,7 +142,11 @@
     return L.TILE_DMA_128x64 if M >= 8192 else (L.TILE_DMA3_64x64 if M >= 2048 else L.TILE_KU2S4_64x64)
 
 
-def choose_launch(M, N, Cin, cin_pad, KH, KW, stride, ups, act, Cin2, cin2_pad, *, plain_linear, f32, tile, split_k, order):
+def choose_launch(M, N, Cin, cin_pad, KH, KW, stride, ups, act, Cin2, cin2_pad, *, plain_linear, f32, tile, split_k, order,
+                  phase_rows=None):
+    if phase_rows is not None:
+        return _choose_phase(M, N, Cin, cin_pad, KH * KW, stride, ups, act, f32=f32, tile=tile, split_k=split_k, order=order,
+                             phase_rows=phase_rows)
     if split_k is not None or tile != 0 or f32:
         return tile, split_k, None, order
     taps, geglu = KH * KW, act == L.ACT_GEGLU
@@ -139,6 +174,33 @@
     return 0, None, None, order
 
 
+def _choose_phase(M, N, Cin, cin_pad, taps, stride, ups, act, *, f32, tile, split_k, order, phase_rows):
+    stay = (0, split_k, None, order)
+    if tile != 0 or f32:
+        return (tile, split_k, None, order) if tile != 0 and phase_tile_ok(tile, phase_rows) else stay
+    geglu = act == L.ACT_GEGLU
+    key = tuning_key(M, N, Cin, taps, stride, ups, geglu, 0)
+    tuned = TUNING.get(key)
+    if tuned is not None and tuned["tile"] != 0 and not phase_tile_ok(tuned["tile"], phase_rows):
+        tuned = None
+    if tuned is None and TUNING_NEAREST:
+        tuned = _nearest(key, M, N, Cin, taps, stride, ups, geglu, 0, phase_rows)
+    if tuned is not None and tuned["tile"] >= DMA_TILE_FIRST and cin_pad > DMA_MAX_CHANNELS:
+        tuned = None
+    if tuned is not None:
+        if tuned["tile"] == 0:
+            return stay
+        if split_k is not None:
+            return tuned["tile"], split_k, None, order or tuned.get("order", 1)
+        return tuned["tile"], tuned["split_k"], bool(tuned.get("in_kernel", 0)), order or tuned.get("order", 1)
+    if cin_pad > DMA_MAX_CHANNELS:
+        return stay
+    for t in ((L.TILE_DMA3_64x64,) if N <= 64 or M * N < 256 * 128 * 160 else (34, L.TILE_DMA3_64x64)):
+        if phase_tile_ok(t, phase_rows):
+            return t, split_k, None, order
+    return stay
+
+
 def splitk_in_kernel(split_k, in_kernel, *, explicit, reduce_launch, rowstats, colstats) -> bool:
     if reduce_launch:
         return False
diff --git a/diffusion_pruning_amd/ops.py b/diffusion_pruning_amd/ops.py
--- a/diffusion_pruning_amd/ops.py
+++ b/diffusion_pruning_amd/ops.py
@@ -19,7 +19,8 @@
                    GegluParams, GroupNormBwdParams, GroupNormParams, LayerNormBwdParams, LayerNormParams,
                    ColsumParams, LayerNormPgradParams, AttentionWideParams, ImageOutParams)
 from .launch_policy import (BK, SK_AUTO, SK_TILE_FIRST, TUNING, _HALO_TILES, choose_launch, key_of, parse_key,
-                            set_entry, set_tuning, splitk_in_kernel, tuning_key, tuning_lookup)
+                            set_entry, set_tuning, splitk_in_kernel, tuning_key, tuning_lookup, UPS_PHASE_MODE)
+from . import launch_policy as _policy
 
 ACT_DTYPE = torch.bfloat16
 
@@ -76,6 +77,7 @@
     Cin2: int = 0
     cin2_pad: int = 0
     cin_pad_: int = 0
+    phase: Optional["PackedWeight"] = None
 
     @property
     def cin_pad(self) -> int:
@@ -86,10 +88,22 @@
     return (v + m - 1) // m * m
 
 
+def fold_phase_weights(w: torch.Tensor) -> torch.Tensor:
+    assert w.dim() == 4 and w.shape[2] == 3 and w.shape[3] == 3
+
+    def axis(t):
+        a, b, c = t[..., 0], t[..., 1], t[..., 2]
+        return torch.stack([a, b + c], -1), torch.stack([a + b, c], -1)
+    out = []
+    for rows in axis(w.transpose(2, 3)):
+        out += list(axis(rows.transpose(2, 3)))
+    return torch.stack(out, 0)
+
+
 def pack_weight(w: torch.Tensor, bias: Optional[torch.Tensor] = None, *, out_idx: Optional[torch.Tensor] = None,
                 in_idx: Optional[torch.Tensor] = None, n_pad_to: int = 8, cin_pad_to: int = 8,
                 geglu: bool = False, device=None, ln_gamma: Optional[torch.Tensor] = None,
-                ln_beta: Optional[torch.Tensor] = None) -> PackedWeight:
+                ln_beta: Optional[torch.Tensor] = None, ups_phase: bool = False) -> PackedWeight:
     if w.dim() == 2:
         w = w[:, :, None, None]
     device = device or w.device
@@ -148,7 +162,14 @@
     packed = torch.zeros(N, KH * KW, cin_pad, dtype=ACT_DTYPE, device=device)
     packed[:, :, :Cin] = w.permute(0, 2, 3, 1).reshape(N, KH * KW, Cin).to(ACT_DTYPE)
     colsum = packed.float().sum(dim=(1, 2)).contiguous() if ln_gamma is not None else None
-    return PackedWeight(packed.contiguous(), None if bias is None else bias.contiguous(), N, cin_live, KH, KW, geglu, colsum)
+    bias = None if bias is None else bias.contiguous()
+    phase = None
+    if ups_phase:
+        assert KH == 3 and KW == 3 and not geglu and ln_gamma is None, "ups_phase: the 3x3 weights of an upsampler"
+        pk = torch.zeros(4, N, 4, cin_pad, dtype=ACT_DTYPE, device=device)
+        pk[..., :Cin] = fold_phase_weights(w).permute(0, 1, 3, 4, 2).reshape(4, N, 4, Cin).to(ACT_DTYPE)
+        phase = PackedWeight(pk.contiguous(), bias, N, cin_live, 2, 2, cin_pad_=cin_pad)
+    return PackedWeight(packed.contiguous(), bias, N, cin_live, KH, KW, geglu, colsum, phase=phase)
 
 
 def pack_weight_cat(pw: PackedWeight, w2: torch.Tensor, bias2: Optional[torch.Tensor] = None, *,
@@ -319,12 +340,22 @@
             raise ValueError(f"conv_gemm: out shape {tuple(out.shape)} != {(B, Hout, Wout, nout)}")
         if out.dtype != (torch.float32 if out_f32 else torch.bfloat16):
             raise ValueError("conv_gemm: out dtype mismatch")
+    kpw, phase_launch = pw, None
+    if (ups == 1 and pw.phase is not None and _policy.UPS_PHASE and pw.KH == 3 and pw.KW == 3 and stride == 1 and pad == 1
+            and pw.phase.w.dtype == pw.w.dtype and x2 is None and corr is None and residual is None and rowbias is None
+            and colgate is None and depth is None and act in (ACT_NONE, ACT_SILU) and ln is None and not rowstats and gn is None):
+        phase_launch = choose_launch(B * Hout * Wout, pw.N, Cx, pw.cin_pad, 2, 2, 1, UPS_PHASE_MODE, act, 0, 0, plain_linear=False,
+                                     f32=f32, tile=tile, split_k=split_k, order=order, phase_rows=Hin * Win)
+        if phase_launch[0] == 0:
+            phase_launch = None
+        else:
+            kpw, ups = pw.phase, UPS_PHASE_MODE
     p = ConvGemmParams()
     p.x, p.ldx = x.data_ptr(), _ld(x)
     p.B, p.Hin, p.Win, p.Cin, p.Hout, p.Wout = B, Hin, Win, Cx, Hout, Wout
-    p.KH, p.KW, p.stride, p.pad, p.ups = pw.KH, pw.KW, stride, pad, ups
+    p.KH, p.KW, p.stride, p.pad, p.ups = kpw.KH, kpw.KW, stride, pad, ups
     p.pad_end = pad_end
-    p.w, p.N, p.cin_pad = pw.w.data_ptr(), pw.N, pw.cin_pad
+    p.w, p.N, p.cin_pad = kpw.w.data_ptr(), pw.N, pw.cin_pad
     if (x2 is not None) != (pw.Cin2 > 0):
         raise ValueError("conv_gemm: x2 goes with weights packed by pack_weight_cat (and only with them)")
     if x2 is not None:
@@ -368,14 +399,17 @@
     elif PREFETCH_WEIGHTS and prefetch is None:
         plan = _current_prefetch_plan()
         if plan is not None:
-            prefetch = plan.step(pw.w)
+            prefetch = plan.step(kpw.w)
     if prefetch is not None:
         p.prefetch, p.prefetch_bytes = prefetch.data_ptr(), prefetch.numel() * prefetch.element_size()
     plain_linear = pw.KH == 1 and pw.KW == 1 and stride == 1 and not ups and x2 is None and colgate is None and corr is None \
         and rowbias is None and depth is None and not out_f32 and gn is None and (act != ACT_GEGLU or (residual is None and not rowstats))
     p.split_k = 1
-    p.tile, sk, in_kernel, p.order = choose_launch(B * Hout * Wout, pw.N, Cx, pw.cin_pad, pw.KH, pw.KW, stride, ups, act, pw.Cin2, pw.cin2_pad,
-                                                   plain_linear=plain_linear, f32=f32, tile=tile, split_k=split_k, order=order)
+    if phase_launch is not None:
+        p.tile, sk, in_kernel, p.order = phase_launch
+    else:
+        p.tile, sk, in_kernel, p.order = choose_launch(B * Hout * Wout, pw.N, Cx, pw.cin_pad, pw.KH, pw.KW, stride, ups, act, pw.Cin2,
+                                                       pw.cin2_pad, plain_linear=plain_linear, f32=f32, tile=tile, split_k=split_k, order=order)
     p.split_k = max(1, int(lib.aptp_conv_gemm_suggest_split_k(ctypes.byref(p)) if sk is None else sk))
     ws = cnt = None
     gn_fused = False
diff --git a/diffusion_pruning_amd/unet.py b/diffusion_pruning_amd/unet.py
--- a/diffusion_pruning_amd/unet.py
+++ b/diffusion_pruning_amd/unet.py
@@ -3,6 +3,7 @@
 import os
 
 import math
+import dataclasses
 from dataclasses import dataclass, field
 from typing import Any, Dict, List, Optional, Tuple, Union
 
@@ -868,7 +869,7 @@
             from . import autograd as AG
             return _nchw(AG.conv(x, pw, get_bwd, **self.conv_kw))
         dst = _take_dst(self, x.shape[0], *self._out_hw(x.shape[1], x.shape[2]), pw.N, x.device)
-        return _nchw(ops.conv_gemm(x, pw, out=dst, colstats=True, **self.conv_kw))
+        return _nchw(ops.conv_gemm(x, pl.get("pw_infer", pw), out=dst, colstats=True, **self.conv_kw))
 
 
 class Downsample2D(_Resample2D):
@@ -883,6 +884,19 @@
 
 class Upsample2D(_Resample2D):
     conv_kw = {"ups": 1}
+
+    def plan(self, device) -> dict:
+        from . import launch_policy
+        want = launch_policy.UPS_PHASE
+
+        def make():
+            pwp = ops.pack_weight(self.conv.weight.detach(), self.conv.bias.detach(), device=device, ups_phase=want)
+            return {"pw": dataclasses.replace(pwp, phase=None) if want else pwp, "pw_infer": pwp, "phase": want}
+        pl = self._plans.lookup(str(device), _versions(self), make)
+        if want and not pl["phase"]:
+            pl["pw_infer"] = ops.pack_weight(self.conv.weight.detach(), self.conv.bias.detach(), device=device, ups_phase=True)
+            pl["phase"] = True
+        return pl
 
     def _out_hw(self, H, W):
         return 2 * H, 2 * W
```

New measurement: 204.0 steps/s. 0.988x the previous value.
